# AlexandreRouma/SDRPlusPlus

Measured on AMD Instinct MI355X. Metric: IQ Msamples/s ingested (65536-pt FFT + 32 VFO WFM), higher is better.
Workload: dtype f32

## Files before the change

sdrplusplus_amd/csrc/gfx950/sdrpp_gfx950.h:

```cpp
#pragma once
#include <hip/hip_runtime.h>
#include <stdint.h>

namespace sdrpp_k {

struct UniformF32 {
    const float __attribute__((address_space(4))) * p;
    __device__ __forceinline__ float operator[](int i) const { return p[i]; }
};
__device__ __forceinline__ UniformF32 as_uniform(const void* ptr) {
    UniformF32 u;
    u.p = (const float __attribute__((address_space(4)))*)(uintptr_t)ptr;
    return u;
}

struct UniformI32 {
    const int __attribute__((address_space(4))) * p;
    __device__ __forceinline__ int operator[](int i) const { return p[i]; }
};
__device__ __forceinline__ UniformI32 as_uniform_i32(const void* ptr) {
    UniformI32 u;
    u.p = (const int __attribute__((address_space(4)))*)(uintptr_t)ptr;
    return u;
}

__device__ __forceinline__ int wave_uniform(int v) { return __builtin_amdgcn_readfirstlane(v); }

typedef float f32x2 __attribute__((ext_vector_type(2)));
__device__ __forceinline__ float global_load_f32(const float* p, long long i) { return ((const float __attribute__((address_space(1)))*)(uintptr_t)p)[i]; }
__device__ __forceinline__ int global_load_i32(const int* p, long long i) { return ((const int __attribute__((address_space(1)))*)(uintptr_t)p)[i]; }
__device__ __forceinline__ float2 global_load_f32x2(const float2* p, long long i) {
    const f32x2 v = ((const f32x2 __attribute__((address_space(1)))*)(uintptr_t)p)[i];
    return make_float2(v.x, v.y);
}
__device__ __forceinline__ float4 global_load_f32x4(const float4* p, long long i) {
    typedef float f32x4_ld __attribute__((ext_vector_type(4)));
    const f32x4_ld v = ((const f32x4_ld __attribute__((address_space(1)))*)(uintptr_t)p)[i];
    return make_float4(v.x, v.y, v.z, v.w);
}
typedef float f32x4_a4 __attribute__((ext_vector_type(4), aligned(4)));
__device__ __forceinline__ float4 global_load_f32x4_unaligned(const float* p, long long i) {
    const f32x4_a4 v = *((const f32x4_a4 __attribute__((address_space(1)))*)(uintptr_t)(p + i));
    return make_float4(v.x, v.y, v.z, v.w);
}
__device__ __forceinline__ void global_store_f32x2(float2* p, long long i, float2 v) {
    f32x2 t;
    t.x = v.x;
    t.y = v.y;
    ((f32x2 __attribute__((address_space(1)))*)(uintptr_t)p)[i] = t;
}

__device__ __forceinline__ float2 global_load_f32x2_boff(const void* base, unsigned byte_off) {
    const f32x2 v = *((const f32x2 __attribute__((address_space(1)))*)((const char __attribute__((address_space(1)))*)(uintptr_t)base + byte_off));
    return make_float2(v.x, v.y);
}
__device__ __forceinline__ void global_store_f32x2_boff(void* base, unsigned byte_off, float2 v) {
    f32x2 t;
    t.x = v.x;
    t.y = v.y;
    *((f32x2 __attribute__((address_space(1)))*)((char __attribute__((address_space(1)))*)(uintptr_t)base + byte_off)) = t;
}

__device__ __forceinline__ void global_store_f32_boff(void* base, unsigned byte_off, float v) {
    *((float __attribute__((address_space(1)))*)((char __attribute__((address_space(1)))*)(uintptr_t)base + byte_off)) = v;
}

__device__ __forceinline__ float fast_rcp(float x) { return __builtin_amdgcn_rcpf(x); }

typedef float f32x4_a16 __attribute__((ext_vector_type(4)));
__device__ __forceinline__ void global_store_f32x4(float* p, long long i, float4 v) {
    f32x4_a16 t;
    t.x = v.x;
    t.y = v.y;
    t.z = v.z;
    t.w = v.w;
    *((f32x4_a16 __attribute__((address_space(1)))*)(uintptr_t)(p + i)) = t;
}

typedef unsigned u32x4_t __attribute__((ext_vector_type(4)));
__device__ __forceinline__ uint4 global_load_u32x4(const void* p, long long i) {
    const u32x4_t v = ((const u32x4_t __attribute__((address_space(1)))*)(uintptr_t)p)[i];
    return make_uint4(v.x, v.y, v.z, v.w);
}
__device__ __forceinline__ void global_store_u32x4(void* p, long long i, uint4 v) {
    u32x4_t t;
    t.x = v.x; t.y = v.y; t.z = v.z; t.w = v.w;
    ((u32x4_t __attribute__((address_space(1)))*)(uintptr_t)p)[i] = t;
}
__device__ __forceinline__ unsigned global_load_u32(const void* p, long long i) { return ((const unsigned __attribute__((address_space(1)))*)(uintptr_t)p)[i]; }
__device__ __forceinline__ void global_store_u32(void* p, long long i, unsigned v) { ((unsigned __attribute__((address_space(1)))*)(uintptr_t)p)[i] = v; }

__device__ __forceinline__ void global_store_f32x4_unaligned(float* p, long long i, float4 v) {
    f32x4_a4 t;
    t.x = v.x;
    t.y = v.y;
    t.z = v.z;
    t.w = v.w;
    *((f32x4_a4 __attribute__((address_space(1)))*)(uintptr_t)(p + i)) = t;
}

__device__ __forceinline__ void sched_fence() { __builtin_amdgcn_sched_barrier(0); }
__device__ __forceinline__ int opaque(int v) {
    asm volatile("" : "+v"(v));
    return v;
}

__device__ __forceinline__ void wave_sync() {
    __builtin_amdgcn_fence(__ATOMIC_RELEASE, "wavefront");
    __builtin_amdgcn_wave_barrier();
    __builtin_amdgcn_fence(__ATOMIC_ACQUIRE, "wavefront");
}

#ifdef SDRPP_TICK_TRACE
__device__ unsigned long long g_tick_mark[1 << 16][4];
#define TICK_MARK(k)                                                                                      \
    do {                                                                                                  \
        if (threadIdx.x == 0) { g_tick_mark[blockIdx.x & 0xffff][k] = (unsigned long long)wall_clock64(); } \
    } while (0)
#else
#define TICK_MARK(k) \
    do {             \
    } while (0)
#endif

__device__ __forceinline__ void wave_stores_done() { asm volatile("s_waitcnt vmcnt(0) lgkmcnt(0)" ::: "memory"); }

__device__ __forceinline__ int wave_upper_bound(const int* ends, int n, int b, int* prev_end) {
    const int lane = threadIdx.x & 63;
    const int mine = global_load_i32(ends, lane < n ? lane : (n > 0 ? n - 1 : 0));
    const unsigned long long below = __ballot(lane < n && mine <= b);
    const int idx = (int)__builtin_popcountll(below);
    const int prev = __builtin_amdgcn_readlane(mine, idx > 0 ? idx - 1 : 0);
    *prev_end = idx > 0 ? prev : 0;
    return idx;
}

__device__ __forceinline__ void lds_flag_set(int* f, int v) { __hip_atomic_store(f, v, __ATOMIC_RELEASE, __HIP_MEMORY_SCOPE_WORKGROUP); }
#ifndef SDRPP_FLAG_SLEEP
#define SDRPP_FLAG_SLEEP 8
#endif
__device__ __forceinline__ void lds_flag_wait_ge(int* f, int need, int* timeouts) {
    int looks = 0;
    while (__hip_atomic_load(f, __ATOMIC_ACQUIRE, __HIP_MEMORY_SCOPE_WORKGROUP) < need) {
        __builtin_amdgcn_s_sleep(SDRPP_FLAG_SLEEP);
        if (++looks > (1 << 20)) {
            if ((threadIdx.x & 63) == 0 && timeouts) { __hip_atomic_fetch_add(timeouts, 1, __ATOMIC_RELAXED, __HIP_MEMORY_SCOPE_SYSTEM); }
            break;
        }
    }
}

__device__ __forceinline__ int wave_upper_bound64_rec(const int* ends, int n, int b, int* prev_end, const void* recs, int stride_bytes, int (&rec)[6]) {
    const int lane = threadIdx.x & 63;
    const int mine = global_load_i32(ends, lane);
    const float* rp = reinterpret_cast<const float*>(reinterpret_cast<const char*>(recs) + (size_t)lane * (size_t)stride_bytes);
    const float4 r0 = global_load_f32x4_unaligned(rp, 0);
    const float r4 = global_load_f32(rp, 4), r5 = global_load_f32(rp, 5);
    const unsigned long long below = __ballot(lane < n && mine <= b);
    const int idx = __popcll(below);
    const int prev = __builtin_amdgcn_readlane(mine, idx > 0 ? idx - 1 : 0);
    *prev_end = idx > 0 ? prev : 0;
    const int src = idx < 64 ? idx : 63;
    rec[0] = __builtin_amdgcn_readlane(__float_as_int(r0.x), src);
    rec[1] = __builtin_amdgcn_readlane(__float_as_int(r0.y), src);
    rec[2] = __builtin_amdgcn_readlane(__float_as_int(r0.z), src);
    rec[3] = __builtin_amdgcn_readlane(__float_as_int(r0.w), src);
    rec[4] = __builtin_amdgcn_readlane(__float_as_int(r4), src);
    rec[5] = __builtin_amdgcn_readlane(__float_as_int(r5), src);
    return idx;
}

__device__ __forceinline__ void wave_prio_high() { __builtin_amdgcn_s_setprio(3); }
__device__ __forceinline__ void wave_prio_low() { __builtin_amdgcn_s_setprio(0); }

__device__ __forceinline__ float wave_bcast(float v, int src) { return __int_as_float(__builtin_amdgcn_readlane(__float_as_int(v), src)); }
__device__ __forceinline__ float wave_shr1(float v, float first) {
    const float r = __shfl_up(v, 1, 64);
    return ((threadIdx.x & 63) == 0) ? first : r;
}
__device__ __forceinline__ int wave_first(bool pred) {
    const unsigned long long m = __ballot(pred);
    return m ? (int)__builtin_ctzll(m) : 64;
}
__device__ __forceinline__ float wave_sum(float v) {
#pragma unroll
    for (int d = 32; d >= 1; d >>= 1) { v += __shfl_xor(v, d, 64); }
    return v;
}
__device__ __forceinline__ float wave_max(float v) {
#pragma unroll
    for (int d = 32; d >= 1; d >>= 1) {
        const float o = __shfl_xor(v, d, 64);
        v = (o > v) ? o : v;
    }
    return v;
}

typedef float f32x16 __attribute__((ext_vector_type(16)));
__device__ __forceinline__ f32x16 mfma_zero() {
    f32x16 z;
#pragma unroll
    for (int i = 0; i < 16; i++) { z[i] = 0.0f; }
    return z;
}
__device__ __forceinline__ f32x16 mfma_32x32x2(float a, float b, f32x16 c) { return __builtin_amdgcn_mfma_f32_32x32x2f32(a, b, c, 0, 0, 0); }

__device__ __forceinline__ void pk_sum_diff_f32(float2 a, float2 b, f32x2& s, f32x2& d) {
    f32x2 av, bv;
    av.x = a.x; av.y = a.y; bv.x = b.x; bv.y = b.y;
    asm("v_pk_add_f32 %0, %2, %3\n\tv_pk_add_f32 %1, %2, %3 neg_lo:[1,0] neg_hi:[0,1]\n\ts_nop 1" : "=&v"(s), "=&v"(d) : "v"(av), "v"(bv));
}

typedef float f32x4 __attribute__((ext_vector_type(4)));
__device__ __forceinline__ f32x4 mfma4_zero() {
    f32x4 z;
    z[0] = 0.0f; z[1] = 0.0f; z[2] = 0.0f; z[3] = 0.0f;
    return z;
}
__device__ __forceinline__ f32x4 mfma_16x16x4(float a, float b, f32x4 c) { return __builtin_amdgcn_mfma_f32_16x16x4f32(a, b, c, 0, 0, 0); }

}
```

sdrplusplus_amd/csrc/host_ctx.h:

```cpp
#pragma once

namespace {

constexpr int kArenaSlots = 24;
constexpr size_t kArenaBytes = 4u << 20;
constexpr int kRing = 4;
constexpr int kTickDepth = 18;
constexpr int kResSlots = SDRPP_RESULT_SLOTS;
constexpr int kGroupMax = SDRPP_GROUP_MAX;
constexpr int kResMeta = kResSlots * kGroupMax;
constexpr int kStageSlots = 4;
constexpr int kChanHistCap = 4095;
constexpr size_t kScratchBytes = 64u << 20;
constexpr int kMaxLds = 64 * 1024;

enum Family { F_FFT1 = 0, F_FFT2, F_FFTS, F_ZOOM, F_S1, F_DECIM, F_POLY, F_FIR, F_DEMOD, F_MISC, F_AF, F_PIPE, F_TICK };
const char* kFamilyNames[SDRPP_NUM_KERNEL_FAMILIES] = { "fft_pass1", "fft_pass2", "fft_single", "zoom_palette", "vfo_stage1",
                                                        "vfo_decim", "vfo_poly",  "vfo_fir",    "demod",        "carry_misc", "af_chain",  "vfo_pipe", "tick" };

struct Stream {
    int width = 2;
    int hist_len = 0;
    float* data = nullptr;
    float* base = nullptr;
    size_t cap = 0;
    float* hist[2] = { nullptr, nullptr };
    int cur = 0;
    int n = 0;
    float* extra[kRing - 1] = {};
    int n_extra = 0, rot = 0;
    int clevel = 0;
    int wlevel = 0;
};

struct ToepTab {
    float* d_tl = nullptr;
    int* d_lb = nullptr;
    int tl_len = 0, nsteps = 0, s_in = 0, rows = 0, nvar = 0;
    bool ok = false;
};

struct Vfo {
    bool nco_exact = false;
    int id = 0;
    sdrpp_vfo_desc d{};
    std::vector<float> staps[SDRPP_MAX_DECIM_STAGES];
    std::vector<float> rtaps, ctaps_chan, ataps;
    double theta = 0.0, phi = 0.0;
    std::vector<float2> modtaps;
    bool modtaps_dirty = true;
    int soff[SDRPP_MAX_DECIM_STAGES] = { 0, 0, 0, 0 };
    int tpp = 0, pphase = 0, poff = 0;
    long long seen = 0;
    float* d_staps[SDRPP_MAX_DECIM_STAGES] = { nullptr, nullptr, nullptr, nullptr };
    float* d_staps_nat[SDRPP_MAX_DECIM_STAGES] = { nullptr, nullptr, nullptr, nullptr };
    int s_kp[SDRPP_MAX_DECIM_STAGES] = { 0, 0, 0, 0 };
    float* d_bank = nullptr;
    float* d_cyc = nullptr;
    int cyc_rows = 0, cyc_lmax = 0;
    int chan_kp = 0, audio_kp = 0;
    float* d_chan = nullptr;
    int chan_ntaps = 0;
    std::vector<float> chan_stale;
    float* d_audio = nullptr;
    int audio_ntaps = 0;
    char* d_state = nullptr;
    double theta2 = 0.0, phi2 = 0.0;
    std::vector<Stream> st;
    int i_first = 0, i_poly = -1, i_chan = -1, i_dem = -1, i_out = -1, i_if = 0;
    int lvl_if = 1, lvl_out = 1, lvl_af = 1;
    std::vector<int> tk_if, tk_af;
    ToepTab tp_stage[SDRPP_MAX_DECIM_STAGES], tp_poly, tp_chan, tp_audio;
    bool fused_front = false;
    bool no_fuse = false;
    unsigned long long tap_hash = 0;
    float* d_h12 = nullptr;
    int h12_K = 0, h12_lgD = 0;
    struct Retune { long long pos; double theta_before; };
    std::vector<Retune> recs;
    int i_rot = -1;
    float2* d_rot = nullptr;
    struct Af {
        bool on = false;
        int n_stages = 0, decim_s[SDRPP_MAX_DECIM_STAGES] = { 1, 1, 1, 1 };
        std::vector<float> staps[SDRPP_MAX_DECIM_STAGES], rtaps, htaps;
        float* d_staps[SDRPP_MAX_DECIM_STAGES] = { nullptr, nullptr, nullptr, nullptr };
        int s_kp[SDRPP_MAX_DECIM_STAGES] = { 0, 0, 0, 0 };
        ToepTab tp_stage[SDRPP_MAX_DECIM_STAGES], tp_poly, tp_hpf;
        int interp = 1, decim = 1, tpp = 0;
        float* d_bank = nullptr;
        float* d_hpf = nullptr;
        int hpf_kp = 0;
        float alpha = 0.0f;
        float2* d_last = nullptr;
        int state_cur = 0;
        float4* d_seg = nullptr;
        int seg_cap = 0;
        int soff[SDRPP_MAX_DECIM_STAGES] = { 0, 0, 0, 0 };
        int pphase = 0, poff = 0;
        int i_stage0 = -1, i_poly = -1, i_hpf = -1, i_deemp = -1, i_last = -1;
        int base = -1;
    } af;
};

struct TimingPair { hipEvent_t a, b; int family; };

}

struct sdrpp_ctx {
    int device = 0;
    int64_t max_push = 0;
    hipStream_t own_stream = nullptr;
    hipStream_t stream = nullptr;
    hipStream_t fft_stream = nullptr;
    hipStream_t launch_stream = nullptr;
    hipEvent_t ev_fork = nullptr, ev_join = nullptr;
    std::string err;
    std::string devinfo;

    float* iq_land[2] = { nullptr, nullptr };
    int16_t* iq_land16[2] = { nullptr, nullptr };
    hipEvent_t land_ev[2] = { nullptr, nullptr };
    bool land_used[2] = { false, false };
    int land_cur = 0;
    hipStream_t copy_stream = nullptr;
    hipStream_t side_stream = nullptr;
    std::mutex side_mtx;
    bool async_staged = false;
    bool async_inflight = false;
    hipEvent_t ev_copy = nullptr;
    bool deferred = false;
    int64_t pending = 0;
    std::vector<int> pend_ends;
    float* iq_hist[2] = { nullptr, nullptr };
    int iq_hist_cap = 0;
    int iq_cur = 0;

    struct Pre {
        bool ref_order = false;
        bool on = false;
        int n_stages = 0, decim_s[SDRPP_MAX_DECIM_STAGES] = { 1, 1, 1, 1 };
        std::vector<float> staps[SDRPP_MAX_DECIM_STAGES];
        ToepTab tp[SDRPP_MAX_DECIM_STAGES];
        float* d_staps[SDRPP_MAX_DECIM_STAGES] = { nullptr, nullptr, nullptr, nullptr };
        int s_kp[SDRPP_MAX_DECIM_STAGES] = { 0, 0, 0, 0 };
        int soff[SDRPP_MAX_DECIM_STAGES] = { 0, 0, 0, 0 };
        float dc_rate = 0.0f;
        int conj = 0;
        Stream raw;
        std::vector<Stream> st;
        Stream out;
        float2* d_off = nullptr;
        int state_cur = 0;
        float4* d_seg = nullptr;
        int seg_cap = 0;
        const float* last = nullptr;
        int last_n = 0;
    } pre;

    struct Wf {
        int height = 0;
        float* d_ring = nullptr;
        int cur = 0, lines = 0;
        int width = 0;
        float* d_latest = nullptr;
        float* d_smooth = nullptr;
        float* d_hold = nullptr;
        bool hold_on = false, have_latest = false;
        float alpha = 0.0f, beta = 1.0f, hold_speed = 0.0f;
    } wf;

    char* d_pack = nullptr;
    size_t pack_cap = 0;
    float2* d_gather = nullptr;
    size_t gather_cap = 0;
    GatherJob* d_gather_jobs = nullptr;
    int gather_jobs_cap = 0;

    char* arena_host[kArenaSlots] = {};
    char* arena_host_dev[kArenaSlots] = {};
    hipEvent_t arena_ev[kArenaSlots] = {};
    bool arena_used[kArenaSlots] = {};
    char* arena_dev_slot[kArenaSlots] = {};
    char* arena_dev = nullptr;
    int arena_slot = 0;
    size_t arena_off = 0;

    bool fft_on = false;
    int fft_size = 0, fft_lg = 0, nz = 0, skip = 0;
    float* d_window = nullptr;
    float2* d_tw1 = nullptr;
    float2* d_tw2 = nullptr;
    float2* d_twn = nullptr;
    float2* d_scratch = nullptr;
    float* d_lines = nullptr;
    float* d_lines_grp = nullptr;
    int zoom_grp = 0;
    size_t lines_cap = 0;
    int64_t fft_pos = 0, fft_next = 0;
    int n_lines = 0;
    int view_start = 0, view_size = 0, data_width = 0;
    float wf_min = -120.0f, wf_max = 0.0f;
    int32_t* d_zstart = nullptr;
    std::vector<int32_t> h_zstart, h_zcount;
    int zoom_tp_cache = 0, zoom_tp_grp = -1;
    int32_t* d_zcount = nullptr;
    float* d_zoomed = nullptr;
    int32_t* d_index = nullptr;
    size_t zoom_cap = 0;
    struct FftBufs { float2* scratch = nullptr; float* lines = nullptr; float* grp = nullptr; float* zoomed = nullptr; int32_t* index = nullptr; };
    FftBufs fft_extra[kRing - 1];
    int fft_extra_n = 0, fft_rot = 0;

    int ref_block = 0;
    int nco_exact = 0;
    int pipe_on = 1;
    bool pipe_launched = false;
    int timeouts_seen = 0;
    std::vector<int> vfo_bounds;

    std::map<int, std::unique_ptr<Vfo>> vfos;
    std::vector<Vfo*> vfo_list;
// ... 108 lines not shown
```

sdrplusplus_amd/csrc/host_util.h:

```cpp
#pragma once

namespace {

int fail(sdrpp_ctx* c, int code, const char* fmt, ...) {
    char buf[512];
    va_list ap;
    va_start(ap, fmt);
    vsnprintf(buf, sizeof(buf), fmt, ap);
    va_end(ap);
    if (c) { c->err = buf; }
    return code;
}

#define HIPCHK(c, expr)                                                                                           \
    do {                                                                                                          \
        hipError_t e_ = (expr);                                                                                   \
        if (e_ != hipSuccess) { return fail((c), SDRPP_ERR_HIP, "%s failed: %s", #expr, hipGetErrorString(e_)); } \
    } while (0)

template <class T>
int dev_alloc(sdrpp_ctx* c, T** p, size_t count) {
    void* q = nullptr;
    hipError_t e = hipMalloc(&q, std::max<size_t>(count * sizeof(T), 16));
    if (e != hipSuccess) { return fail(c, SDRPP_ERR_NOMEM, "hipMalloc(%zu bytes) failed: %s", count * sizeof(T), hipGetErrorString(e)); }
// ... 173 lines not shown
    }
    if (s.hist_len > 0) {
        HIPCHK(c, hipMemcpy(nh[0] + (size_t)(new_len - s.hist_len) * s.width, s.hist[s.cur], (size_t)s.hist_len * s.width * sizeof(float), hipMemcpyDeviceToDevice));
    }
    dev_free(s.hist[0]);
    dev_free(s.hist[1]);
    s.hist[0] = nh[0];
    s.hist[1] = nh[1];
    s.cur = 0;
    s.hist_len = new_len;
    return SDRPP_OK;
}

int ensure_iq_hist(sdrpp_ctx* c, int need) {
    if (need <= c->iq_hist_cap) { return SDRPP_OK; }
    int cap = std::max(need, 1024);
    float* nh[2] = { nullptr, nullptr };
    for (int i = 0; i < 2; i++) {
        int rc = dev_alloc(c, &nh[i], (size_t)cap * 2);
        if (rc) { return rc; }
        HIPCHK(c, hipMemset(nh[i], 0, (size_t)cap * 2 * sizeof(float)));
    }
    if (c->iq_hist[c->iq_cur] && c->iq_hist_cap > 0) {
        HIPCHK(c, hipStreamSynchronize(c->stream));
        HIPCHK(c, hipMemcpy(nh[0] + (size_t)(cap - c->iq_hist_cap) * 2, c->iq_hist[c->iq_cur], (size_t)c->iq_hist_cap * 2 * sizeof(float), hipMemcpyDeviceToDevice));
    }
    dev_free(c->iq_hist[0]);
    dev_free(c->iq_hist[1]);
    c->iq_hist[0] = nh[0];
    c->iq_hist[1] = nh[1];
    c->iq_cur = 0;
    c->iq_hist_cap = cap;
    return SDRPP_OK;
}

std::vector<float> blocked_taps(const float* h, int K, int D, int* kp_out) {
    const int R = SDRPP_FIR_R;
    const int per = (K + D - 1) / D;
    const int kp = ((per + R - 1) / R) * R;
    std::vector<float> t((size_t)D * kp, 0.0f);
    for (int k = 0; k < K; k++) { t[(size_t)(k % D) * kp + (size_t)(k / D)] = h[k]; }
    *kp_out = kp;
    return t;
}
int upload_blocked(sdrpp_ctx* c, float** dst, const float* h, int K, int D, int* kp) {
    std::vector<float> t = blocked_taps(h, K, D, kp);
    return upload(c, dst, t.data(), t.size());
}

void toep_free(ToepTab& T) {
    dev_free(T.d_tl);
    dev_free(T.d_lb);
    T = ToepTab{};
}
int toep_upload(sdrpp_ctx* c, ToepTab& T, const std::vector<float>& tl, const std::vector<int>& lb) {
    dev_free(T.d_tl);
    dev_free(T.d_lb);
    T.ok = false;
    int rc = upload(c, &T.d_tl, tl.data(), tl.size());
    if (rc) { return rc; }
    rc = upload(c, &T.d_lb, lb.data(), lb.size());
    if (rc) { return rc; }
    T.tl_len = (int)tl.size();
    T.nvar = (int)lb.size() / 64;
    const int span = (2 * 16 - 1) * T.s_in + 4 * T.nsteps, pl = (span + 8) & ~3;
    T.ok = ((size_t)((T.tl_len + 3) & ~3) + (size_t)4 * 2 * pl) * sizeof(float) <= (size_t)(160 * 1024 / 3);
    return SDRPP_OK;
}
int toep_build_fir(sdrpp_ctx* c, ToepTab& T, const float* h, int K, int D) {
    const int rows = 15, padl = (rows - 1) * D, kp = K + padl, nsteps = (kp + 3) / 4;
    const int mainlen = padl + 4 * nsteps + 4, zb = mainlen;
    std::vector<float> tl((size_t)mainlen + 4 * (size_t)nsteps + 4, 0.0f);
    for (int k = 0; k < K; k++) { tl[(size_t)padl + k] = h[k]; }
    std::vector<int> lb(64);
    for (int lane = 0; lane < 64; lane++) {
        const int m = lane & 15, kk = lane >> 4;
        lb[(size_t)lane] = (m < rows) ? padl - D * m + kk : zb + kk;
    }
    T.nsteps = nsteps;
    T.s_in = rows * D;
    T.rows = rows;
    return toep_upload(c, T, tl, lb);
}
int toep_build_poly(sdrpp_ctx* c, ToepTab& T, const std::vector<float>& bank, int L, int M, int tpp) {
    const int cy_n = 15 / L;
    if (cy_n < 1) { return SDRPP_OK; }
    const int rows = cy_n * L, omax = ((L - 1) + (L - 1) * M) / L, shift_max = (cy_n - 1) * M + omax;
    const int kp = shift_max + tpp, nsteps = (kp + 3) / 4, padp = shift_max, row = padp + 4 * nsteps + 4, zb = L * row;
    std::vector<float> tl((size_t)zb + 4 * (size_t)nsteps + 4, 0.0f);
    for (int ph = 0; ph < L; ph++) {
        for (int q = 0; q < tpp; q++) { tl[(size_t)ph * row + (size_t)padp + q] = bank[(size_t)ph * tpp + q]; }
    }
    std::vector<int> lb((size_t)L * 64);
    for (int ph0 = 0; ph0 < L; ph0++) {
        for (int lane = 0; lane < 64; lane++) {
            const int m = lane & 15, kk = lane >> 4;
            if (m < rows) {
                const int cy = m / L, r = m % L, A = ph0 + r * M;
                lb[(size_t)ph0 * 64 + lane] = (A % L) * row + padp - (cy * M + A / L) + kk;
            }
            else { lb[(size_t)ph0 * 64 + lane] = zb + kk; }
        }
    }
    T.nsteps = nsteps;
    T.s_in = cy_n * M;
    T.rows = rows;
    return toep_upload(c, T, tl, lb);
}

void build_modtaps(Vfo& v) {
    const int K = v.d.stage_ntaps[0];
    const int npairs = (K + 1) / 2;
    v.modtaps.resize((size_t)npairs);
    const double kc = 0.5 * (double)(K - 1);
    for (int k = 0; k < npairs; k++) {
        double t = ((double)k - kc) * v.theta;
        t -= std::rint(t);
        const double a = 2.0 * 3.14159265358979323846 * t;
        const double h = (double)v.staps[0][(size_t)k];
        v.modtaps[(size_t)k] = make_float2((float)(h * std::cos(a)), (float)(h * std::sin(a)));
    }
    if (K & 1) { v.modtaps[(size_t)npairs - 1] = make_float2(v.staps[0][(size_t)npairs - 1], 0.0f); }
    v.modtaps_dirty = false;
}

void vfo_free(Vfo& v) {
    for (int i = 0; i < SDRPP_MAX_DECIM_STAGES; i++) { dev_free(v.d_staps[i]); dev_free(v.d_staps_nat[i]); }
    dev_free(v.d_bank);
    dev_free(v.d_cyc);
    dev_free(v.d_chan);
    dev_free(v.d_audio);
    dev_free(v.d_state);
    dev_free(v.d_h12);
    dev_free(v.d_rot);
    for (int i = 0; i < SDRPP_MAX_DECIM_STAGES; i++) { toep_free(v.tp_stage[i]); }
    toep_free(v.tp_poly);
    toep_free(v.tp_chan);
    toep_free(v.tp_audio);
    for (int i = 0; i < SDRPP_MAX_DECIM_STAGES; i++) {
        dev_free(v.af.d_staps[i]);
        toep_free(v.af.tp_stage[i]);
    }
    toep_free(v.af.tp_poly);
    toep_free(v.af.tp_hpf);
    dev_free(v.af.d_bank);
    dev_free(v.af.d_hpf);
    dev_free(v.af.d_last);
    dev_free(v.af.d_seg);
    for (auto& s : v.st) { stream_free(s); }
    v.st.clear();
}

int vfo_reset_state(sdrpp_ctx* c, Vfo& v) {
    v.phi = 0.0;
    v.phi2 = 0.0;
    v.seen = 0;
    v.recs.clear();
    std::fill(v.chan_stale.begin(), v.chan_stale.end(), 0.0f);
    for (int i = 0; i < SDRPP_MAX_DECIM_STAGES; i++) { v.soff[i] = 0; }
    v.pphase = 0;
    v.poff = 0;
    for (int i = 0; i < SDRPP_MAX_DECIM_STAGES; i++) { v.af.soff[i] = 0; }
    v.af.pphase = 0;
    v.af.poff = 0;
    if (v.af.d_last) { HIPCHK(c, hipMemsetAsync(v.af.d_last, 0, 2 * sizeof(float2), c->stream)); }
    for (auto& s : v.st) {
        for (int i = 0; i < 2; i++) {
            if (s.hist[i]) { HIPCHK(c, hipMemsetAsync(s.hist[i], 0, (size_t)std::max(s.hist_len, 1) * s.width * sizeof(float), c->stream)); }
        }
        s.n = 0;
    }
    AgcState st[2];
    for (int i = 0; i < 2; i++) {
        st[i].set_point = v.d.agc_set_point;
        st[i].attack = v.d.agc_attack;
        st[i].inv_attack = 1.0f - v.d.agc_attack;
        st[i].decay = v.d.agc_decay;
        st[i].inv_decay = 1.0f - v.d.agc_decay;
        st[i].max_gain = v.d.agc_max_gain;
        st[i].max_output_amp = v.d.agc_max_output_amp;
        st[i].amp = v.d.agc_set_point / v.d.agc_init_gain;
    }
    char blob[2 * sizeof(AgcState) + sizeof(float)];
    memcpy(blob, st, sizeof(st));
    float zero = 0.0f;
    memcpy(blob + sizeof(st), &zero, sizeof(float));
    HIPCHK(c, hipStreamSynchronize(c->stream));
    HIPCHK(c, hipMemcpy(v.d_state, blob, sizeof(blob), hipMemcpyHostToDevice));
    const float2 unit[2] = { make_float2(1.0f, 0.0f), make_float2(1.0f, 0.0f) };
    HIPCHK(c, hipMemcpy(v.d_rot, unit, sizeof(unit), hipMemcpyHostToDevice));
    return SDRPP_OK;
}

inline int decim_nout(int n, int off, int D) { return (n > off) ? (n - off + D - 1) / D : 0; }
inline int poly_nout(int n, int poff, int pphase, int L, int M) {
    if (n <= poff) { return 0; }
    const long long need = (long long)L * (n - poff) - pphase;
    return (int)((need + M - 1) / M);
}

void bounds_decim(std::vector<int>& b, int off, int D) {
    for (auto& x : b) { x = decim_nout(x, off, D); }
}
void bounds_poly(std::vector<int>& b, int poff, int pphase, int L, int M) {
    for (auto& x : b) { x = poly_nout(x, poff, pphase, L, M); }
}

struct HostProf {
    struct Acc { double total = 0.0, mx = 0.0; long n = 0; };
    std::map<std::string, Acc> acc;
    bool on = getenv("SDRPP_GPU_HOSTPROF") != nullptr;
    void add(const char* name, double us) {
        Acc& a = acc[name];
        a.total += us;
        a.mx = std::max(a.mx, us);
        a.n++;
    }
    void report() {
        if (!on) { return; }
        for (auto& kv : acc) { fprintf(stderr, "[sdrpp hostprof] %-28s n=%6ld avg %8.1f us max %9.1f us\n", kv.first.c_str(), kv.second.n, kv.second.total / (double)kv.second.n, kv.second.mx); }
    }
};
HostProf g_hostprof;
struct HostScope {
    const char* name;
    std::chrono::steady_clock::time_point t0;
    explicit HostScope(const char* n) : name(n) { if (g_hostprof.on) { t0 = std::chrono::steady_clock::now(); } }
    ~HostScope() {
        if (g_hostprof.on) { g_hostprof.add(name, std::chrono::duration<double, std::micro>(std::chrono::steady_clock::now() - t0).count()); }
    }
};

template <class K, class... A>
void launch(sdrpp_ctx* c, K kernel, dim3 grid, dim3 block, size_t lds, A... args) {
    if (c->tick_planning) {
        if (!c->tick_abort && getenv("SDRPP_TICK_DEBUG")) { fprintf(stderr, "[sdrpp tick] ordinary pass because of %s\n", __PRETTY_FUNCTION__); }
        c->tick_abort = true;
        return;
    }
    HostScope hs("launch");
    hipLaunchKernelGGL(kernel, grid, block, lds, c->launch_stream, args...);
}

void launch_role(sdrpp_ctx* c, const sdrpp_ctx::RoleLaunch& r) {
    const TickEntry& e = r.e;
    const dim3 grid((unsigned)e.gx, (unsigned)e.gy), b256(256);
    hipStream_t st = c->launch_stream;
    HostScope hs("launch");
    switch (e.role) {
    case TR_COPY: hipLaunchKernelGGL(copy_kernel, grid, b256, 0, st, (const CopyJob*)e.jobs); break;
    case TR_CARRY: hipLaunchKernelGGL(carry_kernel, grid, b256, 0, st, (const CarryJob*)e.jobs, e.aux); break;
    case TR_ROT: hipLaunchKernelGGL(vfo_rotate_kernel, grid, b256, 0, st, e.p.src, (const RotJob*)e.jobs); break;
    case TR_FCM_132_4: hipLaunchKernelGGL((vfo_frontcm_kernel<10, 132, 4>), grid, b256, r.lds, st, e.p.src, (const FrontCMJob*)e.jobs); break;
    case TR_FCM_6: hipLaunchKernelGGL((vfo_frontcm_kernel<6, 0, 0>), grid, b256, r.lds, st, e.p.src, (const FrontCMJob*)e.jobs); break;
    case TR_FCM_10: hipLaunchKernelGGL((vfo_frontcm_kernel<10, 0, 0>), grid, b256, r.lds, st, e.p.src, (const FrontCMJob*)e.jobs); break;
    case TR_FCM_16: hipLaunchKernelGGL((vfo_frontcm_kernel<16, 0, 0>), grid, b256, r.lds, st, e.p.src, (const FrontCMJob*)e.jobs); break;
    case TR_FCM16_132_4: hipLaunchKernelGGL((vfo_frontcm16_kernel<132, 4>), grid, b256, r.lds, st, e.p.src, (const FrontCMJob*)e.jobs); break;
    case TR_FCL_0: hipLaunchKernelGGL((vfo_frontcl_kernel<0>), grid, dim3(128), r.lds, st, e.p.src, (const FrontCMJob*)e.jobs); break;
    case TR_FCL_PF: hipLaunchKernelGGL((vfo_frontcl_kernel<SDRPP_FCL_PF>), grid, dim3(128), r.lds, st, e.p.src, (const FrontCMJob*)e.jobs); break;
    case TR_TOEP_C: hipLaunchKernelGGL((vfo_toep_kernel<2, 2, false>), grid, b256, r.lds, st, (const ToepJob*)e.jobs); break;
    case TR_TOEP_R: hipLaunchKernelGGL((vfo_toep_kernel<1, 2, false>), grid, b256, r.lds, st, (const ToepJob*)e.jobs); break;
    case TR_TOEP_Q: hipLaunchKernelGGL((vfo_toep_kernel<1, 2, true>), grid, b256, r.lds, st, (const ToepJob*)e.jobs); break;
    case TR_FIRB_C: hipLaunchKernelGGL((vfo_firb_kernel<2, false>), grid, dim3((unsigned)e.aux), r.lds, st, (const FirBJob*)e.jobs); break;
    case TR_FIRB_R: hipLaunchKernelGGL((vfo_firb_kernel<1, false>), grid, dim3((unsigned)e.aux), r.lds, st, (const FirBJob*)e.jobs); break;
    case TR_FIRB_S: hipLaunchKernelGGL((vfo_firb_kernel<1, true>), grid, dim3((unsigned)e.aux), r.lds, st, (const FirBJob*)e.jobs); break;
    case TR_FIRB_Q: hipLaunchKernelGGL((vfo_firb_kernel<1, true, true>), grid, dim3((unsigned)e.aux), r.lds, st, (const FirBJob*)e.jobs); break;
    case TR_PRE: hipLaunchKernelGGL(vfo_demod_pre_kernel, grid, b256, 0, st, (const PreJob*)e.jobs); break;
    case TR_SEQ: hipLaunchKernelGGL(vfo_sequential_kernel, grid, dim3(64), 0, st, (const SeqJob*)e.jobs, e.aux); break;
    case TR_PIPE: hipLaunchKernelGGL(vfo_pipe_kernel<1>, grid, b256, r.lds, st, (const PipeJob*)e.jobs); break;
    case TR_POLYC: hipLaunchKernelGGL(vfo_polyc_kernel, grid, b256, r.lds, st, (const PolyJob*)e.jobs, e.aux); break;
    case TR_DEEMP_P0: hipLaunchKernelGGL((vfo_deemph_kernel<0, 0>), grid, b256, 0, st, (const DeempJob*)e.jobs); break;
    case TR_DEEMP_P1: hipLaunchKernelGGL((vfo_deemph_kernel<0, 1>), grid, b256, 0, st, (const DeempJob*)e.jobs); break;
    case TR_DC_P0: hipLaunchKernelGGL((vfo_deemph_kernel<1, 0>), grid, b256, 0, st, (const DeempJob*)e.jobs); break;
    case TR_DC_P1: hipLaunchKernelGGL((vfo_deemph_kernel<1, 1>), grid, b256, 0, st, (const DeempJob*)e.jobs); break;
    case TR_WF_RING: hipLaunchKernelGGL(wf_ring_store_kernel, grid, b256, 0, st, e.p.wf.src, e.p.wf.n0, e.p.wf.n1, e.p.wf.a, e.p.wf.n2, e.p.wf.n3); break;
    case TR_WF_TRACE: hipLaunchKernelGGL(wf_trace_kernel, grid, b256, 0, st, e.p.wf.src, e.p.wf.n0, e.p.wf.n1, e.p.wf.a, e.p.wf.b, e.p.wf.f0, e.p.wf.f1, e.p.wf.c, e.p.wf.f2); break;
    default: break;
    }
}
void emit(sdrpp_ctx* c, int level, int fam, int role, int gx, int gy, size_t lds, const void* jobs, const IqSrc* src = nullptr, int aux = 0) {
    if (gx <= 0 || gy <= 0) { return; }
    sdrpp_ctx::RoleLaunch r{};
    r.e.role = role;
    r.e.gx = gx;
    r.e.gy = gy;
    r.e.aux = aux;
    r.e.jobs = jobs;
    if (src) { r.e.p.src = *src; }
    r.lds = lds;
    r.level = level;
    r.fam = fam;
    if (c->tick_planning) { c->emits.push_back(r); }
    else { launch_role(c, r); }
}

void emit_wf(sdrpp_ctx* c, int level, int fam, int role, int gx, int gy, const TickWf& q) {
    if (gx <= 0 || gy <= 0) { return; }
    sdrpp_ctx::RoleLaunch r{};
    r.e.role = role;
    r.e.gx = gx;
    r.e.gy = gy;
    r.e.p.wf = q;
    r.level = level;
    r.fam = fam;
    if (c->tick_planning) { c->emits.push_back(r); }
    else { launch_role(c, r); }
}

int pick_tile(int D, int K, int width_bytes) {
    for (int tile : { 256, 128, 64 }) {
        const int extra = (K - 1 + D - 1) / D;
        const size_t lds = (size_t)D * (tile + extra + 1) * width_bytes;
        if (lds <= (size_t)kMaxLds) { return tile; }
    }
    return 0;
}
size_t fir_lds(int tile, int D, int K, int width_bytes) {
    const int extra = (K - 1 + D - 1) / D;
    return (size_t)D * (tile + extra + 1) * width_bytes;
}

}
```

sdrplusplus_amd/csrc/plan_push.h:

```cpp
#pragma once

namespace {

struct PlanSnapshot {
    struct V { int soff[SDRPP_MAX_DECIM_STAGES]; int pphase, poff; double phi, phi2; long long seen; int i_if, lvl_if, lvl_out, lvl_af; int n[24], cur[24]; size_t nrecs;
               int af_soff[SDRPP_MAX_DECIM_STAGES], af_pphase, af_poff, af_last, af_state; };
    std::vector<V> v;
    int64_t fft_pos, fft_next;
    int n_lines, iq_cur, wf_cur, wf_lines;
    bool wf_have;
    int pre_soff[SDRPP_MAX_DECIM_STAGES], pre_state, pre_raw_cur, pre_cur[SDRPP_MAX_DECIM_STAGES];
};
void plan_snapshot(sdrpp_ctx* c, PlanSnapshot& S, bool rotate = false) {
    S.v.resize(c->vfo_list.size());
    for (size_t i = 0; i < c->vfo_list.size(); i++) {
        Vfo& v = *c->vfo_list[i];
        PlanSnapshot::V& q = S.v[i];
        for (int k = 0; k < SDRPP_MAX_DECIM_STAGES; k++) { q.soff[k] = v.soff[k]; q.af_soff[k] = v.af.soff[k]; }
        q.pphase = v.pphase; q.poff = v.poff; q.phi = v.phi; q.phi2 = v.phi2; q.seen = v.seen; q.i_if = v.i_if; q.lvl_if = v.lvl_if; q.lvl_out = v.lvl_out; q.lvl_af = v.lvl_af;
        q.nrecs = v.recs.size();
        q.af_pphase = v.af.pphase; q.af_poff = v.af.poff; q.af_last = v.af.i_last; q.af_state = v.af.state_cur;
        for (size_t k = 0; k < v.st.size() && k < 24; k++) { q.n[k] = v.st[k].n; q.cur[k] = v.st[k].cur; }
        if (rotate) {
            for (auto& st : v.st) { stream_rotate(st); }
        }
    }
    S.fft_pos = c->fft_pos; S.fft_next = c->fft_next; S.n_lines = c->n_lines; S.iq_cur = c->iq_cur;
    S.wf_cur = c->wf.cur; S.wf_lines = c->wf.lines; S.wf_have = c->wf.have_latest;
    for (int k = 0; k < SDRPP_MAX_DECIM_STAGES; k++) { S.pre_soff[k] = c->pre.soff[k]; }
    S.pre_state = c->pre.state_cur;
    S.pre_raw_cur = c->pre.raw.cur;
    for (size_t k = 0; k < c->pre.st.size() && k < SDRPP_MAX_DECIM_STAGES; k++) { S.pre_cur[k] = c->pre.st[k].cur; }
}
void plan_restore(sdrpp_ctx* c, const PlanSnapshot& S) {
    for (size_t i = 0; i < c->vfo_list.size(); i++) {
        Vfo& v = *c->vfo_list[i];
        const PlanSnapshot::V& q = S.v[i];
        for (int k = 0; k < SDRPP_MAX_DECIM_STAGES; k++) { v.soff[k] = q.soff[k]; v.af.soff[k] = q.af_soff[k]; }
        v.pphase = q.pphase; v.poff = q.poff; v.phi = q.phi; v.phi2 = q.phi2; v.seen = q.seen; v.i_if = q.i_if; v.lvl_if = q.lvl_if; v.lvl_out = q.lvl_out; v.lvl_af = q.lvl_af;
        v.af.pphase = q.af_pphase; v.af.poff = q.af_poff; v.af.i_last = q.af_last; v.af.state_cur = q.af_state;
        for (size_t k = 0; k < v.st.size() && k < 24; k++) { v.st[k].n = q.n[k]; v.st[k].cur = q.cur[k]; }
    }
    c->fft_pos = S.fft_pos; c->fft_next = S.fft_next; c->n_lines = S.n_lines; c->iq_cur = S.iq_cur;
    c->wf.cur = S.wf_cur; c->wf.lines = S.wf_lines; c->wf.have_latest = S.wf_have;
    for (int k = 0; k < SDRPP_MAX_DECIM_STAGES; k++) { c->pre.soff[k] = S.pre_soff[k]; }
    c->pre.state_cur = S.pre_state;
    c->pre.raw.cur = S.pre_raw_cur;
    for (size_t k = 0; k < c->pre.st.size() && k < SDRPP_MAX_DECIM_STAGES; k++) { c->pre.st[k].cur = S.pre_cur[k]; }
}

void block_bounds(sdrpp_ctx* c, int64_t count, const std::vector<int>* push_ends) {
    c->arena_begins++;
    c->arena_allocs = 0;
    std::vector<int>& B = c->vfo_bounds;
    B.clear();
    const std::vector<int> whole{ (int)count };
    int64_t lo = 0;
    for (int e : (push_ends ? *push_ends : whole)) {
        if (c->ref_block > 0) {
            for (int64_t q = lo + c->ref_block; q < e; q += c->ref_block) { B.push_back((int)q); }
        }
        if (e > lo || B.empty()) { B.push_back(e); }
        lo = e;
    }
}
int iq_hist_need(sdrpp_ctx* c) {
    int need_hist = 1;
    if (c->fft_on) { need_hist = std::max(need_hist, c->nz - 1); }
    for (auto& kv : c->vfos) {
        const sdrpp_vfo_desc& d = kv.second->d;
        if (d.n_stages > 0) { need_hist = std::max(need_hist, d.stage_ntaps[0] - 1); }
        if (d.n_stages > 1) { need_hist = std::max(need_hist, d.stage_ntaps[0] - 1 + d.stage_decim[0] * (d.stage_ntaps[1] - 1)); }
    }
    return need_hist;
}
CarryJob iq_carry_job(sdrpp_ctx* c, const float* d_iq, int64_t count) {
    int need = 1;
    if (c->fft_on) {
        const int64_t P = (int64_t)c->nz + c->skip;
        const int64_t partial = c->fft_pos - c->fft_next * P;
        if (partial > 0) { need = std::max(need, (int)std::min<int64_t>(partial, c->nz - 1)); }
    }
    for (auto& kv : c->vfos) {
        const sdrpp_vfo_desc& d = kv.second->d;
        if (d.n_stages > 0) { need = std::max(need, d.stage_ntaps[0] - 1); }
        if (d.n_stages > 1) { need = std::max(need, d.stage_ntaps[0] - 1 + d.stage_decim[0] * (d.stage_ntaps[1] - 1)); }
    }
    need = std::min(need, c->iq_hist_cap);
    return CarryJob{ d_iq, c->iq_hist[c->iq_cur], c->iq_hist[c->iq_cur ^ 1], c->iq_hist_cap, (int)count, 2, need };
}

int push_common(sdrpp_ctx* c, const float* d_iq, int64_t count, const std::vector<int>* push_ends = nullptr) {
    if (count == 0) {
        c->n_lines = 0;
        for (auto& kv : c->vfos) {
            for (auto& s : kv.second->st) { s.n = 0; }
        }
        return SDRPP_OK;
    }
    int rc0;
    {
        HostScope hs("arena_begin (backpressure)");
        rc0 = arena_begin(c);
    }
    if (rc0) { return rc0; }
    static thread_local PlanSnapshot snap;
    plan_snapshot(c, snap);
    c->plan_lvl0 = 0;
    block_bounds(c, count, push_ends);
    if (c->pre.on) {
        rc0 = run_preproc(c, &d_iq, &count);
        if (rc0) {
            plan_restore(c, snap);
            return rc0;
        }
        if (count == 0) {
            c->n_lines = 0;
            for (auto& kv : c->vfos) {
                for (auto& s : kv.second->st) { s.n = 0; }
            }
            return arena_end(c);
        }
    }
    int rc = ensure_iq_hist(c, iq_hist_need(c));
    if (rc) {
        plan_restore(c, snap);
        return rc;
    }
    IqSrc src{ (const float2*)d_iq, (const float2*)c->iq_hist[c->iq_cur], c->iq_hist_cap, (long long)count };
    bool fft_work = false;
    if (c->fft_on) {
        const int64_t P = (int64_t)c->nz + c->skip;
        fft_work = (c->fft_pos + count) - c->nz - c->fft_next * P >= 0;
    }
    const bool fork = fft_work && !c->vfos.empty();
    if (fork) {
        HostScope hs("fork events");
        HIPCHK(c, hipEventRecord(c->ev_fork, c->stream));
        HIPCHK(c, hipStreamWaitEvent(c->fft_stream, c->ev_fork, 0));
        c->launch_stream = c->fft_stream;
    }
    {
        HostScope hs("do_fft");
        rc = do_fft(c, src, count);
    }
    c->launch_stream = c->stream;
    if (fork) { (void)hipEventRecord(c->ev_join, c->fft_stream); }
    if (!rc) {
        const CarryJob iqc = iq_carry_job(c, d_iq, count);
        if (c->vfos.empty()) {
            std::vector<CarryJob> carry{ iqc };
            CarryJob* d_carry = arena_push(c, carry);
            rc = arena_commit(c);
            if (!rc) {
                FamilyTimer t(c, F_MISC);
                const int iq_elems = carry[0].need * 2;
                launch(c, carry_kernel, dim3((unsigned)std::max(1, std::min((iq_elems + 8191) / 8192, 512)), 1), dim3(256), 0, (const CarryJob*)d_carry, 0);
            }
        }
        else {
            HostScope hs("do_vfos");
            rc = do_vfos_plan(c, src, count, iqc);
        }
    }
    HostScope hs2("join + arena_end");
    if (fork) { (void)hipStreamWaitEvent(c->stream, c->ev_join, 0); }
    if (rc) {
        plan_restore(c, snap);
        (void)arena_end(c);
        return rc;
    }
    c->iq_cur ^= 1;
    rc = arena_end(c);
    if (rc) { return rc; }
    hipError_t e = hipGetLastError();
    if (e != hipSuccess) { return fail(c, SDRPP_ERR_HIP, "kernel launch failed: %s", hipGetErrorString(e)); }
    return SDRPP_OK;
}

}
```

sdrplusplus_amd/csrc/plan_vfo.h:

```cpp
#pragma once

namespace {

struct S1Member { Vfo* v; int K, lgD, off0, nout; double phi0; int min_idx; int fused, K2, lgD2, off2, nout2; unsigned long long taph;
                  int shift = 0, oshift = 0; };

std::string member_key(char kind, const S1Member* m, int n) {
    unsigned long long h1 = 1469598103934665603ull ^ (unsigned char)kind, h2 = 0x9e3779b97f4a7c15ull + (unsigned char)kind;
    for (int i = 0; i < n; i++) {
        unsigned long long tb;
        memcpy(&tb, &m[i].v->theta, 8);
        const unsigned long long id = (unsigned long long)(unsigned)m[i].v->id;
        h1 = (h1 ^ id) * 1099511628211ull;
        h1 = (h1 ^ tb) * 1099511628211ull;
        h2 ^= id + 0x9e3779b97f4a7c15ull + (h2 << 6) + (h2 >> 2);
        h2 ^= tb + 0x9e3779b97f4a7c15ull + (h2 << 6) + (h2 >> 2);
    }
    char raw[16];
    memcpy(raw, &h1, 8);
    memcpy(raw + 8, &h2, 8);
    return std::string(raw, 16);
}

int front2_t2(int K1, int D1, int K2, int D2, int vt) {
// ... 10 lines not shown
bool frontcm_ok(int K1, int lgD1, int K2, int lgD2, int* pf) {
    const int K = K1 + (K2 - 1) * (1 << lgD1), lgD = lgD1 + lgD2;
    if (K < 9 || lgD < 1 || lgD > 5) { return false; }
    const int nsamp = (SDRPP_FCM_TILE - 1) * (1 << lgD) + K;
    if (nsamp > 16 * 64) { return false; }
    *pf = nsamp <= 6 * 64 ? 6 : (nsamp <= 10 * 64 ? 10 : 16);
    return (size_t)frontcm_layout(K, lgD).total * 4 <= (size_t)(160 * 1024 / 3);
}

ToepJob toep_job(const ToepTab& T, int var, StreamIn in, float* out, int base0, int nout, float inv_dev) {
    ToepJob j{};
    j.in = in;
    j.out = out;
    j.tl = T.d_tl;
    j.lbase = T.d_lb + (size_t)var * 64;
    j.tl_len = T.tl_len;
    j.nsteps = T.nsteps;
    j.s_in = T.s_in;
    j.rows = T.rows;
    j.base0 = base0;
    j.nout = nout;
    j.mt_per_wave = 1;
    j.inv_deviation = inv_dev;
    return j;
}

struct ToepPlan { int grid_x = 0; size_t lds = 0; };
ToepPlan toep_plan(std::vector<ToepJob>& jobs, int npl, int max_blocks = 2048) {
    ToepPlan P;
    if (jobs.empty()) { return P; }
    const int G = 2;
    int mtw = 1;
    for (; mtw < 16; mtw++) {
        size_t blocks = 0;
        for (auto& jb : jobs) { blocks += (size_t)((jb.nout + G * 16 * jb.rows - 1) / (G * 16 * jb.rows) + 4 * mtw - 1) / (size_t)(4 * mtw); }
        if (blocks <= (size_t)max_blocks) { break; }
    }
    for (auto& jb : jobs) {
        jb.mt_per_wave = mtw;
        const int nmt = (jb.nout + G * 16 * jb.rows - 1) / (G * 16 * jb.rows);
        P.grid_x = std::max(P.grid_x, (nmt + 4 * mtw - 1) / (4 * mtw));
        const int span = (G * 16 - 1) * jb.s_in + 4 * jb.nsteps, pl = (span + 8) & ~3;
        P.lds = std::max(P.lds, ((size_t)((jb.tl_len + 3) & ~3) + (size_t)4 * npl * pl) * sizeof(float));
    }
    return P;
}

void launch_toep(sdrpp_ctx* c, std::vector<ToepJob>& jobs, ToepJob* d_jobs, const ToepPlan& P, int width, bool quad) {
    if (jobs.empty() || P.grid_x == 0) { return; }
    const dim3 grid((unsigned)P.grid_x, (unsigned)jobs.size());
    if (quad) { launch(c, vfo_toep_kernel<1, 2, true>, grid, dim3(256), P.lds, (const ToepJob*)d_jobs); }
    else if (width == 2) { launch(c, vfo_toep_kernel<2, 2, false>, grid, dim3(256), P.lds, (const ToepJob*)d_jobs); }
    else { launch(c, vfo_toep_kernel<1, 2, false>, grid, dim3(256), P.lds, (const ToepJob*)d_jobs); }
}

constexpr int kPipeG = 1;
constexpr int kPipeBpc = 5;
constexpr int kPipeBpcMin = 3;
bool pipe_layout_try(PipeJob& J, int fifo_tiles, size_t* lds_bytes) {
    const int G = kPipeG;
    int off = 0;
    auto take = [&](int nfloats) { const int o = off; off += (nfloats + 3) & ~3; return o; };
    for (int s = 0; s < 4; s++) { J.tl_off[s] = take(J.st[s].tl_len); }
    int W[4], span[4], omt[4];
    for (int s = 0; s < 4; s++) {
        W[s] = G * 16 * J.st[s].s_in;
        span[s] = W[s] - J.st[s].s_in + 4 * J.st[s].nsteps;
        omt[s] = G * 16 * J.st[s].rows;
    }
    if (((span[0] + 1) >> 1) > (G == 1 ? 5 : 9) * 64) { return false; }
    J.win_off = take(2 * ((span[0] + 8) & ~3));
    J.zero_lo = off;
    for (int i = 0; i < 3; i++) {
        const int s = i + 1, h = span[s] - W[s];
        if (h < 0) { return false; }
        const int R = std::max(2, (W[s] + h + omt[i] + W[s] - 1) / W[s]) * W[s];
        if (i < 2) {
            J.ring_len[i] = R;
            J.ring_mir[i] = h;
            J.ring_off[i] = take(2 * (R + h));
        }
        else {
            J.dring_len = R;
            J.dring_mir = h;
            J.dring_off = take(R + h);
        }
    }
    J.ring_len[2] = fifo_tiles * omt[2];
    J.ring_mir[2] = 0;
    J.ring_off[2] = take(J.ring_len[2]);
    J.zero_hi = off;
    J.flag_off = take(8);
    *lds_bytes = (size_t)off * sizeof(float);
    return *lds_bytes <= (size_t)(160 * 1024) / kPipeBpcMin;
}
bool pipe_layout(PipeJob& J, size_t* lds_bytes) { return pipe_layout_try(J, 2, lds_bytes) || pipe_layout_try(J, 1, lds_bytes); }
int pipe_segments(const std::vector<PipeJob>& pipes, int forced, size_t lds) {
    if (pipes.empty()) { return 0; }
    const int bpc = std::max(kPipeBpcMin, std::min(kPipeBpc, (int)((size_t)(160 * 1024) / std::max<size_t>(lds, 1))));
    int max_nmt = 1;
    for (auto& pj : pipes) { max_nmt = std::max(max_nmt, (pj.st[3].nout + kPipeG * 16 * pj.st[3].rows - 1) / (kPipeG * 16 * pj.st[3].rows)); }
    if (forced >= 2) { return std::min(forced, max_nmt); }
    const int s_full = (256 * bpc + (int)pipes.size() - 1) / (int)pipes.size();
    if (max_nmt >= 12 * s_full) { return s_full; }
    if (max_nmt <= 16) { return std::max(1, (max_nmt + 1) / 2); }
    return 0;
}

constexpr int kLevels = 28;
template <class T>
struct Lev {
    std::vector<T> at[kLevels];
    T* dev[kLevels] = {};
    int top = 0;
    void add(int l, const T& j) {
        if (l >= kLevels) { l = kLevels - 1; }
        at[l].push_back(j);
        if (l + 1 > top) { top = l + 1; }
    }
};
template <class T>
bool arena_push_lev(sdrpp_ctx* c, Lev<T>& L) {
    for (int l = 0; l < L.top; l++) {
        if (L.at[l].empty()) { continue; }
        L.dev[l] = arena_push(c, L.at[l]);
        if (!L.dev[l]) { return false; }
    }
    return true;
}

struct BankPlan {
    sdrpp_ctx* c;
    IqSrc src{};
    int n_in = 0;
    bool ticking = false;
    int L0 = 0;
    static constexpr int carry_last = kLevels - 1;
    static constexpr int carry_wave_max = 8192;
    const std::vector<int>& fb;
    bool blocks = false;
    std::vector<S1Member> s1;
    std::vector<RotJob> rot;
    Lev<FirBJob> f_dec;
    std::vector<RotXJob> rotx;
    std::vector<RetuneJob> retune;
    Lev<PolyJob> poly;
    Lev<PolyBJob> polyb[4];
    Lev<FirBJob> chan;
    Lev<SeqJob> seq;
    Lev<PreJob> pre;
    Lev<FirBJob> audio;
    Lev<FirBJob> audio_fm;
    Lev<ToepJob> t_dec, t_poly, t_chan, t_audio, t_audio_fm;
    std::vector<PipeJob> pipes;
    size_t pipe_lds = 0;
    PipeJob* d_pipes = nullptr;
    int pipe_seg = 0;
    int pipe_lvl = 0;
    Lev<ToepJob> t_af_dec, t_af_poly, t_af_hpf;
    Lev<FirBJob> af_dec, af_hpf;
    Lev<PolyJob> af_poly;
    Lev<DeempJob> af_deemp;
    Lev<SsbRotXJob> ssbx_l;
    Lev<CarryJob> carry;
    int max_rot = 0;
    struct S1Launch { int vt; std::vector<Stage1Job> jobs; int max_nout = 0; int tile = 256; size_t lds = 0; };
    struct F2Launch { int vt; std::vector<Front2Job> jobs; int max_blocks = 0; size_t lds = 0; };
    struct FCMLaunch { std::vector<FrontCMJob> jobs; int max_blocks = 0; size_t lds = 0; };
    S1Launch s1l[4];
    F2Launch f2l[4];
    FCMLaunch fcm[3];
    FCMLaunch fcl;
    int fcl_nw = 2;
    const int vts[4] = { 8, 4, 2, 1 };
    Stage1Job* d_s1[4] = {};
    Front2Job* d_f2[4] = {};
    FrontCMJob* d_fcl = nullptr;
    FrontCMJob* d_fcm[3] = {};
    RotXJob* d_rotx = nullptr;
    RotXHead* d_rotx_head = nullptr;
    RetuneJob* d_retune = nullptr;
    RotJob* d_rot = nullptr;
    const int* d_fb = nullptr;
    struct ToepList { Lev<ToepJob>* L; int npl, width; bool quad; int fam; int role; };
    static constexpr int kToepLists = 8;
    ToepList tlists[kToepLists] = { { &t_dec, 2, 2, false, F_DECIM, TR_TOEP_C },      { &t_poly, 2, 2, false, F_POLY, TR_TOEP_C },       { &t_chan, 2, 2, false, F_FIR, TR_TOEP_C },
                                    { &t_audio, 1, 1, false, F_FIR, TR_TOEP_R },      { &t_audio_fm, 2, 1, true, F_FIR, TR_TOEP_Q },     { &t_af_dec, 2, 2, false, F_AF, TR_TOEP_C },
                                    { &t_af_poly, 2, 2, false, F_AF, TR_TOEP_C },     { &t_af_hpf, 2, 2, false, F_AF, TR_TOEP_C } };
    ToepPlan tplan[kToepLists][kLevels];

    explicit BankPlan(sdrpp_ctx* c_) : c(c_), fb(c_->vfo_bounds) {
        for (int i = 0; i < 4; i++) { s1l[i].vt = vts[i]; f2l[i].vt = vts[i]; }
    }
    template <class T>
    static void lev_reset(Lev<T>& L) {
        for (int l = 0; l < L.top; l++) {
            L.at[l].clear();
            L.dev[l] = nullptr;
        }
        L.top = 0;
    }
    void begin(const IqSrc& src_, int64_t count, const CarryJob& iq_carry) {
        src = src_;
        n_in = (int)count;
        ticking = c->tick_planning;
        L0 = ticking ? c->plan_lvl0 : 0;
        blocks = fb.size() > 1;
        s1.clear(); rot.clear(); rotx.clear(); retune.clear(); pipes.clear();
        lev_reset(f_dec); lev_reset(poly);
        for (auto& q : polyb) { lev_reset(q); }
        lev_reset(chan); lev_reset(seq); lev_reset(pre); lev_reset(audio); lev_reset(audio_fm);
        lev_reset(t_dec); lev_reset(t_poly); lev_reset(t_chan); lev_reset(t_audio); lev_reset(t_audio_fm);
        lev_reset(t_af_dec); lev_reset(t_af_poly); lev_reset(t_af_hpf); lev_reset(af_dec); lev_reset(af_hpf); lev_reset(af_poly); lev_reset(af_deemp);
        lev_reset(ssbx_l); lev_reset(carry);
        pipe_lds = 0;
        d_pipes = nullptr;
        pipe_seg = 0;
        pipe_lvl = 0;
        max_rot = 0;
        fcl_nw = 2;
        for (int i = 0; i < 4; i++) {
            s1l[i].jobs.clear(); s1l[i].max_nout = 0; s1l[i].tile = 256; s1l[i].lds = 0;
            f2l[i].jobs.clear(); f2l[i].max_blocks = 0; f2l[i].lds = 0;
            d_s1[i] = nullptr;
            d_f2[i] = nullptr;
        }
        for (int i = 0; i < 3; i++) {
            fcm[i].jobs.clear(); fcm[i].max_blocks = 0; fcm[i].lds = 0;
            d_fcm[i] = nullptr;
        }
        fcl.jobs.clear(); fcl.max_blocks = 0; fcl.lds = 0;
        d_fcl = nullptr; d_rotx = nullptr; d_retune = nullptr; d_rot = nullptr; d_fb = nullptr;
        for (auto& row : tplan) {
            for (auto& q : row) { q = ToepPlan{}; }
        }
        carry.add(ticking ? L0 + 1 : carry_last, iq_carry);
    }
    BankPlan(const BankPlan&) = delete;
    BankPlan& operator=(const BankPlan&) = delete;

    int chain(Vfo& v) {
        Stream* cur = &v.st[(size_t)v.i_first];
        int lvl = L0 + 1;
        for (auto& s : v.st) { s.clevel = 0; s.wlevel = 0; }
        cur->wlevel = lvl;
        const bool agc_mode = v.d.demod == SDRPP_DEMOD_AM || (v.d.demod >= SDRPP_DEMOD_USB && v.d.demod <= SDRPP_DEMOD_DSB);
        const bool need_bnd = agc_mode && (blocks || v.nco_exact);
        std::vector<int> bnd;
        if (need_bnd) { bnd = fb; }
        const bool split = c->grp_ends.size() > 1;
        std::vector<int>& tk = v.tk_if;
        tk.clear();
        v.tk_af.clear();
        if (split) { tk = c->grp_ends; }
        int first_sep = 0;
        double phi_end = 0.0;
        bool have_phi_end = false;
        if (v.nco_exact) {
            Stream* tgt = (v.d.n_stages == 0) ? cur : &v.st[(size_t)v.i_rot];
            rotx.push_back(RotXJob{ (float2*)tgt->data, v.d_rot, v.d.phase_delta_re, v.d.phase_delta_im });
            tgt->n = n_in;
            tgt->wlevel = lvl;
            cur = tgt;
        }
        else if (v.d.n_stages == 0) {
            rot.push_back(RotJob{ v.theta, v.phi, (float2*)cur->data, n_in });
            cur->n = n_in;
            max_rot = std::max(max_rot, n_in);
        }
        else {
            const int D = v.d.stage_decim[0];
            const int nout = decim_nout(n_in, v.soff[0], D);
            if (v.modtaps_dirty) { build_modtaps(v); }
            const int K0 = v.d.stage_ntaps[0];
            S1Member mem{ &v, K0, ilog2(D), v.soff[0], nout, v.phi, 0, 0, 0, 0, 0, 0, v.tap_hash };
            int need = K0 - 1;
            first_sep = 1;
            if (need_bnd) { bounds_decim(bnd, v.soff[0], D); }
            if (split) { bounds_decim(tk, v.soff[0], D); }
            if (v.fused_front) {
                const int D2 = v.d.stage_decim[1];
                mem.fused = 1;
                mem.K2 = v.d.stage_ntaps[1];
                mem.lgD2 = ilog2(D2);
                mem.off2 = v.soff[1];
                mem.nout2 = decim_nout(nout, v.soff[1], D2);
                need = K0 - 1 + D * (mem.K2 - 1);
                first_sep = 2;
                if (need_bnd) { bounds_decim(bnd, v.soff[1], D2); }
                if (split) { bounds_decim(tk, v.soff[1], D2); }
            }
            mem.min_idx = (v.seen >= need) ? -need : -(int)v.seen;
            if (!split) { s1.push_back(mem); }
            else {
                int so0 = v.soff[0], so1 = v.soff[1], prev_e = 0, oshift = 0;
                long long seen = v.seen;
                double ph = v.phi;
                for (size_t j = 0; j < c->grp_ends.size(); j++) {
                    const int nj = c->grp_ends[j] - prev_e;
                    S1Member m = mem;
                    m.off0 = so0;
                    m.nout = decim_nout(nj, so0, D);
                    m.phi0 = ph;
                    int outs = m.nout;
                    if (mem.fused) {
                        m.off2 = so1;
                        m.nout2 = decim_nout(m.nout, so1, v.d.stage_decim[1]);
                        outs = m.nout2;
                    }
                    m.min_idx = ((seen >= need) ? -need : -(int)seen) + prev_e;
                    m.shift = prev_e;
                    m.oshift = oshift;
                    if (outs > 0) { s1.push_back(m); }
                    so0 = so0 + m.nout * D - nj;
                    if (mem.fused) { so1 = so1 + m.nout2 * v.d.stage_decim[1] - m.nout; }
                    const double pj = ph + (double)nj * v.theta;
                    ph = pj - std::floor(pj);
                    seen += nj;
                    oshift += outs;
                    prev_e = c->grp_ends[j];
                }
                phi_end = ph;
                have_phi_end = true;
            }
            {
                const int D1 = D, Kc = v.h12_K;
                const int off = mem.fused ? mem.off0 + (mem.off2 - (mem.K2 - 1)) * D1 - (K0 - 1) : mem.off0 - (K0 - 1);
                const int nout_f = mem.fused ? mem.nout2 : nout;
                while (!v.recs.empty() && v.recs.front().pos - v.seen <= (long long)off) { v.recs.erase(v.recs.begin()); }
                while (v.recs.size() > SDRPP_RETUNE_MAX_SEG - 1) { v.recs.erase(v.recs.begin()); }
                if (!v.recs.empty() && nout_f > 0) {
                    const long long r_last = v.recs.back().pos - v.seen;
                    const long long Dc = 1ll << v.h12_lgD;
                    const int nfix = (int)std::min<long long>((long long)nout_f, (r_last - off + Dc - 1) / Dc);
                    if (nfix > 0) {
                        RetuneJob rj{};
                        rj.out = (float2*)v.st[(size_t)v.i_first + (mem.fused ? 1 : 0)].data;
                        rj.taps = v.d_h12;
                        rj.K = Kc;
                        rj.log2_decim = v.h12_lgD;
                        rj.off = off;
                        rj.nfix = nfix;
                        rj.min_idx = mem.min_idx;
                        const int nr = (int)v.recs.size();
                        rj.nseg = nr + 1;
                        double P = v.phi + v.theta * (double)r_last;
                        for (int q = nr; q >= 1; q--) {
                            const long long Sq = v.recs[(size_t)q - 1].pos - v.seen;
                            rj.start[q] = (int)std::max<long long>(Sq, -2000000000ll);
                            rj.theta[q] = (q == nr) ? v.theta : v.recs[(size_t)q].theta_before;
                            rj.phi[q] = P - std::floor(P);
                            if (q >= 2) {
                                const long long Sp = v.recs[(size_t)q - 2].pos - v.seen;
                                P = P + v.recs[(size_t)q - 1].theta_before * (double)(Sp - Sq);
                            }
                        }
                        rj.start[0] = rj.start[1];
                        rj.theta[0] = v.recs[0].theta_before;
                        rj.phi[0] = rj.phi[1];
                        retune.push_back(rj);
                    }
                }
            }
            v.soff[0] = v.soff[0] + nout * D - n_in;
            cur->n = nout;
            if (mem.fused) {
                Stream* nxt = &v.st[(size_t)v.i_first + 1];
                v.soff[1] = v.soff[1] + mem.nout2 * v.d.stage_decim[1] - nout;
                cur->n = 0;
                nxt->n = mem.nout2;
                nxt->wlevel = lvl;
                cur = nxt;
            }
        }
        const int last_dec = v.d.n_stages - 1;
        bool piped_be = c->pipe_on && !ticking && (v.d.demod == SDRPP_DEMOD_WFM || v.d.demod == SDRPP_DEMOD_NFM) && last_dec >= first_sep && v.tp_stage[last_dec].ok &&
                        v.i_poly >= 0 && v.tp_poly.ok && v.i_chan >= 0 && v.chan_ntaps > 0 && v.tp_chan.ok && v.tp_audio.ok;
        PipeJob pj{};
        size_t pj_lds = 0;
        if (piped_be) {
            pj.st[0] = toep_job(v.tp_stage[last_dec], 0, StreamIn{}, nullptr, 0, 0, 0.0f);
            pj.st[1] = toep_job(v.tp_poly, 0, StreamIn{}, nullptr, 0, 0, 0.0f);
            pj.st[2] = toep_job(v.tp_chan, 0, StreamIn{}, nullptr, 0, 0, 0.0f);
            pj.st[3] = toep_job(v.tp_audio, 0, StreamIn{}, nullptr, 0, 0, 0.0f);
            pj.timeouts = c->hd_tick_flag ? (int*)(c->hd_tick_flag + 8) : nullptr;
            piped_be = pipe_layout(pj, &pj_lds);
        }
        for (int s = first_sep; s < v.d.n_stages; s++) {
            Stream* nxt = &v.st[(size_t)v.i_first + s];
            const int Ds = v.d.stage_decim[s];
            const int no = decim_nout(cur->n, v.soff[s], Ds);
            if (need_bnd) { bounds_decim(bnd, v.soff[s], Ds); }
            if (split) { bounds_decim(tk, v.soff[s], Ds); }
            lvl++;
            cur->clevel = lvl;
            if (piped_be && s == last_dec) {
                pj.st[0] = toep_job(v.tp_stage[s], 0, stream_in(*cur), nxt->data, v.soff[s] - (v.d.stage_ntaps[s] - 1), no, 0.0f);
                pj.keep[0] = std::max(0, no - nxt->hist_len);
                pj.dec_stage = s;
                pj.lvl = lvl;
            }
            else if (v.tp_stage[s].ok) { t_dec.add(lvl, toep_job(v.tp_stage[s], 0, stream_in(*cur), nxt->data, v.soff[s] - (v.d.stage_ntaps[s] - 1), no, 0.0f)); }
            else { f_dec.add(lvl, FirBJob{ stream_in(*cur), nxt->data, v.d_staps[s], v.d.stage_ntaps[s], ilog2(Ds), v.soff[s], no, v.s_kp[s] }); }
            v.soff[s] = v.soff[s] + no * Ds - cur->n;
            nxt->n = no;
            nxt->wlevel = lvl;
            cur = nxt;
        }
        if (v.i_poly >= 0) {
            Stream* nxt = &v.st[(size_t)v.i_poly];
            const int no = poly_nout(cur->n, v.poff, v.pphase, v.d.interp, v.d.decim);
            if (need_bnd) { bounds_poly(bnd, v.poff, v.pphase, v.d.interp, v.d.decim); }
            if (split) { bounds_poly(tk, v.poff, v.pphase, v.d.interp, v.d.decim); }
            lvl++;
            cur->clevel = lvl;
            if (piped_be) {
                pj.st[1] = toep_job(v.tp_poly, v.pphase, stream_in(*cur), nxt->data, v.poff - (v.tpp - 1), no, 0.0f);
                pj.keep[1] = std::max(0, no - nxt->hist_len);
            }
            else if (v.tp_poly.ok) { t_poly.add(lvl, toep_job(v.tp_poly, v.pphase, stream_in(*cur), nxt->data, v.poff - (v.tpp - 1), no, 0.0f)); }
            else if (v.d_cyc) {
                polyb[(v.cyc_lmax == 4 ? 0 : 1) + ((v.d.decim & 1) ? 2 : 0)].add(lvl, PolyBJob{ stream_in(*cur), (float2*)nxt->data, v.d_cyc + (size_t)v.pphase * v.cyc_rows * v.cyc_lmax, v.d.interp, v.d.decim,
                                                                  v.tpp, v.poff, no, v.cyc_rows });
            }
            else {
                poly.add(lvl, PolyJob{ stream_in(*cur), (float2*)nxt->data, v.d_bank, v.d.interp, v.d.decim, v.tpp, v.pphase, v.poff, no });
            }
            const long long A = (long long)v.pphase + (long long)no * v.d.decim;
            v.pphase = (int)(A % v.d.interp);
            v.poff = v.poff + (int)(A / v.d.interp) - cur->n;
            nxt->n = no;
            nxt->wlevel = lvl;
            cur = nxt;
        }
        if (v.i_chan >= 0 && v.chan_ntaps > 0) {
            Stream* nxt = &v.st[(size_t)v.i_chan];
            lvl++;
            cur->clevel = lvl;
            if (piped_be) {
                pj.st[2] = toep_job(v.tp_chan, 0, stream_in(*cur), nxt->data, -(v.chan_ntaps - 1), cur->n, 0.0f);
                pj.keep[2] = 0;
            }
            else if (v.tp_chan.ok) { t_chan.add(lvl, toep_job(v.tp_chan, 0, stream_in(*cur), nxt->data, -(v.chan_ntaps - 1), cur->n, 0.0f)); }
            else { chan.add(lvl, FirBJob{ stream_in(*cur), nxt->data, v.d_chan, v.chan_ntaps, 0, 0, cur->n, v.chan_kp }); }
            nxt->n = cur->n;
            nxt->wlevel = lvl;
            cur = nxt;
        }
        v.i_if = (int)(cur - &v.st[0]);
        v.lvl_if = lvl;
        v.lvl_out = lvl;
        const int nif = cur->n;
        AgcState* agc = (AgcState*)v.d_state;
        float* dc = (float*)(v.d_state + 2 * sizeof(AgcState));
        const int* d_bnd = nullptr;
        if (need_bnd) {
            d_bnd = arena_push(c, bnd);
            if (!d_bnd) { return fail(c, SDRPP_ERR_UNSUPPORTED, "job arena exhausted"); }
        }
        const int nbnd = need_bnd ? (int)bnd.size() : 0;
        if (v.d.demod == SDRPP_DEMOD_WFM || v.d.demod == SDRPP_DEMOD_NFM) {
            Stream& out = v.st[(size_t)v.i_out];
            lvl++;
            cur->clevel = lvl;
            if (piped_be) {
                pj.st[3] = toep_job(v.tp_audio, 0, stream_in(*cur), out.data, -(v.audio_ntaps - 1), nif, v.d.inv_deviation);
                pipes.push_back(pj);
                pipe_lds = std::max(pipe_lds, pj_lds);
            }
            else if (v.tp_audio.ok) { t_audio_fm.add(lvl, toep_job(v.tp_audio, 0, stream_in(*cur), out.data, -(v.audio_ntaps - 1), nif, v.d.inv_deviation)); }
            else { audio_fm.add(lvl, FirBJob{ stream_in(*cur), out.data, v.d_audio, v.audio_ntaps, 0, 0, nif, v.audio_kp, v.d.inv_deviation }); }
            out.n = nif;
            out.wlevel = lvl;
            v.lvl_out = lvl;
        }
        else if (v.d.demod == SDRPP_DEMOD_AM) {
            Stream& dem = v.st[(size_t)v.i_dem];
            Stream& out = v.st[(size_t)v.i_out];
            if (!v.d.am_carrier_agc) { pre.add(lvl + 1, PreJob{ 2, nif, (const float2*)cur->data, dem.data, 0.0, 0.0 }); }
            seq.add(lvl + 2, SeqJob{ 2, nif, (const float2*)cur->data, dem.data, nullptr, agc, agc + 1, dc, v.d.dc_block_rate, v.d.am_carrier_agc, d_bnd, nbnd });
            dem.n = nif;
            dem.wlevel = lvl + 2;
            lvl += 3;
            dem.clevel = lvl;
            if (v.tp_audio.ok) { t_audio.add(lvl, toep_job(v.tp_audio, 0, stream_in(dem), out.data, -(v.audio_ntaps - 1), nif, 0.0f)); }
            else { audio.add(lvl, FirBJob{ stream_in(dem), out.data, v.d_audio, v.audio_ntaps, 0, 0, nif, v.audio_kp }); }
            out.n = nif;
            out.wlevel = lvl;
            v.lvl_out = lvl;
        }
        else if (v.d.demod >= SDRPP_DEMOD_USB && v.d.demod <= SDRPP_DEMOD_DSB) {
            Stream& dem = v.st[(size_t)v.i_dem];
            Stream& out = v.st[(size_t)v.i_out];
            if (v.nco_exact) { ssbx_l.add(lvl + 1, SsbRotXJob{ (const float2*)cur->data, dem.data, v.d_rot + 1, v.d.ssb_phase_delta_re, v.d.ssb_phase_delta_im, d_bnd, nbnd }); }
            else if (split) {
                int lo = 0;
                for (size_t j = 0; j < tk.size(); j++) {
                    const int nj = tk[j] - lo;
                    if (nj > 0) { pre.add(lvl + 1, PreJob{ v.d.demod, nj, (const float2*)cur->data + lo, dem.data + (size_t)lo * (size_t)dem.width, v.theta2, v.phi2 }); }
                    const double q2 = v.phi2 + (double)nj * v.theta2;
                    v.phi2 = q2 - std::floor(q2);
                    lo = tk[j];
                }
            }
            else { pre.add(lvl + 1, PreJob{ v.d.demod, nif, (const float2*)cur->data, dem.data, v.theta2, v.phi2 }); }
            seq.add(lvl + 2, SeqJob{ v.d.demod, nif, (const float2*)cur->data, dem.data, out.data, agc, agc + 1, dc, 0.0f, 0, d_bnd, nbnd });
            lvl += 2;
            dem.n = 0;
            out.n = nif;
            out.wlevel = lvl;
            v.lvl_out = lvl;
            if (!split || v.nco_exact) {
                const double p2 = v.phi2 + (double)nif * v.theta2;
                v.phi2 = p2 - std::floor(p2);
            }
        }
        if (v.af.on && v.i_out >= 0) {
            Vfo::Af& a = v.af;
            Stream* acur = &v.st[(size_t)v.i_out];
            if (split) { v.tk_af = tk; }
            for (int s = 0; s < a.n_stages; s++) {
                Stream* nxt = &v.st[(size_t)a.i_stage0 + s];
                const int Ds = a.decim_s[s], K = (int)a.staps[s].size();
                const int no = decim_nout(acur->n, a.soff[s], Ds);
                if (split) { bounds_decim(v.tk_af, a.soff[s], Ds); }
                lvl++;
                acur->clevel = lvl;
                if (a.tp_stage[s].ok) { t_af_dec.add(lvl, toep_job(a.tp_stage[s], 0, stream_in(*acur), nxt->data, a.soff[s] - (K - 1), no, 0.0f)); }
                else { af_dec.add(lvl, FirBJob{ stream_in(*acur), nxt->data, a.d_staps[s], K, ilog2(Ds), a.soff[s], no, a.s_kp[s] }); }
                a.soff[s] = a.soff[s] + no * Ds - acur->n;
                nxt->n = no;
                nxt->wlevel = lvl;
                acur = nxt;
            }
            if (a.i_poly >= 0) {
                Stream* nxt = &v.st[(size_t)a.i_poly];
                const int no = poly_nout(acur->n, a.poff, a.pphase, a.interp, a.decim);
                if (split) { bounds_poly(v.tk_af, a.poff, a.pphase, a.interp, a.decim); }
                lvl++;
                acur->clevel = lvl;
                if (a.tp_poly.ok) { t_af_poly.add(lvl, toep_job(a.tp_poly, a.pphase, stream_in(*acur), nxt->data, a.poff - (a.tpp - 1), no, 0.0f)); }
                else { af_poly.add(lvl, PolyJob{ stream_in(*acur), (float2*)nxt->data, a.d_bank, a.interp, a.decim, a.tpp, a.pphase, a.poff, no }); }
                const long long A = (long long)a.pphase + (long long)no * a.decim;
                a.pphase = (int)(A % a.interp);
                a.poff = a.poff + (int)(A / a.interp) - acur->n;
                nxt->n = no;
                nxt->wlevel = lvl;
                acur = nxt;
            }
            if (a.i_hpf >= 0) {
                Stream* nxt = &v.st[(size_t)a.i_hpf];
                const int K = (int)a.htaps.size();
                lvl++;
                acur->clevel = lvl;
                if (a.tp_hpf.ok) { t_af_hpf.add(lvl, toep_job(a.tp_hpf, 0, stream_in(*acur), nxt->data, -(K - 1), acur->n, 0.0f)); }
                else { af_hpf.add(lvl, FirBJob{ stream_in(*acur), nxt->data, a.d_hpf, K, 0, 0, acur->n, a.hpf_kp }); }
                nxt->n = acur->n;
                nxt->wlevel = lvl;
                acur = nxt;
            }
            if (a.i_deemp >= 0) {
                Stream* nxt = &v.st[(size_t)a.i_deemp];
                lvl++;
                const int nseg = std::min(a.seg_cap, (acur->n + SDRPP_DEEMP_SEG - 1) / SDRPP_DEEMP_SEG);
                af_deemp.add(lvl, DeempJob{ (const float2*)acur->data, (float2*)nxt->data, acur->n, a.alpha, a.d_last + a.state_cur, a.d_last + (a.state_cur ^ 1),
                                             a.d_seg + (size_t)a.state_cur * ((size_t)a.seg_cap + 1), nseg, 0 });
                if (nseg > 0) { a.state_cur ^= 1; }
                nxt->n = acur->n;
                lvl += 1;
                nxt->wlevel = lvl;
                acur = nxt;
            }
            a.i_last = (int)(acur - &v.st[0]);
            v.lvl_af = lvl;
        }
        if (have_phi_end) { v.phi = phi_end; }
        else {
            const double p = v.phi + (double)n_in * v.theta;
            v.phi = p - std::floor(p);
        }
        v.seen += n_in;
        const Stream* phantom = (v.fused_front && v.d.n_stages >= 2 && !v.nco_exact) ? &v.st[(size_t)v.i_first] : nullptr;
        for (auto& s : v.st) {
            if (s.hist_len > 0 && s.data && &s != phantom) {
                const int cl = !ticking ? carry_last : (s.clevel > 0 ? s.clevel : (s.wlevel > 0 ? s.wlevel + 1 : lvl + 1));
                carry.add(cl, CarryJob{ s.data, s.hist[s.cur], s.hist[s.cur ^ 1], s.hist_len, s.n, s.width, s.hist_len });
            }
        }
        c->plan_top = std::max(c->plan_top, lvl + 2);
        return SDRPP_OK;
    }

    int group_front() {
        auto same = [](const S1Member& a, const S1Member& b) {
            return a.fused == b.fused && a.K == b.K && a.lgD == b.lgD && a.off0 == b.off0 && a.nout == b.nout && a.min_idx == b.min_idx && a.K2 == b.K2 &&
                   a.lgD2 == b.lgD2 && a.off2 == b.off2 && a.nout2 == b.nout2 && a.taph == b.taph && a.shift == b.shift && a.oshift == b.oshift;
        };
        std::sort(s1.begin(), s1.end(), [](const S1Member& a, const S1Member& b) {
            if (a.fused != b.fused) { return a.fused < b.fused; }
            if (a.K != b.K) { return a.K < b.K; }
            if (a.lgD != b.lgD) { return a.lgD < b.lgD; }
            if (a.off0 != b.off0) { return a.off0 < b.off0; }
            if (a.nout != b.nout) { return a.nout < b.nout; }
            if (a.min_idx != b.min_idx) { return a.min_idx < b.min_idx; }
            if (a.K2 != b.K2) { return a.K2 < b.K2; }
            if (a.lgD2 != b.lgD2) { return a.lgD2 < b.lgD2; }
            if (a.off2 != b.off2) { return a.off2 < b.off2; }
            if (a.nout2 != b.nout2) { return a.nout2 < b.nout2; }
            if (a.taph != b.taph) { return a.taph < b.taph; }
            if (a.shift != b.shift) { return a.shift < b.shift; }
            if (a.oshift != b.oshift) { return a.oshift < b.oshift; }
            return a.v->id < b.v->id;
        });
        if (ticking) {
            fcl_nw = 4;
            for (auto& m : s1) {
                if (!m.fused && m.lgD >= 5 && m.K >= 9 && (size_t)frontcl_lds_floats(m.K, m.lgD, 4) * 4 > (size_t)(160 * 1024 / 2)) { fcl_nw = 2; }
            }
        }
        size_t i = 0;
        while (i < s1.size()) {
            size_t j = i;
            while (j < s1.size() && same(s1[j], s1[i])) { j++; }
            size_t g = i;
            int m_pf = 0;
            const bool m_fused = s1[i].fused && frontcm_ok(s1[i].K, s1[i].lgD, s1[i].K2, s1[i].lgD2, &m_pf);
            const bool m_long = !m_fused && !s1[i].fused && s1[i].lgD >= 5 && s1[i].K >= 9 && (size_t)frontcl_lds_floats(s1[i].K, s1[i].lgD) * 4 <= (size_t)kMaxLds;
            const bool m_ok = m_fused || m_long;
            const size_t m_min = m_long ? 2 : 17;
            while (m_ok && j - g >= m_min) {
                const int vt = (int)std::min<size_t>(j - g, SDRPP_FCM_VT);
                S1Member h = s1[g];
                if (m_long) {
                    h.K2 = 1;
                    h.lgD2 = 0;
                    h.off2 = 0;
                    h.nout2 = h.nout;
                }
                const int D1 = 1 << h.lgD;
                const int K = h.K + (h.K2 - 1) * D1, lgD = h.lgD + h.lgD2;
                const int NP = (K + 1) / 2, NP4 = (NP + 31) / 32 * 32;
                const std::string key = member_key(m_long ? 'L' : 'M', &s1[g], vt);
                float2* d_taps = nullptr;
                auto it = c->s1_tap_cache.find(key);
                if (it != c->s1_tap_cache.end()) { d_taps = it->second; }
                else {
                    std::vector<float2> host((size_t)NP4 * 32 + (size_t)SDRPP_FCM_VT * SDRPP_FCM_TILE, make_float2(0.0f, 0.0f));
                    float* at = reinterpret_cast<float*>(host.data());
                    std::vector<double> h12((size_t)K);
                    const double kc = 0.5 * (double)(K - 1);
                    for (int m = 0; m < vt; m++) {
                        const Vfo& vv = *s1[g + m].v;
                        std::fill(h12.begin(), h12.end(), 0.0);
                        for (int k2 = 0; k2 < h.K2; k2++) {
                            const double w2 = m_long ? 1.0 : (double)vv.staps[1][(size_t)k2];
                            for (int k1 = 0; k1 < h.K; k1++) { h12[(size_t)k2 * D1 + k1] += w2 * (double)vv.staps[0][(size_t)k1]; }
                        }
                        for (int pz = 0; pz < NP; pz++) {
                            double t = ((double)pz - kc) * vv.theta;
                            t -= std::rint(t);
                            const double a = 2.0 * 3.14159265358979323846 * t;
                            double gr = h12[(size_t)pz] * std::cos(a), gi = h12[(size_t)pz] * std::sin(a);
                            if ((K & 1) && pz == NP - 1) { gr = h12[(size_t)pz]; gi = 0.0; }
                            at[(size_t)pz * 64 + m] = (float)gr;
                            at[(size_t)pz * 64 + 32 + m] = (float)-gi;
                        }
                    }
                    for (int m = 0; m < SDRPP_FCM_VT; m++) {
                        const double step = m < vt ? s1[g + m].v->theta * (double)(1 << lgD) : 0.0;
                        for (int jj = 0; jj < SDRPP_FCM_TILE; jj++) {
                            double tt = step * (double)jj;
                            tt -= std::rint(tt);
                            const double a = 2.0 * 3.14159265358979323846 * tt;
                            host[(size_t)NP4 * 32 + (size_t)m * SDRPP_FCM_TILE + jj] = make_float2((float)std::cos(a), (float)std::sin(a));
                        }
                    }
                    if (c->s1_tap_cache.size() > 4096) {
                        HIPCHK(c, hipStreamSynchronize(c->stream));
                        for (auto& e : c->s1_tap_cache) { (void)hipFree(e.second); }
                        c->s1_tap_cache.clear();
                    }
                    int rc = dev_alloc(c, &d_taps, host.size());
                    if (rc) { return rc; }
                    HIPCHK(c, hipMemcpyAsync(d_taps, host.data(), host.size() * sizeof(float2), hipMemcpyHostToDevice, c->stream));
                    HIPCHK(c, hipStreamSynchronize(c->stream));
                    c->s1_tap_cache[key] = d_taps;
                }
                FrontCMJob job{};
                job.nv = vt;
                job.ntaps = K;
                job.log2_decim = lgD;
                job.off = h.off0 + (h.off2 - (h.K2 - 1)) * D1 - (h.K - 1) + h.shift;
                job.nout = h.nout2;
                job.min_idx = h.min_idx;
                job.anchor = h.shift;
                const int tile_n = (m_long && vt <= 16) ? 16 : SDRPP_FCM_TILE;
                const int ntiles = (h.nout2 + tile_n - 1) / tile_n;
                const int long_blocks = m_long ? std::max(1, (int)((size_t)(160 * 1024) / ((size_t)frontcl_lds_floats(K, lgD, fcl_nw) * 4))) : 0;
                const int nsub = std::max<int>(1, (int)c->grp_ends.size());
                const int resident = std::max(64, (m_long ? 256 * long_blocks * fcl_nw : (c->tick_planning ? std::min(3072, c->tick_fcm_waves) : 3072)) / nsub);
                job.tiles_per_wave = std::max(1, (ntiles + resident - 1) / resident);
                job.atab = reinterpret_cast<const float*>(d_taps);
                job.ptab = d_taps + (size_t)NP4 * 32;
                for (int m = 0; m < SDRPP_FCM_VT; m++) {
                    Vfo* v = s1[g + std::min(m, vt - 1)].v;
                    job.theta[m] = v->theta;
                    job.phi0[m] = s1[g + std::min(m, vt - 1)].phi0;
                    job.out[m] = (float2*)v->st[(size_t)v->i_first + (m_long ? 0 : 1)].data + h.oshift;
                }
                if (m_long) {
                    fcl.jobs.push_back(job);
                    fcl.max_blocks = std::max(fcl.max_blocks, (ntiles + fcl_nw * job.tiles_per_wave - 1) / (fcl_nw * job.tiles_per_wave));
                    fcl.lds = std::max(fcl.lds, (size_t)frontcl_lds_floats(K, lgD, fcl_nw) * 4);
                }
                else {
                    FCMLaunch& L = fcm[m_pf == 6 ? 0 : (m_pf == 10 ? 1 : 2)];
                    L.jobs.push_back(job);
                    L.max_blocks = std::max(L.max_blocks, (ntiles + 4 * job.tiles_per_wave - 1) / (4 * job.tiles_per_wave));
                    L.lds = std::max(L.lds, (size_t)frontcm_layout(K, lgD).total * 4);
                }
                g += (size_t)vt;
            }
            while (g < j) {
                const size_t left = j - g;
                int li = left >= 8 ? 0 : (left >= 4 ? 1 : (left >= 2 ? 2 : 3));
                if (ticking) { li = 3; }
                const int vt = vts[li];
                const std::string key = member_key('V', &s1[g], vt);
                float2* d_taps = nullptr;
                auto it = c->s1_tap_cache.find(key);
                if (it != c->s1_tap_cache.end()) { d_taps = it->second; }
                else {
                    const int K = (s1[g].K + 1) / 2;
                    std::vector<float2> host((size_t)K * vt + (size_t)256 * vt);
                    for (int k = 0; k < K; k++) {
                        for (int m = 0; m < vt; m++) { host[(size_t)k * vt + m] = s1[g + m].v->modtaps[(size_t)k]; }
                    }
// ... 306 lines not shown
            const int tile = threads * R;
            emit(c, level, fam, width == 2 ? TR_FIRB_C : (quad ? TR_FIRB_Q : (stereo ? TR_FIRB_S : TR_FIRB_R)), (max_nout + tile - 1) / tile, (int)jobs.size(), lds, d_jobs, nullptr, threads);
            return SDRPP_OK;
    }
    int launch_polyc(int level, int fam, std::vector<PolyJob>& jobs, PolyJob* d_jobs) {
            if (jobs.empty()) { return SDRPP_OK; }
            int cap2 = kMaxLds / (int)sizeof(float2);
            if (ticking) {
                int need = c->tick_lds_cap / (int)sizeof(float2);
                for (auto& jb : jobs) { need = std::max(need, jb.tpp + 2 * jb.decim + 1); }
                cap2 = std::min(cap2, need);
            }
            bool fits = true;
            int max_nout = 0, max_tiles = 0;
            for (auto& jb : jobs) {
                max_nout = std::max(max_nout, jb.nout);
                const int ct = std::min(64, (cap2 - jb.tpp - jb.decim) / jb.decim);
                if (ct < 1) { fits = false; continue; }
                const int ncyc = (jb.nout + jb.interp - 1) / jb.interp;
                max_tiles = std::max(max_tiles, (ncyc + ct - 1) / ct);
            }
            if (max_nout == 0) { return SDRPP_OK; }
            if (fits) {
                const int ppw = (long long)max_tiles * (long long)jobs.size() >= 64 ? 6 : 2;
                int G = 1;
                for (auto& jb : jobs) { G = std::max(G, ((jb.interp + 3) / 4 + ppw - 1) / ppw); }
                if (!ticking && (long long)max_tiles * (long long)jobs.size() >= 1024) { G = 1; }
                G = std::max(1, std::min(G, 128));
                emit(c, level, fam, TR_POLYC, max_tiles * G, (int)jobs.size(), (size_t)cap2 * sizeof(float2), d_jobs, nullptr, cap2 | ((G - 1) << 24));
                return SDRPP_OK;
            }
            size_t lds = 0;
            const int tile = 256;
            for (auto& jb : jobs) {
                const size_t ns = (size_t)((long long)tile * jb.decim / jb.interp) + jb.tpp + 4;
                lds = std::max(lds, ns * sizeof(float2));
            }
            if (lds > (size_t)kMaxLds) { return fail(c, SDRPP_ERR_UNSUPPORTED, "polyphase tile does not fit in LDS"); }
            if (c->tick_planning) { emit(c, level, fam, TR_POLY, (max_nout + tile - 1) / tile, (int)jobs.size(), lds, d_jobs); }
            else { launch(c, vfo_poly_kernel, dim3((max_nout + tile - 1) / tile, (unsigned)jobs.size()), dim3(tile), lds, (const PolyJob*)d_jobs); }
            return SDRPP_OK;
    }
    int launch_polyb(int li, std::vector<PolyBJob>& jobs, PolyBJob* d_jobs) {
            if (jobs.empty()) { return SDRPP_OK; }
            int max_cycles = 0, threads = 256;
            size_t lds = 0;
            auto lds_for = [&](const PolyBJob& jb, int nt) { return (size_t)jb.decim * (size_t)(nt + jb.rows / jb.decim + 2) * sizeof(float2); };
            for (auto& jb : jobs) {
                max_cycles = std::max(max_cycles, (jb.nout + jb.interp - 1) / jb.interp);
                int nt = 256;
                while (nt >= 32 && lds_for(jb, nt) > (size_t)kMaxLds) { nt >>= 1; }
                if (nt < 32) { return fail(c, SDRPP_ERR_UNSUPPORTED, "polyphase tile does not fit in LDS"); }
                threads = std::min(threads, nt);
            }
            if (max_cycles == 0) { return SDRPP_OK; }
            while (threads > 64 && (size_t)((max_cycles + threads - 1) / threads) * jobs.size() < 2048) { threads >>= 1; }
            for (auto& jb : jobs) { lds = std::max(lds, lds_for(jb, threads)); }
            const dim3 grid((max_cycles + threads - 1) / threads, (unsigned)jobs.size());
            if (li == 0) { launch(c, vfo_polyb_kernel<4, false>, grid, dim3(threads), lds, (const PolyBJob*)d_jobs); }
            else if (li == 1) { launch(c, vfo_polyb_kernel<8, false>, grid, dim3(threads), lds, (const PolyBJob*)d_jobs); }
            else if (li == 2) { launch(c, vfo_polyb_kernel<4, true>, grid, dim3(threads), lds, (const PolyBJob*)d_jobs); }
            else { launch(c, vfo_polyb_kernel<8, true>, grid, dim3(threads), lds, (const PolyBJob*)d_jobs); }
            return SDRPP_OK;
    }
    void emit_toep(int i, int l) {
            Lev<ToepJob>& L = *tlists[i].L;
            if (l >= L.top || L.at[l].empty() || tplan[i][l].grid_x == 0) { return; }
            emit(c, l, tlists[i].fam, tlists[i].role, tplan[i][l].grid_x, (int)L.at[l].size(), tplan[i][l].lds, L.dev[l]);
    }
    void launch_carry(int l) {
            std::vector<CarryJob>& cj = carry.at[l];
            if (cj.empty()) { return; }
            const bool has_iq = (l == (ticking ? L0 + 1 : carry_last));
            const int iq_elems = has_iq ? cj[0].need * cj[0].width : 0;
            int mx = 0;
            for (size_t k = has_iq ? 1 : 0; k < cj.size(); k++) { mx = std::max(mx, cj[k].need * cj[k].width); }
            auto per_vfo = [&](const CarryJob* dev, int njobs) {
                if (njobs <= 0) { return; }
                if (mx <= carry_wave_max) { emit(c, l, F_MISC, TR_CARRY, 1, (njobs + 3) / 4, 0, dev, nullptr, njobs); }
                else { emit(c, l, F_MISC, TR_CARRY, std::max(1, std::min((mx + 8191) / 8192, 64)), njobs, 0, dev); }
            };
            if (!ticking && iq_elems > carry_wave_max && iq_elems <= 128 * 1024 * 2 && cj.size() > 1) {
                emit(c, l, F_MISC, TR_CARRY, 32, (int)cj.size(), 0, carry.dev[l]);
            }
            else if (has_iq && (iq_elems > carry_wave_max || cj.size() == 1)) {
                emit(c, l, F_MISC, TR_CARRY, std::max(1, std::min((iq_elems + 8191) / 8192, 512)), 1, 0, carry.dev[l]);
                per_vfo(carry.dev[l] + 1, (int)cj.size() - 1);
            }
            else {
                mx = std::max(mx, iq_elems);
                per_vfo(carry.dev[l], (int)cj.size());
            }
    }

    int emit_levels() {
        int rc = SDRPP_OK;
        int top = std::max({ t_dec.top, t_poly.top, t_chan.top, t_audio.top, t_audio_fm.top, t_af_dec.top, t_af_poly.top, t_af_hpf.top, f_dec.top, poly.top,
                             polyb[0].top, polyb[1].top, polyb[2].top, polyb[3].top, chan.top, seq.top, pre.top, audio.top, audio_fm.top, af_dec.top, af_hpf.top,
                             af_poly.top, af_deemp.top, ssbx_l.top, carry.top, d_pipes ? pipe_lvl + 1 : 0 });
        for (int l = 1; l < top; l++) {
            {
                FamilyTimer t(c, F_DECIM);
                emit_toep(0, l);
                if (l < f_dec.top) {
                    rc = launch_fir(l, F_DECIM, f_dec.at[l], f_dec.dev[l], 2, false);
                    if (rc) { return rc; }
                }
            }
            if (d_pipes && l == pipe_lvl) {
                FamilyTimer t(c, F_PIPE);
                c->pipe_launched = true;
                emit(c, l, F_PIPE, TR_PIPE, pipe_seg, (int)pipes.size(), pipe_lds, d_pipes);
            }
            {
                FamilyTimer t(c, F_POLY);
                emit_toep(1, l);
                if (l < poly.top) {
                    rc = launch_polyc(l, F_POLY, poly.at[l], poly.dev[l]);
                    if (rc) { return rc; }
                }
                for (int li = 0; li < 4; li++) {
                    if (l < polyb[li].top) {
                        rc = launch_polyb(li, polyb[li].at[l], polyb[li].dev[l]);
                        if (rc) { return rc; }
                    }
                }
            }
            {
                FamilyTimer t(c, F_FIR);
                emit_toep(2, l);
                if (l < chan.top) {
                    rc = launch_fir(l, F_FIR, chan.at[l], chan.dev[l], 2, false);
                    if (rc) { return rc; }
                }
            }
            if ((l < pre.top && !pre.at[l].empty()) || (l < seq.top && !seq.at[l].empty()) || (l < ssbx_l.top && !ssbx_l.at[l].empty())) {
                FamilyTimer t(c, F_DEMOD);
                if (l < ssbx_l.top && !ssbx_l.at[l].empty()) {
                    const int nj = (int)ssbx_l.at[l].size();
                    if (c->tick_planning) { emit(c, l, F_DEMOD, TR_SSBX, (nj + 3) / 4, 1, 0, ssbx_l.dev[l], nullptr, nj); }
                    else { launch(c, vfo_ssb_rotate_exact_kernel, dim3((unsigned)nj), dim3(64), 0, (const SsbRotXJob*)ssbx_l.dev[l]); }
                }
                if (l < pre.top && !pre.at[l].empty()) {
                    int mx = 0;
                    for (auto& q : pre.at[l]) { mx = std::max(mx, q.n); }
                    if (mx > 0) { emit(c, l, F_DEMOD, TR_PRE, std::min((mx + 255) / 256, 1024), (int)pre.at[l].size(), 0, pre.dev[l]); }
                }
                if (l < seq.top && !seq.at[l].empty()) { emit(c, l, F_DEMOD, TR_SEQ, (int)seq.at[l].size(), 1, 0, seq.dev[l], nullptr, (int)seq.at[l].size()); }
            }
            {
                FamilyTimer t(c, F_FIR);
                emit_toep(3, l);
                emit_toep(4, l);
                if (l < audio.top) {
                    rc = launch_fir(l, F_FIR, audio.at[l], audio.dev[l], 1, true);
                    if (rc) { return rc; }
                }
                if (l < audio_fm.top) {
                    rc = launch_fir(l, F_FIR, audio_fm.at[l], audio_fm.dev[l], 1, true, true);
                    if (rc) { return rc; }
                }
            }
            if (l < std::max({ t_af_dec.top, t_af_poly.top, t_af_hpf.top, af_dec.top, af_hpf.top, af_poly.top, af_deemp.top })) {
                FamilyTimer t(c, F_AF);
                emit_toep(5, l);
                if (l < af_dec.top) {
                    rc = launch_fir(l, F_AF, af_dec.at[l], af_dec.dev[l], 2, false);
                    if (rc) { return rc; }
                }
                emit_toep(6, l);
                if (l < af_poly.top) {
                    rc = launch_polyc(l, F_AF, af_poly.at[l], af_poly.dev[l]);
                    if (rc) { return rc; }
                }
                emit_toep(7, l);
                if (l < af_hpf.top) {
                    rc = launch_fir(l, F_AF, af_hpf.at[l], af_hpf.dev[l], 2, false);
                    if (rc) { return rc; }
                }
                if (l < af_deemp.top && !af_deemp.at[l].empty()) {
                    int max_seg = 0;
                    for (auto& jb : af_deemp.at[l]) { max_seg = std::max(max_seg, jb.nseg); }
                    if (max_seg > 0) {
                        emit(c, l, F_AF, TR_DEEMP_P0, max_seg, (int)af_deemp.at[l].size(), 3 * 256 * sizeof(float), af_deemp.dev[l]);
                        emit(c, l + 1, F_AF, TR_DEEMP_P1, max_seg, (int)af_deemp.at[l].size(), 3 * 256 * sizeof(float), af_deemp.dev[l]);
                    }
                }
            }
            if (l < carry.top && !carry.at[l].empty()) {
                FamilyTimer t(c, F_MISC);
                launch_carry(l);
            }
        }
        return SDRPP_OK;
    }
};

int do_vfos_plan(sdrpp_ctx* c, const IqSrc& src, int64_t count, const CarryJob& iq_carry) {
    if (c->vfos.empty()) { return SDRPP_OK; }
#ifdef SDRPP_TOEP_KNOCK
    {
        static bool once = false;
        if (!once) {
            once = true;
            const int m = getenv("SDRPP_TOEP_KNOCK") ? atoi(getenv("SDRPP_TOEP_KNOCK")) : 0;
            (void)hipMemcpyToSymbol(HIP_SYMBOL(sdrpp_k::g_toep_knock), &m, sizeof(int));
        }
    }
#endif
    HostScope hs_all("plan: vfo bank");
    if (!c->bank_plan) {
        c->bank_plan = new BankPlan(c);
        c->bank_plan_free = [](void* q) { delete static_cast<BankPlan*>(q); };
    }
    BankPlan* P = static_cast<BankPlan*>(c->bank_plan);
    P->begin(src, count, iq_carry);
    int rc = SDRPP_OK;
    {
        HostScope hs("plan: chains");
        for (size_t i = 0; i < c->vfo_list.size(); i++) {
            rc = P->chain(*c->vfo_list[i]);
            if (rc) { return rc; }
        }
    }
    {
        HostScope hs("plan: group_front");
        rc = P->group_front();
    }
    if (!rc) {
        HostScope hs("plan: upload");
        rc = P->upload();
    }
    if (!rc) {
        HostScope hs("plan: emit");
        rc = P->emit_front();
        if (!rc) { rc = P->emit_levels(); }
    }
    if (rc) { return rc; }
    for (size_t i = 0; i < c->vfo_list.size(); i++) {
        for (auto& s : c->vfo_list[i]->st) {
            if (s.hist_len > 0 && s.data) { s.cur ^= 1; }
        }
    }
    return SDRPP_OK;
}

}
```

sdrplusplus_amd/csrc/sdrpp_gpu.hip:

```cpp
#include <hip/hip_runtime.h>
#include <hip/hip_ext.h>

#include <algorithm>
#include <chrono>
#include <atomic>
#include <cmath>
#include <cstdarg>
#include <cstdio>
#include <cstring>
#include <deque>
#include <map>
#include <memory>
#include <mutex>
#include <string>
#include <thread>
#include <vector>

#include "../../include/sdrpp_gpu.h"
#include "fft_kernels.h"
#include "host_design.h"
#include "vfo_kernels.h"
#include "pipe_kernels.h"
#include "tick_kernels.h"

// ... 732 lines not shown
        }
    }
    const bool has_poly = (d->interp != d->decim);
    if (has_poly && (d->interp <= 0 || d->decim <= 0 || d->resamp_ntaps <= 0 || !d->resamp_taps)) { return fail(c, SDRPP_ERR_INVALID, "bad polyphase description"); }
    if (d->chan_ntaps < 0 || d->chan_ntaps > kChanHistCap + 1) { return fail(c, SDRPP_ERR_UNSUPPORTED, "channel filter of %d taps (max %d)", d->chan_ntaps, kChanHistCap + 1); }
    if (d->demod < SDRPP_DEMOD_RAW || d->demod > SDRPP_DEMOD_DSB) { return fail(c, SDRPP_ERR_INVALID, "demod %d", d->demod); }
    HIPCHK(c, hipStreamSynchronize(c->stream));
    struct VfoFreer {
        void operator()(Vfo* p) const {
            if (p) {
                vfo_free(*p);
                delete p;
            }
        }
    };
    std::unique_ptr<Vfo, VfoFreer> v(new Vfo);
    v->id = c->next_id++;
    v->d = *d;
    if (d->nco_mode < 0 || d->nco_mode > 2) { return fail(c, SDRPP_ERR_INVALID, "nco_mode %d: 0 (context), 1 (closed form) or 2 (reference rotator)", d->nco_mode); }
    v->nco_exact = d->nco_mode == 0 ? (c->nco_exact != 0) : (d->nco_mode == 2);
    int rc;
    size_t cap = (size_t)c->max_push;
    auto add_stream = [&](int width, int hist, size_t capn) -> int {
        v->st.emplace_back();
        int r = stream_alloc(c, v->st.back(), width, hist, capn);
        return r ? -1 : (int)v->st.size() - 1;
    };
    const int tpp = has_poly ? (d->resamp_ntaps + d->interp - 1) / d->interp : 0;
    const bool fm = (d->demod == SDRPP_DEMOD_WFM || d->demod == SDRPP_DEMOD_NFM);
    const bool fm_mode = (d->demod == SDRPP_DEMOD_WFM || d->demod == SDRPP_DEMOD_NFM);
    const int if_hist = fm_mode ? std::max(d->audio_ntaps, 1) + 1 : 1;
    const int chan_hist = ((std::max(std::max(d->chan_ntaps - 1, 1), if_hist) + 63) / 64) * 64;
    auto hist_after_decim = [&]() -> int {
        if (has_poly) { return tpp - 1; }
        return chan_hist;
    };
    for (int s = 0; s < d->n_stages; s++) {
        v->staps[s].assign(d->stage_taps[s], d->stage_taps[s] + d->stage_ntaps[s]);
        v->d.stage_taps[s] = nullptr;
        rc = upload_blocked(c, &v->d_staps[s], v->staps[s].data(), (int)v->staps[s].size(), d->stage_decim[s], &v->s_kp[s]);
        if (rc) { return rc; }
        rc = upload(c, &v->d_staps_nat[s], v->staps[s].data(), v->staps[s].size());
        if (rc) { return rc; }
        if (s >= 1 || v->nco_exact) {
            rc = toep_build_fir(c, v->tp_stage[s], v->staps[s].data(), (int)v->staps[s].size(), d->stage_decim[s]);
            if (rc) { return rc; }
        }
        cap = cap / (size_t)d->stage_decim[s] + 2;
        const int hist = (s + 1 < d->n_stages) ? d->stage_ntaps[s + 1] - 1 : hist_after_decim();
        if (add_stream(2, hist, cap) < 0) { return SDRPP_ERR_NOMEM; }
    }
    if (d->n_stages == 0) {
        if (add_stream(2, hist_after_decim(), cap) < 0) { return SDRPP_ERR_NOMEM; }
    }
    v->i_first = 0;
    {
        unsigned long long hsh = 1469598103934665603ull;
        for (int s = 0; s < std::min(d->n_stages, 2); s++) {
            for (float t : v->staps[s]) {
                unsigned u;
                memcpy(&u, &t, 4);
                hsh = (hsh ^ u) * 1099511628211ull;
            }
        }
        v->tap_hash = hsh;
        if (d->n_stages >= 2) {
            const std::vector<float>& h2 = v->staps[1];
            for (size_t k = 0; k < h2.size() / 2; k++) { v->no_fuse = v->no_fuse || (h2[k] != h2[h2.size() - 1 - k]); }
        }
        v->fused_front = !v->nco_exact && !v->no_fuse && d->n_stages >= 2 && front2_t2(d->stage_ntaps[0], d->stage_decim[0], d->stage_ntaps[1], d->stage_decim[1], 8) > 0;
        if (d->n_stages >= 1 && !v->nco_exact) {
            const int K0 = d->stage_ntaps[0], D1 = d->stage_decim[0], K2 = v->fused_front ? d->stage_ntaps[1] : 1;
            const int K = K0 + (K2 - 1) * D1;
            std::vector<double> h12((size_t)K, 0.0);
            for (int k2 = 0; k2 < K2; k2++) {
                const double w2 = v->fused_front ? (double)v->staps[1][(size_t)k2] : 1.0;
                for (int k1 = 0; k1 < K0; k1++) { h12[(size_t)k2 * D1 + k1] += w2 * (double)v->staps[0][(size_t)k1]; }
            }
            std::vector<float> hf(h12.begin(), h12.end());
            rc = upload(c, &v->d_h12, hf.data(), hf.size());
            if (rc) { return rc; }
            v->h12_K = K;
            v->h12_lgD = ilog2(D1) + (v->fused_front ? ilog2(d->stage_decim[1]) : 0);
        }
        if (v->nco_exact && d->n_stages >= 1) {
            v->i_rot = add_stream(2, d->stage_ntaps[0] - 1, (size_t)c->max_push);
            if (v->i_rot < 0) { return SDRPP_ERR_NOMEM; }
        }
    }
    if (has_poly) {
        v->rtaps.assign(d->resamp_taps, d->resamp_taps + d->resamp_ntaps);
        v->d.resamp_taps = nullptr;
        v->tpp = tpp;
        std::vector<float> bank((size_t)d->interp * tpp, 0.0f);
        const int tot = d->interp * tpp;
        for (int i = 0; i < tot; i++) { bank[(size_t)((d->interp - 1) - (i % d->interp)) * tpp + (size_t)(i / d->interp)] = (i < d->resamp_ntaps) ? v->rtaps[(size_t)i] : 0.0f; }
        rc = upload(c, &v->d_bank, bank.data(), bank.size());
        if (rc) { return rc; }
        rc = toep_build_poly(c, v->tp_poly, bank, d->interp, d->decim, tpp);
        if (rc) { return rc; }
        if (d->interp <= 8) {
            const int L = d->interp, M = d->decim, lmax = (L <= 4) ? 4 : 8, rows = tpp + M;
            std::vector<float> cyc((size_t)L * rows * lmax, 0.0f);
            for (int ph0 = 0; ph0 < L; ph0++) {
                for (int r = 0; r < L; r++) {
                    const int A = ph0 + r * M, ph = A % L, o = A / L;
                    for (int k = 0; k < tpp; k++) { cyc[((size_t)ph0 * rows + (size_t)(k + o)) * lmax + r] = bank[(size_t)ph * tpp + k]; }
                }
            }
            rc = upload(c, &v->d_cyc, cyc.data(), cyc.size());
            if (rc) { return rc; }
            v->cyc_rows = rows;
            v->cyc_lmax = lmax;
        }
        cap = cap * (size_t)d->interp / (size_t)d->decim + 4;
        v->i_poly = add_stream(2, chan_hist, cap);
        if (v->i_poly < 0) { return SDRPP_ERR_NOMEM; }
    }
    v->i_chan = add_stream(2, if_hist, cap);
    if (v->i_chan < 0) { return SDRPP_ERR_NOMEM; }
    if (d->chan_ntaps > 0) {
        if (!d->chan_taps) { return fail(c, SDRPP_ERR_INVALID, "chan_taps null"); }
        v->ctaps_chan.assign(d->chan_taps, d->chan_taps + d->chan_ntaps);
        rc = upload_blocked(c, &v->d_chan, v->ctaps_chan.data(), (int)v->ctaps_chan.size(), 1, &v->chan_kp);
        if (rc) { return rc; }
        rc = toep_build_fir(c, v->tp_chan, v->ctaps_chan.data(), (int)v->ctaps_chan.size(), 1);
        if (rc) { return rc; }
        v->chan_ntaps = d->chan_ntaps;
    }
    v->d.chan_taps = nullptr;
    if (d->demod != SDRPP_DEMOD_RAW) {
        if (fm || d->demod == SDRPP_DEMOD_AM) {
            static const float unit = 1.0f;
            const float* at = d->audio_ntaps > 0 ? d->audio_taps : &unit;
            const int an = d->audio_ntaps > 0 ? d->audio_ntaps : 1;
            if (d->audio_ntaps > 0 && !d->audio_taps) { return fail(c, SDRPP_ERR_INVALID, "audio_taps null"); }
            v->ataps.assign(at, at + an);
            v->audio_ntaps = an;
            rc = upload_blocked(c, &v->d_audio, v->ataps.data(), (int)v->ataps.size(), 1, &v->audio_kp);
            if (rc) { return rc; }
            rc = toep_build_fir(c, v->tp_audio, v->ataps.data(), (int)v->ataps.size(), 1);
            if (rc) { return rc; }
            if (!fm) {
                v->i_dem = add_stream(1, std::max(an - 1, 1), cap);
                if (v->i_dem < 0) { return SDRPP_ERR_NOMEM; }
            }
        }
        if (d->demod >= SDRPP_DEMOD_USB) {
            v->i_dem = add_stream(1, 0, cap);
            if (v->i_dem < 0) { return SDRPP_ERR_NOMEM; }
        }
        v->i_out = add_stream(2, 0, cap);
        if (v->i_out < 0) { return SDRPP_ERR_NOMEM; }
    }
    v->d.audio_taps = nullptr;
    rc = dev_alloc(c, &v->d_state, 2 * sizeof(AgcState) + sizeof(float));
    if (rc) { return rc; }
    rc = dev_alloc(c, &v->d_rot, 2);
    if (rc) { return rc; }
    v->theta = sdrpp_host::turnsPerSample(d->phase_delta_re, d->phase_delta_im);
    v->theta2 = sdrpp_host::turnsPerSample(d->ssb_phase_delta_re, d->ssb_phase_delta_im);
    if (d->demod < SDRPP_DEMOD_USB) { v->theta2 = 0.0; }
    v->modtaps_dirty = true;
    rc = vfo_reset_state(c, *v);
    if (rc) { return rc; }
    const int vid = v->id;
    *id = vid;
    c->vfos[vid] = std::unique_ptr<Vfo>(v.release());
    vfo_list_rebuild(c);
    return SDRPP_OK;
}

int sdrpp_vfo_remove(sdrpp_ctx* c, int id) {
    DeviceScope dev_scope_(c);
    if (!c) { return SDRPP_ERR_INVALID; }
    FLUSH_PENDING(c);
    auto it = c->vfos.find(id);
    if (it == c->vfos.end()) { return fail(c, SDRPP_ERR_NOT_FOUND, "no VFO %d", id); }
    HIPCHK(c, hipStreamSynchronize(c->stream));
    vfo_free(*it->second);
    c->vfos.erase(it);
    vfo_list_rebuild(c);
    return SDRPP_OK;
}

int sdrpp_vfo_count(sdrpp_ctx* c) { return c ? (int)c->vfos.size() : SDRPP_ERR_INVALID; }

static int hist_tail_copy(sdrpp_ctx* c, Stream& to, const Stream& from, int max_samples) {
    if (!to.hist[to.cur] || !from.hist[from.cur] || to.width != from.width) { return SDRPP_OK; }
    const int H = std::min(std::min(from.hist_len, to.hist_len), max_samples);
    if (H <= 0) { return SDRPP_OK; }
    const size_t w = (size_t)to.width;
    HIPCHK(c, hipMemcpy(to.hist[to.cur] + (size_t)(to.hist_len - H) * w, from.hist[from.cur] + (size_t)(from.hist_len - H) * w, (size_t)H * w * sizeof(float), hipMemcpyDeviceToDevice));
    return SDRPP_OK;
}
int sdrpp_vfo_replace(sdrpp_ctx* c, int old_id, const sdrpp_vfo_desc* d, int keep, int* new_id) {
    DeviceScope dev_scope_(c);
    if (!c || !d || !new_id || keep < 0 || keep > 3) { return SDRPP_ERR_INVALID; }
    FLUSH_PENDING(c);
    if (c->vfos.find(old_id) == c->vfos.end()) { return fail(c, SDRPP_ERR_NOT_FOUND, "no VFO %d", old_id); }
    int nid = 0;
    int rc = sdrpp_vfo_add(c, d, &nid);
    if (rc) { return rc; }
    HIPCHK(c, hipStreamSynchronize(c->stream));
    Vfo& o = *c->vfos[old_id];
    Vfo& n = *c->vfos[nid];
    auto feed_idx = [](const Vfo& v) { return (v.i_poly >= 0) ? v.i_poly : v.i_first + std::max(v.d.n_stages, 1) - 1; };
    Stream& of = o.st[(size_t)feed_idx(o)];
    Stream& nf = n.st[(size_t)feed_idx(n)];
    if (keep & 1) {
        if (o.nco_exact == n.nco_exact) {
            n.phi = o.phi;
            if (o.d_rot && n.d_rot) { HIPCHK(c, hipMemcpy(n.d_rot, o.d_rot, sizeof(float2), hipMemcpyDeviceToDevice)); }
        }
        const int w = of.width;
        std::vector<float> line;
        if (o.chan_ntaps > 1 && of.hist[of.cur] && of.hist_len >= o.chan_ntaps - 1) {
            line.resize((size_t)(o.chan_ntaps - 1) * (size_t)w);
            HIPCHK(c, hipMemcpy(line.data(), of.hist[of.cur] + (size_t)(of.hist_len - (o.chan_ntaps - 1)) * w, line.size() * sizeof(float), hipMemcpyDeviceToHost));
        }
        else if (o.chan_ntaps == 0) { line = o.chan_stale; }
        if (n.chan_ntaps > 0 && nf.width == w) {
            if (nf.hist[nf.cur]) {
                HIPCHK(c, hipMemset(nf.hist[nf.cur], 0, (size_t)nf.hist_len * (size_t)w * sizeof(float)));
                const int have = (int)(line.size() / (size_t)w), m = std::min(have, std::min(n.chan_ntaps - 1, nf.hist_len));
                if (m > 0) { HIPCHK(c, hipMemcpy(nf.hist[nf.cur] + (size_t)(nf.hist_len - m) * w, line.data() + (size_t)(have - m) * w, (size_t)m * w * sizeof(float), hipMemcpyHostToDevice)); }
            }
        }
        else if (n.chan_ntaps == 0) { n.chan_stale = line; }
    }
    if ((keep & 2) && o.d.demod == n.d.demod) {
        Stream& oif = (o.chan_ntaps > 0 && o.i_chan >= 0) ? o.st[(size_t)o.i_chan] : of;
        Stream& nif = (n.chan_ntaps > 0 && n.i_chan >= 0) ? n.st[(size_t)n.i_chan] : nf;
        const int if_need = (n.d.demod == SDRPP_DEMOD_WFM || n.d.demod == SDRPP_DEMOD_NFM) ? std::max(n.audio_ntaps, 1) + 1 : 1;
        rc = hist_tail_copy(c, nif, oif, if_need);
        if (rc) { return rc; }
        if (o.i_dem >= 0 && n.i_dem >= 0) {
            rc = hist_tail_copy(c, n.st[(size_t)n.i_dem], o.st[(size_t)o.i_dem], 1 << 30);
            if (rc) { return rc; }
        }
        if (o.d_state && n.d_state) { HIPCHK(c, hipMemcpy(n.d_state, o.d_state, 2 * sizeof(AgcState) + sizeof(float), hipMemcpyDeviceToDevice)); }
        n.phi2 = o.phi2;
        if (o.d_rot && n.d_rot) { HIPCHK(c, hipMemcpy(n.d_rot + 1, o.d_rot + 1, sizeof(float2), hipMemcpyDeviceToDevice)); }
    }
    rc = sdrpp_vfo_remove(c, old_id);
    if (rc) { return rc; }
    *new_id = nid;
    return SDRPP_OK;
}

int sdrpp_vfo_set_phase_delta(sdrpp_ctx* c, int id, float re, float im) {
    DeviceScope dev_scope_(c);
    if (!c) { return SDRPP_ERR_INVALID; }
    FLUSH_PENDING(c);
    auto it = c->vfos.find(id);
    if (it == c->vfos.end()) { return fail(c, SDRPP_ERR_NOT_FOUND, "no VFO %d", id); }
    Vfo& v = *it->second;
    const double th = sdrpp_host::turnsPerSample(re, im);
    if (!v.nco_exact && v.d.n_stages > 0 && th != v.theta) {
        if (!v.recs.empty() && v.recs.back().pos == v.seen) {  }
        else { v.recs.push_back(Vfo::Retune{ v.seen, v.theta }); }
    }
    v.d.phase_delta_re = re;
    v.d.phase_delta_im = im;
    v.theta = th;
    v.modtaps_dirty = true;
    return SDRPP_OK;
}

int sdrpp_vfo_set_channel_taps(sdrpp_ctx* c, int id, const float* taps, int n) {
    DeviceScope dev_scope_(c);
    if (!c || n < 0 || n > kChanHistCap + 1 || (n > 0 && !taps)) { return SDRPP_ERR_INVALID; }
    FLUSH_PENDING(c);
    auto it = c->vfos.find(id);
    if (it == c->vfos.end()) { return fail(c, SDRPP_ERR_NOT_FOUND, "no VFO %d", id); }
    Vfo& v = *it->second;
    HIPCHK(c, hipStreamSynchronize(c->stream));
    {
        const int idx = (v.i_poly >= 0) ? v.i_poly : v.i_first + std::max(v.d.n_stages, 1) - 1;
        Stream& fs = v.st[(size_t)idx];
        const int old_n = v.chan_ntaps, w = fs.width;
        const bool was_on = old_n > 0, now_on = n > 0;
        if (was_on != now_on && v.i_chan >= 0) {
            Stream& cs = v.st[(size_t)v.i_chan];
            if (was_on) {
                v.chan_stale.assign((size_t)std::max(old_n - 1, 0) * (size_t)w, 0.0f);
                if (old_n > 1 && fs.hist[fs.cur] && fs.hist_len >= old_n - 1) {
                    HIPCHK(c, hipMemcpy(v.chan_stale.data(), fs.hist[fs.cur] + (size_t)(fs.hist_len - (old_n - 1)) * w, v.chan_stale.size() * sizeof(float), hipMemcpyDeviceToHost));
                }
            }
            if (now_on) {
                int rc = stream_grow_hist(c, fs, n - 1);
                if (rc) { return rc; }
            }
            Stream& from = was_on ? cs : fs;
            Stream& to = was_on ? fs : cs;
            const int H = std::min(from.hist_len, to.hist_len);
            if (H > 0 && from.hist[from.cur] && to.hist[to.cur] && from.width == to.width) {
                HIPCHK(c, hipMemcpy(to.hist[to.cur] + (size_t)(to.hist_len - H) * w, from.hist[from.cur] + (size_t)(from.hist_len - H) * w, (size_t)H * w * sizeof(float), hipMemcpyDeviceToDevice));
            }
            if (now_on && fs.hist[fs.cur]) {
                HIPCHK(c, hipMemset(fs.hist[fs.cur], 0, (size_t)fs.hist_len * (size_t)w * sizeof(float)));
                const int have = (int)(v.chan_stale.size() / (size_t)w), m = std::min(have, std::min(n - 1, fs.hist_len));
                if (m > 0) {
                    HIPCHK(c, hipMemcpy(fs.hist[fs.cur] + (size_t)(fs.hist_len - m) * w, v.chan_stale.data() + (size_t)(have - m) * w, (size_t)m * w * sizeof(float), hipMemcpyHostToDevice));
                }
            }
        }
        else {
            int rc = stream_grow_hist(c, fs, n - 1);
            if (rc) { return rc; }
            const int keep = std::max(old_n - 1, 0);
            if (n > old_n && fs.hist_len > keep && fs.hist[fs.cur]) {
                HIPCHK(c, hipMemset(fs.hist[fs.cur], 0, (size_t)(fs.hist_len - keep) * (size_t)w * sizeof(float)));
            }
        }
    }
    v.ctaps_chan.assign(taps, taps + n);
    v.chan_ntaps = n;
    v.d.chan_ntaps = n;
    if (n > 0) {
        int rc = upload_blocked(c, &v.d_chan, v.ctaps_chan.data(), n, 1, &v.chan_kp);
        if (rc) { return rc; }
        rc = toep_build_fir(c, v.tp_chan, v.ctaps_chan.data(), n, 1);
        if (rc) { return rc; }
    }
    return SDRPP_OK;
}

static void af_detach(Vfo& v) {
    Vfo::Af& a = v.af;
    for (int i = 0; i < SDRPP_MAX_DECIM_STAGES; i++) {
        dev_free(a.d_staps[i]);
        toep_free(a.tp_stage[i]);
    }
    toep_free(a.tp_poly);
    toep_free(a.tp_hpf);
    dev_free(a.d_bank);
    dev_free(a.d_hpf);
    dev_free(a.d_last);
    dev_free(a.d_seg);
    if (a.base >= 0) {
        for (size_t i = (size_t)a.base; i < v.st.size(); i++) { stream_free(v.st[i]); }
        v.st.resize((size_t)a.base);
    }
    a = Vfo::Af{};
}

int sdrpp_vfo_set_af(sdrpp_ctx* c, int id, const sdrpp_af_desc* af) {
    DeviceScope dev_scope_(c);
    if (!c) { return SDRPP_ERR_INVALID; }
    FLUSH_PENDING(c);
    auto it = c->vfos.find(id);
    if (it == c->vfos.end()) { return fail(c, SDRPP_ERR_NOT_FOUND, "no VFO %d", id); }
    Vfo& v = *it->second;
    HIPCHK(c, hipStreamSynchronize(c->stream));
    af_detach(v);
    if (!af) { return SDRPP_OK; }
    if (v.d.demod == SDRPP_DEMOD_RAW || v.i_out < 0) { return fail(c, SDRPP_ERR_UNSUPPORTED, "the AF chain needs a demodulating VFO"); }
    if (af->n_stages < 0 || af->n_stages > SDRPP_MAX_DECIM_STAGES) { return fail(c, SDRPP_ERR_INVALID, "af n_stages %d", af->n_stages); }
    for (int s = 0; s < af->n_stages; s++) {
        if (!is_pow2(af->stage_decim[s]) || af->stage_ntaps[s] <= 0 || !af->stage_taps[s]) { return fail(c, SDRPP_ERR_UNSUPPORTED, "af stage %d: decimation must be a power of two with taps", s); }
    }
    const bool has_poly = af->interp != af->decim;
    if (has_poly && (af->interp <= 0 || af->decim <= 0 || af->resamp_ntaps <= 0 || !af->resamp_taps)) { return fail(c, SDRPP_ERR_INVALID, "bad af polyphase description"); }
    if (af->hpf_ntaps < 0 || af->hpf_ntaps > kChanHistCap + 1 || (af->hpf_ntaps > 0 && !af->hpf_taps)) { return fail(c, SDRPP_ERR_INVALID, "bad af high-pass description"); }
    Vfo::Af& a = v.af;
    a.base = (int)v.st.size();
    a.n_stages = af->n_stages;
    a.interp = has_poly ? af->interp : 1;
    a.decim = has_poly ? af->decim : 1;
    a.tpp = has_poly ? (af->resamp_ntaps + af->interp - 1) / af->interp : 0;
    a.alpha = af->deemph_alpha;
    int rc;
    auto need_of = [&](int stage) -> int {
        if (stage < a.n_stages) { return af->stage_ntaps[stage] - 1; }
        if (stage <= a.n_stages && has_poly) { return a.tpp - 1; }
        if (stage <= a.n_stages + 1 && af->hpf_ntaps > 0) { return af->hpf_ntaps - 1; }
        return 0;
    };
    rc = stream_grow_hist(c, v.st[(size_t)v.i_out], need_of(0));
    if (rc) { return rc; }
    size_t cap = v.st[(size_t)v.i_out].cap;
    auto add_stream = [&](int hist, size_t capn) -> int {
        v.st.emplace_back();
        int r = stream_alloc(c, v.st.back(), 2, hist, capn);
        return r ? -1 : (int)v.st.size() - 1;
    };
    for (int s = 0; s < a.n_stages; s++) {
        a.decim_s[s] = af->stage_decim[s];
        a.staps[s].assign(af->stage_taps[s], af->stage_taps[s] + af->stage_ntaps[s]);
        rc = upload_blocked(c, &a.d_staps[s], a.staps[s].data(), (int)a.staps[s].size(), a.decim_s[s], &a.s_kp[s]);
        if (rc) { return rc; }
        rc = toep_build_fir(c, a.tp_stage[s], a.staps[s].data(), (int)a.staps[s].size(), a.decim_s[s]);
        if (rc) { return rc; }
        cap = cap / (size_t)a.decim_s[s] + 2;
        const int idx = add_stream(need_of(s + 1), cap);
        if (idx < 0) { return SDRPP_ERR_NOMEM; }
        if (s == 0) { a.i_stage0 = idx; }
    }
    if (has_poly) {
        a.rtaps.assign(af->resamp_taps, af->resamp_taps + af->resamp_ntaps);
        std::vector<float> bank((size_t)a.interp * a.tpp, 0.0f);
        const int tot = a.interp * a.tpp;
        for (int i = 0; i < tot; i++) { bank[(size_t)((a.interp - 1) - (i % a.interp)) * a.tpp + (size_t)(i / a.interp)] = (i < af->resamp_ntaps) ? a.rtaps[(size_t)i] : 0.0f; }
        rc = upload(c, &a.d_bank, bank.data(), bank.size());
        if (rc) { return rc; }
        rc = toep_build_poly(c, a.tp_poly, bank, a.interp, a.decim, a.tpp);
        if (rc) { return rc; }
        cap = cap * (size_t)a.interp / (size_t)a.decim + 4;
        a.i_poly = add_stream(need_of(a.n_stages + 1), cap);
        if (a.i_poly < 0) { return SDRPP_ERR_NOMEM; }
    }
    if (af->hpf_ntaps > 0) {
        a.htaps.assign(af->hpf_taps, af->hpf_taps + af->hpf_ntaps);
        rc = upload_blocked(c, &a.d_hpf, a.htaps.data(), (int)a.htaps.size(), 1, &a.hpf_kp);
        if (rc) { return rc; }
        rc = toep_build_fir(c, a.tp_hpf, a.htaps.data(), (int)a.htaps.size(), 1);
        if (rc) { return rc; }
        a.i_hpf = add_stream(0, cap);
        if (a.i_hpf < 0) { return SDRPP_ERR_NOMEM; }
    }
    if (a.alpha != 0.0f) {
        rc = dev_alloc(c, &a.d_last, 2);
        if (rc) { return rc; }
        HIPCHK(c, hipMemset(a.d_last, 0, 2 * sizeof(float2)));
        a.state_cur = 0;
        a.seg_cap = (int)(cap / SDRPP_DEEMP_SEG) + 2;
        rc = dev_alloc(c, &a.d_seg, 2 * ((size_t)a.seg_cap + 1));
        if (rc) { return rc; }
// ... 601 lines not shown
    c->stage_open = -1;
    c->pipelined = on != 0;
    c->res_flags = on ? result_flags : 0;
    return SDRPP_OK;
}
int sdrpp_set_pipeline_group(sdrpp_ctx* c, int max_blocks, int adaptive) {
    DeviceScope dev_scope_(c);
    if (!c || max_blocks < 1 || max_blocks > kGroupMax) { return c ? fail(c, SDRPP_ERR_INVALID, "sdrpp_set_pipeline_group: 1 .. %d blocks per launch", kGroupMax) : SDRPP_ERR_INVALID; }
    if (c->pipelined) {
        int rc = tick_group_launch(c);
        if (rc) { return rc; }
    }
    c->group_max = max_blocks;
    c->group_adaptive = (adaptive & 1) != 0;
    c->stage_pend_stable = (adaptive & 2) != 0;
    return SDRPP_OK;
}
int sdrpp_pipeline_launch_held(sdrpp_ctx* c) {
    DeviceScope dev_scope_(c);
    if (!c) { return SDRPP_ERR_INVALID; }
    return c->pipelined ? tick_group_launch(c) : SDRPP_OK;
}
int sdrpp_pipeline_group_stats(sdrpp_ctx* c, int64_t* out, int max) {
    if (!c || !out || max < 0) { return SDRPP_ERR_INVALID; }
    const int64_t v[5] = { (int64_t)c->groups, c->stat_groups, c->stat_group_blocks, c->stat_group_max, (int64_t)c->held.ends.size() };
    int n = 0;
    for (; n < 5 && n < max; n++) { out[n] = v[n]; }
    return n;
}
uint64_t sdrpp_ticket(sdrpp_ctx* c) { return c ? c->pushes : 0; }
int sdrpp_pipeline_flush(sdrpp_ctx* c) {
    DeviceScope dev_scope_(c);
    if (!c) { return SDRPP_ERR_INVALID; }
    if (!c->pipelined) { return SDRPP_OK; }
    int rc = tick_group_launch(c);
    return rc ? rc : tick_drain(c);
}
static bool ticket_is_held_back(const sdrpp_ctx* c, uint64_t ticket) {
    return c->held.kind >= 0 && !c->held.ends.empty() && ticket <= c->pushes && ticket + c->held.ends.size() > c->pushes;
}
static sdrpp_ctx::Result* result_of(sdrpp_ctx* c, uint64_t ticket) {
    if (!c || ticket == 0 || ticket > c->pushes) { return nullptr; }
    sdrpp_ctx::Result& R = c->res[ticket % kResMeta];
    if (R.ticket != ticket) { return nullptr; }
    if (R.held) { return &R; }
    return (R.epoch == c->res_epoch && tick_results_region(c, R.group)) ? &R : nullptr;
}
int sdrpp_result_ready(sdrpp_ctx* c, uint64_t ticket) {
    if (c && ticket_is_held_back(c, ticket)) { return 0; }
    sdrpp_ctx::Result* R = result_of(c, ticket);
    if (!R) { return c ? fail(c, SDRPP_ERR_NOT_FOUND, "no results for block %llu (not gathered, overwritten, or processed as an ordinary pass)", (unsigned long long)ticket) : SDRPP_ERR_INVALID; }
    if (R->done_tick > c->ticks) { return 0; }
    DeviceScope dev_scope_(c);
    return tick_results_visible(c, R->done_tick, false);
}
int sdrpp_result_wait(sdrpp_ctx* c, uint64_t ticket, sdrpp_result* out) {
    DeviceScope dev_scope_(c);
    if (!c || !out) { return SDRPP_ERR_INVALID; }
    if (ticket_is_held_back(c, ticket)) {
        int rc = tick_group_launch(c);
        if (rc) { return rc; }
    }
    sdrpp_ctx::Result* R = result_of(c, ticket);
    if (!R) { return fail(c, SDRPP_ERR_NOT_FOUND, "no results for block %llu (not gathered, overwritten, or processed as an ordinary pass)", (unsigned long long)ticket); }
    while (R->done_tick > c->ticks) {
        int rc = tick_group_launch(c);
        if (!rc && R->done_tick <= c->ticks) { break; }
        if (!rc) { rc = arena_begin(c); }
        if (!rc) { rc = tick_launch(c, nullptr); }
        if (rc) { return rc; }
        if (c->tickq.empty() && R->done_tick > c->ticks) { return fail(c, SDRPP_ERR_HIP, "internal: block %llu cannot complete", (unsigned long long)ticket); }
    }
    {
        const int vis = tick_results_visible(c, R->done_tick, true);
        if (vis < 0) { return vis; }
    }
    if (!tick_is_done(c, R->done_tick)) { return fail(c, SDRPP_ERR_HIP, "tick %llu did not complete", (unsigned long long)R->done_tick); }
    if (!R->held) {
        sdrpp_ctx::ResRegion* g = tick_results_region(c, R->group);
        if (!g) { return fail(c, SDRPP_ERR_NOT_FOUND, "no results for block %llu (overwritten)", (unsigned long long)ticket); }
        R->held = true;
        g->held++;
    }
    const char* base = R->base;
    out->ticket = ticket;
    out->n_vfo = (int)R->ids.size();
    out->ids = R->ids.data();
    out->offsets = R->offsets.data();
    out->counts = R->counts.data();
    out->samples = reinterpret_cast<const float*>(base);
    out->n_lines = R->n_lines;
    out->fft_size = R->fft_size;
    out->data_width = R->data_width;
    const bool zo = R->n_lines > 0 && (R->flags & 2) && R->data_width > 0;
    out->zoomed = zo ? reinterpret_cast<const float*>(base + R->off_zoomed) : nullptr;
    out->index = zo ? reinterpret_cast<const int32_t*>(base + R->off_index) : nullptr;
    out->raw = (R->n_lines > 0 && (R->flags & 4)) ? reinterpret_cast<const float*>(base + R->off_raw) : nullptr;
    out->n_iq = R->n_iq;
    out->iq = R->n_iq > 0 ? reinterpret_cast<const float*>(base + R->off_iq) : nullptr;
    return SDRPP_OK;
}
int sdrpp_result_release(sdrpp_ctx* c, uint64_t ticket) {
    if (!c || ticket == 0 || ticket > c->pushes) { return c ? SDRPP_ERR_NOT_FOUND : SDRPP_ERR_INVALID; }
    sdrpp_ctx::Result& R = c->res[ticket % kResMeta];
    if (R.ticket != ticket) { return SDRPP_ERR_NOT_FOUND; }
    if (R.held) {
        if (sdrpp_ctx::ResRegion* g = tick_results_region(c, R.group)) {
            if (g->held > 0) { g->held--; }
        }
        if (R.epoch != c->res_epoch) {
            for (size_t i = 0; i < c->res_retired.size(); i++) {
                if (c->res_retired[i].epoch == R.epoch && --c->res_retired[i].held <= 0) {
                    DeviceScope dev_scope_(c);
                    (void)hipHostFree(c->res_retired[i].ring);
                    c->res_retired.erase(c->res_retired.begin() + (long)i);
                    break;
                }
            }
        }
    }
    R.held = false;
    R.ticket = 0;
    return SDRPP_OK;
}

int sdrpp_result_take_lines(sdrpp_ctx* c, uint64_t ticket, float* zoomed_dst, int32_t* index_dst, int max_lines, int* n_lines) {
    sdrpp_result r{};
    int rc = sdrpp_result_wait(c, ticket, &r);
    if (rc) { return rc; }
    if (n_lines) { *n_lines = r.n_lines; }
    if (r.n_lines > max_lines) {
        (void)sdrpp_result_release(c, ticket);
        return fail(c, SDRPP_ERR_INVALID, "block %llu completed %d lines, room for %d", (unsigned long long)ticket, r.n_lines, max_lines);
    }
    if (r.n_lines > 0 && r.zoomed) {
        const size_t bytes = (size_t)r.n_lines * (size_t)r.data_width * 4;
        if (zoomed_dst) { memcpy(zoomed_dst, r.zoomed, bytes); }
        if (index_dst) { memcpy(index_dst, r.index, bytes); }
    }
    return sdrpp_result_release(c, ticket);
}
int sdrpp_pipeline_stats(sdrpp_ctx* c, int64_t* out, int max) {
    if (!c || !out || max < 0) { return SDRPP_ERR_INVALID; }
    const int64_t head[SDRPP_PIPELINE_STATS_HEAD] = { (int64_t)c->ticks, c->stat_tick_blocks, c->stat_pass_blocks, c->stat_crowded, c->stat_last_depth, (int64_t)TR_COUNT, 0, c->stat_last_table_bytes };
    int n = 0;
    for (; n < SDRPP_PIPELINE_STATS_HEAD && n < max; n++) { out[n] = head[n]; }
    for (int r = 0; r < TR_COUNT && n < max; r++, n++) { out[n] = c->stat_role_wgs[r]; }
    return n;
}
const char* sdrpp_pipeline_role_name(int role) {
    static const char* const names[] = { "none", "copy", "carry", "rot", "fcm_132_4", "fcm_6", "fcm_10", "fcm_16", "fcm16_132_4", "fcl_0", "fcl_pf", "toep_c", "toep_r", "toep_q",
                                         "firb_c", "firb_r", "firb_s", "firb_q", "pre", "seq", "fft_s10", "fft_s11", "fft_s12", "fft_p1_5", "fft_p1_6", "fft_p1_7", "fft_p1_8", "fft_p1_9",
                                         "fft_p1_10", "fft_p2_7", "fft_p2_8", "fft_p2_9", "fft_p2_10", "fft_p2row", "fft_tr", "zoom_16", "zoom_4", "zoom_1", "polyc", "deemp_p0", "deemp_p1",
                                         "dc_p0", "dc_p1", "wf_ring", "wf_trace", "pipe", "rotx16", "fird", "ssbx", "s1_1", "s1d_1", "f2_1", "poly" };
    static_assert(sizeof(names) / sizeof(names[0]) == TR_COUNT, "role names out of step with TickRole");
    return (role >= 0 && role < TR_COUNT) ? names[role] : nullptr;
}

int sdrpp_timing_enable(sdrpp_ctx* c, int on) {
    DeviceScope dev_scope_(c);
    if (!c) { return SDRPP_ERR_INVALID; }
    timing_flush(c);
    c->timing = on != 0;
    c->timing_mask = (on > 1) ? (unsigned)(on >> 1) : 0xffffffffu;
    for (int i = 0; i < SDRPP_NUM_KERNEL_FAMILIES; i++) {
        c->fam_ms[i] = 0.0;
        c->fam_launch[i] = 0;
    }
    return SDRPP_OK;
}

int sdrpp_timing_read(sdrpp_ctx* c, double* ms, int64_t* launches) {
    DeviceScope dev_scope_(c);
    if (!c) { return SDRPP_ERR_INVALID; }
    timing_flush(c);
    for (int i = 0; i < SDRPP_NUM_KERNEL_FAMILIES; i++) {
        if (ms) { ms[i] = c->fam_ms[i]; }
        if (launches) { launches[i] = c->fam_launch[i]; }
    }
    return SDRPP_OK;
}

}
```

sdrplusplus_amd/csrc/tick_host.h:

```cpp
#pragma once

namespace {

void tick_wait_done(sdrpp_ctx* c, uint64_t nticks) {
    if (!c->h_tick_flag) { return; }
    const volatile unsigned* f = c->h_tick_flag;
    long spins = 0;
    while ((int)((unsigned)nticks - *f) > 0) {
        if (++spins > 2000) { std::this_thread::yield(); }
        if (spins > 40000000) {
            (void)hipStreamSynchronize(c->stream);
            if ((int)((unsigned)nticks - *f) > 0) { return; }
        }
    }
}
hipEvent_t tick_event_take(sdrpp_ctx* c, uint64_t behind_tick) {
    const int k = c->tick_ev_next;
    c->tick_ev_next = (k + 1) % sdrpp_ctx::kTickEvents;
    tick_ev_resolve(c, k);
    if (!c->tick_ev[k] && hipEventCreate(&c->tick_ev[k]) != hipSuccess) { return nullptr; }
    c->tick_ev_tick[k] = behind_tick;
    c->tick_ev_last = behind_tick;
    return c->tick_ev[k];
}
int tick_results_visible(sdrpp_ctx* c, uint64_t nticks, bool wait) {
    if (nticks == 0) { return 1; }
    if (wait) { tick_wait_done(c, nticks); }
    else if (c->h_tick_flag && (int)((unsigned)nticks - *(const volatile unsigned*)c->h_tick_flag) > 0) { return 0; }
    int best = -1;
    for (int k = 0; k < sdrpp_ctx::kTickEvents; k++) {
        if (c->tick_ev[k] && c->tick_ev_tick[k] >= nticks && (best < 0 || c->tick_ev_tick[k] < c->tick_ev_tick[best])) { best = k; }
    }
    hipEvent_t ev = best >= 0 ? c->tick_ev[best] : nullptr;
    if (!ev) {
        ev = tick_event_take(c, c->ticks);
        if (!ev || hipEventRecord(ev, c->stream) != hipSuccess) { return fail(c, SDRPP_ERR_HIP, "hipEventRecord failed"); }
    }
    long spins = 0;
    for (;;) {
        const hipError_t e = hipEventQuery(ev);
        if (e == hipSuccess) { return 1; }
        if (e != hipErrorNotReady) { return fail(c, SDRPP_ERR_HIP, "hipEventQuery: %s", hipGetErrorString(e)); }
        if (!wait) { return 0; }
        if (++spins > 200) { std::this_thread::yield(); }
    }
}
bool tick_is_done(const sdrpp_ctx* c, uint64_t nticks) { return !c->h_tick_flag || (int)((unsigned)nticks - *(const volatile unsigned*)c->h_tick_flag) <= 0; }

inline int tick_role_weight(int role, bool crowded) {
    if (role == TR_ROTX16) { return 120; }
    if (role == TR_COPY) { return 110; }
    if (role >= TR_FFT_P1_5 && role <= TR_FFT_P1_10) { return crowded ? 45 : 70; }
    switch (role) {
    case TR_FCL_0: case TR_FCL_PF: return 72;
    case TR_FCM_132_4: case TR_FCM_6: case TR_FCM_10: case TR_FCM_16: case TR_FCM16_132_4: case TR_S1_1: case TR_S1D_1: case TR_F2_1: return 90;
    case TR_SEQ: case TR_SSBX: return 85;
    case TR_FIRB_C: case TR_FIRB_R: case TR_FIRB_S: case TR_FIRB_Q: return 70;
    case TR_POLYC: return 55;
    case TR_DEEMP_P1: case TR_DC_P1: return 52;
    case TR_DEEMP_P0: case TR_DC_P0: return 48;
    case TR_TOEP_Q: return 65;
    case TR_TOEP_C: case TR_TOEP_R: case TR_FFT_S10: case TR_FFT_S11: case TR_FFT_S12: return 60;
    case TR_FFT_P2_7: case TR_FFT_P2_8: case TR_FFT_P2_9: case TR_FFT_P2_10: case TR_FFT_P2ROW: return 50;
    case TR_FFT_TR: return 25;
    case TR_ROT: case TR_PRE: return 30;
    case TR_ZOOM_16: case TR_ZOOM_4: case TR_ZOOM_1: return 20;
    default: return 10;
    }
}
int tick_launch(sdrpp_ctx* c, const CopyJob* land) {
    std::vector<sdrpp_ctx::RoleLaunch> now;
    if (!c->tickq.empty()) {
        now.swap(c->tickq.front());
        c->tickq.pop_front();
    }
    if ((int)now.size() != c->next_tab_n) { return fail(c, SDRPP_ERR_HIP, "internal: tick table out of step (%zu roles queued, %d uploaded)", now.size(), c->next_tab_n); }
    TickTable* tab_dev_next = nullptr;
    int tab_n_next = 0;
    if (!c->tickq.empty() && !c->tickq.front().empty()) {
        std::vector<sdrpp_ctx::RoleLaunch>& nx = c->tickq.front();
        long long wgs = 0;
        for (auto& r : nx) { wgs += (long long)r.e.gx * r.e.gy; }
        const bool crowded = wgs > 3ll * c->num_cus;
        std::stable_sort(nx.begin(), nx.end(), [crowded](const sdrpp_ctx::RoleLaunch& a, const sdrpp_ctx::RoleLaunch& b) { return tick_role_weight(a.e.role, crowded) > tick_role_weight(b.e.role, crowded); });
        if (nx.size() > SDRPP_TICK_MAX_ENTRIES) { return fail(c, SDRPP_ERR_UNSUPPORTED, "internal: %zu roles in one tick", nx.size()); }
        const size_t off = (c->arena_off + 63) & ~(size_t)63;
        if (off + sizeof(TickTable) > kArenaBytes) { return fail(c, SDRPP_ERR_UNSUPPORTED, "job arena exhausted"); }
        TickTable* T = reinterpret_cast<TickTable*>(c->arena_host[c->arena_slot] + off);
        T->n = (int)nx.size();
        int total = 0;
        for (size_t i = 0; i < nx.size(); i++) {
            total += nx[i].e.gx * nx[i].e.gy;
            T->block_end[i] = total;
            T->e[i] = nx[i].e;
        }
        c->arena_off = off + offsetof(TickTable, e) + nx.size() * sizeof(TickEntry);
        tab_dev_next = reinterpret_cast<TickTable*>(c->arena_dev + off);
        tab_n_next = (int)nx.size();
    }
    TickL0 l0{};
    if (land && land->bytes > 0) {
        l0.job[0] = *land;
        l0.blocks[0] = (int)std::max<long long>(1, std::min<long long>((land->bytes + 8191) / 8192, c->tick_land_blocks));
    }
    if (c->arena_off > 0) {
        l0.job[1] = CopyJob{ c->arena_host_dev[c->arena_slot], c->arena_dev, (long long)((c->arena_off + 15) & ~(size_t)15), 0, 0 };
        l0.blocks[1] = (int)std::max<size_t>(1, std::min<size_t>((c->arena_off + 4095) / 4096, 16));
    }
    int blocks = l0.blocks[0] + l0.blocks[1];
    size_t lds = 0;
    bool set1 = false;
    long long role_wgs = 0;
    bool to_host = false;
    for (auto& r : now) {
        to_host = to_host || r.to_host;
        blocks += r.e.gx * r.e.gy;
        role_wgs += (long long)r.e.gx * r.e.gy;
        lds = std::max(lds, r.lds);
        set1 = set1 || r.e.role == TR_FCL_PF || r.e.role == TR_FCM_6 || r.e.role == TR_FCM_10 || r.e.role == TR_FCM_16;
        if (r.e.role >= 0 && r.e.role < 64) { c->stat_role_wgs[r.e.role] += (int64_t)r.e.gx * r.e.gy; }
    }
    if (role_wgs > 3ll * c->num_cus) { c->stat_crowded++; }
    {
        const int l0_at = c->tick_l0_at;
        const int role_blocks = blocks - l0.blocks[0] - l0.blocks[1];
        l0.first = l0_at < 0 ? role_blocks : std::min(l0_at, role_blocks);
    }
    if (blocks == 0) {
        c->next_tab = tab_dev_next;
        c->next_tab_n = tab_n_next;
        for (auto& R : c->res) {
            if (R.ticket != 0 && R.done_tick > c->ticks) { R.done_tick--; }
        }
        return SDRPP_OK;
    }
    c->tick_target += (unsigned)blocks;
    c->ticks++;
    TickDone done{ c->d_tick_counter, c->hd_tick_flag, c->tick_target, (unsigned)c->ticks };
    hipEvent_t stop_ev = nullptr;
    const TickTable* tab = c->next_tab_n > 0 ? c->next_tab : c->empty_tab;
    {
        const bool timed = c->timing && ((c->timing_mask >> F_TICK) & 1u);
        c->fam_launch[F_TICK]++;
        hipEvent_t ea = nullptr;
        if (timed || to_host) {
            const int k = c->tick_ev_next;
            stop_ev = tick_event_take(c, c->ticks);
            if (!stop_ev) { return fail(c, SDRPP_ERR_HIP, "hipEventCreate failed"); }
            if (timed) {
                ea = get_event(c);
                c->tick_ev_start[k] = ea;
            }
        }
        HostScope hs("launch");
        if (stop_ev) {
            if (set1) { hipExtLaunchKernelGGL((tick_kernel<1>), dim3((unsigned)blocks), dim3(256), (unsigned)lds, c->stream, ea, stop_ev, 0, l0, tab, done); }
            else { hipExtLaunchKernelGGL((tick_kernel<0>), dim3((unsigned)blocks), dim3(256), (unsigned)lds, c->stream, ea, stop_ev, 0, l0, tab, done); }
        }
        else if (set1) { hipLaunchKernelGGL((tick_kernel<1>), dim3((unsigned)blocks), dim3(256), lds, c->stream, l0, tab, done); }
        else { hipLaunchKernelGGL((tick_kernel<0>), dim3((unsigned)blocks), dim3(256), lds, c->stream, l0, tab, done); }
    }
    c->arena_tick[c->arena_slot] = c->ticks;
    c->next_tab = tab_dev_next;
    c->next_tab_n = tab_n_next;
    hipError_t e = hipGetLastError();
    if (e != hipSuccess) { return fail(c, SDRPP_ERR_HIP, "tick launch failed: %s", hipGetErrorString(e)); }
    return SDRPP_OK;
}
int tick_drain(sdrpp_ctx* c) {
    while (!c->tickq.empty()) {
        int rc = arena_begin(c);
        if (rc) { return rc; }
        rc = tick_launch(c, nullptr);
        if (rc) { return rc; }
    }
    return SDRPP_OK;
}

bool tick_eligible(sdrpp_ctx* c) {
    if ((c->pre.on && c->pre.ref_order) || c->deferred) { return false; }
    for (auto& kv : c->vfos) {
        const Vfo& v = *kv.second;
        if ((v.nco_exact && c->rot_exact_single) || !v.recs.empty() || v.st.size() > 24) { return false; }
    }
    return true;
}

const Stream& result_stream(const Vfo& v, int* level = nullptr) {
    if (v.af.on && v.af.i_last >= 0 && v.d.demod != SDRPP_DEMOD_RAW) {
        if (level) { *level = v.lvl_af; }
        return v.st[(size_t)v.af.i_last];
    }
    const bool raw = v.d.demod == SDRPP_DEMOD_RAW;
    if (level) { *level = raw ? v.lvl_if : v.lvl_out; }
    return raw ? v.st[(size_t)v.i_if] : v.st[(size_t)v.i_out];
}
size_t tick_results_need(sdrpp_ctx* c) {
    size_t need = 0;
    if (c->res_flags & 1) {
        for (auto& kv : c->vfos) {
            const Vfo& v = *kv.second;
            size_t cap = std::max(result_stream(v).cap, v.st[(size_t)v.i_if].cap);
            if (v.i_out >= 0) { cap = std::max(cap, v.st[(size_t)v.i_out].cap); }
            need += ((cap + 16) * 8 + 15) & ~(size_t)15;
        }
    }
    if ((c->res_flags & 8) && c->pre.on) {
        size_t cap = c->pre.out.base ? c->pre.out.cap : 0;
        for (auto& st : c->pre.st) { cap = std::max(cap, st.cap); }
        need += ((cap + 16) * 8 + 15) & ~(size_t)15;
    }
    if (c->fft_on) {
        if ((c->res_flags & 2) && c->data_width > 0) { need += 2 * ((c->lines_cap * (size_t)c->data_width * 4 + 15) & ~(size_t)15); }
        if (c->res_flags & 4) { need += (c->lines_cap * (size_t)c->fft_size * 4 + 15) & ~(size_t)15; }
// ... 463 lines not shown
```

sdrplusplus_amd/csrc/tick_kernels.h:

```cpp
#pragma once
#include <cstddef>

namespace sdrpp_k {

struct CopyJob {
    const void* src;
    void* dst;
    long long bytes;
    int kind;
    int pad;
};
__device__ __forceinline__ void copy_one(const CopyJob& job, int bx, int gx) {
    const long long tid = (long long)bx * 256 + threadIdx.x, nth = (long long)gx * 256;
    if ((job.kind & 0xff) == 1) {
        const short* in = reinterpret_cast<const short*>(job.src);
        float* out = reinterpret_cast<float*>(job.dst);
        const float inv = 1.0f / 32768.0f;
        const long long n = job.bytes / 2;
        for (long long i = tid; i < n; i += nth) { out[i] = ((float)in[i]) * inv; }
    }
    else if ((job.kind & 0xff) == 2) {
        const float2* in = reinterpret_cast<const float2*>(job.src);
        float2* out = reinterpret_cast<float2*>(job.dst);
        const long long n = job.bytes / 8;
        for (long long i = tid; i < n; i += nth) {
            const float2 x = in[i];
            out[i] = make_float2(x.x, -x.y);
        }
    }
    else {
        const bool al16 = ((((unsigned long long)job.src) | ((unsigned long long)job.dst)) & 15ull) == 0ull;
        long long done = 0;
        if (al16) {
            const long long n16 = job.bytes / 16;
            constexpr int U = 8;
            long long i = tid;
            for (; i + (U - 1) * nth < n16; i += U * nth) {
                uint4 v[U];
#pragma unroll
                for (int u = 0; u < U; u++) { v[u] = global_load_u32x4(job.src, i + u * nth); }
#pragma unroll
                for (int u = 0; u < U; u++) { global_store_u32x4(job.dst, i + u * nth, v[u]); }
            }
            for (; i < n16; i += nth) { global_store_u32x4(job.dst, i, global_load_u32x4(job.src, i)); }
            done = n16 * 4;
        }
        const long long n4 = job.bytes / 4;
        for (long long i = done + tid; i < n4; i += nth) { global_store_u32(job.dst, i, global_load_u32(job.src, i)); }
    }
}
__device__ __forceinline__ void copy_body(const KIdx bid, const KIdx gdim, const CopyJob* __restrict__ jobs) { copy_one(jobs[bid.y], bid.x, gdim.x); }
__global__ __launch_bounds__(256) void copy_kernel(const CopyJob* __restrict__ jobs) { copy_body(kidx(blockIdx), kidx(gridDim), jobs); }

enum TickRole : int {
    TR_NONE = 0,
    TR_COPY,
    TR_CARRY,
    TR_ROT,
    TR_FCM_132_4,
    TR_FCM_6,
    TR_FCM_10,
    TR_FCM_16,
    TR_FCM16_132_4,
    TR_FCL_0,
    TR_FCL_PF,
    TR_TOEP_C,
    TR_TOEP_R,
    TR_TOEP_Q,
    TR_FIRB_C,
    TR_FIRB_R,
    TR_FIRB_S,
    TR_FIRB_Q,
    TR_PRE,
    TR_SEQ,
    TR_FFT_S10, TR_FFT_S11, TR_FFT_S12,
    TR_FFT_P1_5, TR_FFT_P1_6, TR_FFT_P1_7, TR_FFT_P1_8, TR_FFT_P1_9, TR_FFT_P1_10,
    TR_FFT_P2_7, TR_FFT_P2_8, TR_FFT_P2_9, TR_FFT_P2_10,
    TR_FFT_P2ROW, TR_FFT_TR,
    TR_ZOOM_16, TR_ZOOM_4, TR_ZOOM_1,
    TR_POLYC,
    TR_DEEMP_P0, TR_DEEMP_P1,
    TR_DC_P0, TR_DC_P1,
    TR_WF_RING, TR_WF_TRACE,
    TR_PIPE,
    TR_ROTX16,
    TR_FIRD,
    TR_SSBX,
    TR_S1_1,
    TR_S1D_1,
    TR_F2_1,
    TR_POLY,
    TR_COUNT
};
struct TickP1 { IqSrc src; FrameGeom g; const float* window; const float2* tw1; const float2* twn; float2* scratch; int lg2, ntiles; };
struct TickP2 { const float2* scratch; const float2* tw2; float* out; float* grp; int lg1, ntiles; };
struct TickFS { IqSrc src; FrameGeom g; const float* window; const float2* tw; float* out; };
struct TickZoom { const float* lines; const int32_t* zs; const int32_t* zc; float* zoomed; int32_t* index; const float* grp; int fft_size, data_width, gsz; float wf_min, wf_max; int pad; };
struct TickWf { const float* src; float* a; float* b; float* c; int n0, n1, n2, n3; float f0, f1, f2, pad; };
struct TickEntry {
    int role, gx, gy, aux;
    const void* jobs;
    union {
        IqSrc src;
        TickP1 p1;
        TickP2 p2;
        TickFS fs;
        TickZoom z;
        TickWf wf;
    } p;
};
#define SDRPP_TICK_MAX_ENTRIES 64
struct TickTable {
    int n, pad[3];
    int block_end[SDRPP_TICK_MAX_ENTRIES];
    TickEntry e[SDRPP_TICK_MAX_ENTRIES];
};
struct TickL0 {
    CopyJob job[2];
    int blocks[2];
    int first;
    int pad;
};
struct TickDone {
    unsigned* counter;
    unsigned* host_flag;
    unsigned target;
    unsigned value;
};
__device__ __forceinline__ void tick_finish(const TickDone& d) {
    wave_stores_done();
    __syncthreads();
    if (threadIdx.x == 0) {
        const unsigned old = atomicAdd(d.counter, 1u);
        if (old + 1u == d.target) {
            __threadfence_system();
            *reinterpret_cast<volatile unsigned*>(d.host_flag) = d.value;
        }
    }
}

__host__ __device__ inline size_t tick_lds_fft_single(int lg, int fpw) { return ((size_t)(1 << lg) / 2 + (size_t)fpw * ((1 << lg) + (1 << lg) / 16)) * 8; }
__host__ __device__ inline size_t tick_lds_fft_p1(int lg1, int c) { return ((size_t)(1 << lg1) / 2 + (size_t)(1 << lg1) * c) * 8; }
__host__ __device__ inline size_t tick_lds_fft_p2(int lg2, int r) { return ((size_t)(1 << lg2) / 2 + (size_t)r * ((1 << lg2) + (1 << lg2) / 16)) * 8; }
__host__ __device__ inline size_t tick_lds_zoom(int tp) { return (size_t)(256 / tp) * (tp + 1) * 4; }

template <int LG, int FPW>
__device__ __forceinline__ void tick_fft_single(const KIdx bid, float* smem, const TickFS& q) {
    const IqSrc src = q.src;
    const FrameGeom g = q.g;
    float2* tw = reinterpret_cast<float2*>(smem);
    fft_single_body<LG, FPW>(bid, tw, tw + FftSingleLds<LG, FPW>::TW, src, g, q.window, q.tw, q.out);
}
template <int LG1, int C>
__device__ __forceinline__ void tick_fft_p1(const KIdx bid, const KIdx gdim, float* smem, const TickP1& q) {
    static_assert(((1 << LG1) / 16) * C == 256, "tick roles run in 256-thread workgroups");
    const IqSrc src = q.src;
    const FrameGeom g = q.g;
    float2* tw = reinterpret_cast<float2*>(smem);
    fft_pass1_body<LG1, C>(bid, tw, tw + (1 << LG1) / 2, src, g, q.window, q.tw1, q.twn, q.scratch, q.lg2, q.ntiles, gdim.x);
}
template <int LG2, int R>
__device__ __forceinline__ void tick_fft_p2(const KIdx bid, const KIdx gdim, float* smem, const TickP2& q) {
    static_assert(((1 << LG2) / 16) * R == 256, "tick roles run in 256-thread workgroups");
    float2* tw = reinterpret_cast<float2*>(smem);
    fft_pass2_body<LG2, R>(bid, tw, tw + (1 << LG2) / 2, q.scratch, q.tw2, q.out, q.lg1, q.ntiles, q.grp, gdim.x);
}
template <int TP>
__device__ __forceinline__ void tick_zoom(const KIdx bid, float* smem, const TickZoom& q, int groups) {
    for (int i = 0; i < groups; i++) {
        if (i > 0) { __syncthreads(); }
        zoom_palette_body<TP>(KIdx{ bid.x * groups + i, bid.y }, smem, q.lines, q.fft_size, q.data_width, q.zs, q.zc, q.wf_min, q.wf_max, q.zoomed, q.index, q.grp, q.gsz);
    }
}

#ifdef SDRPP_TICK_TRACE
struct TickTraceRec { unsigned tick; short role, entry; int block; unsigned long long t0, t1; unsigned hwid, xcc; unsigned long long m[4]; };
#define SDRPP_TICK_TRACE_CAP (1 << 20)
__device__ TickTraceRec g_tick_trace[SDRPP_TICK_TRACE_CAP];
__device__ unsigned g_tick_trace_n;
#endif

template <int SET>
__global__ __launch_bounds__(256, SET == 1 ? 2 : 3) void tick_kernel(TickL0 l0, const TickTable* __restrict__ tab, TickDone done) {
    HIP_DYNAMIC_SHARED(float, smem)
    int b = (int)blockIdx.x;
    const int nb0 = l0.blocks[0] + l0.blocks[1];
    const bool is_l0 = b >= l0.first && b < l0.first + nb0;
    if (is_l0) { b -= l0.first; }
    else if (b >= l0.first + nb0) { b -= nb0; }
#ifdef SDRPP_TICK_TRACE
    const unsigned long long tr_t0 = (unsigned long long)wall_clock64();
    int tr_role = -1, tr_entry = -1;
#endif
    if (is_l0) {
        if (b < l0.blocks[0]) { copy_one(l0.job[0], b, l0.blocks[0]); }
        else { copy_one(l0.job[1], b - l0.blocks[0], l0.blocks[1]); }
    }
    else {
        const int n = tab->n;
        int first = 0;
        static_assert(offsetof(TickEntry, jobs) == 16 && sizeof(void*) == 8, "wave_upper_bound64_rec hands out the first six dwords of an entry");
        int hdr[6];
        const int ei = wave_upper_bound64_rec(tab->block_end, n, b, &first, tab->e, (int)sizeof(TickEntry), hdr);
        if (ei < n) {
            const TickEntry& e = tab->e[ei];
            const int e_role = hdr[0], e_gy = hdr[2], e_aux = hdr[3];
            const void* e_jobs = reinterpret_cast<const void*>(((unsigned long long)(unsigned)hdr[5] << 32) | (unsigned long long)(unsigned)hdr[4]);
#ifdef SDRPP_TICK_TRACE
            tr_role = e_role;
            tr_entry = ei;
#endif
            const int lb = b - first, gx = hdr[1];
            const KIdx bid{ lb % gx, lb / gx }, gdim{ gx, e_gy };
            switch (e_role) {
            case TR_COPY: copy_body(bid, gdim, reinterpret_cast<const CopyJob*>(e_jobs)); break;
            case TR_CARRY: carry_body(bid, gdim, reinterpret_cast<const CarryJob*>(e_jobs), e_aux); break;
            case TR_ROTX16: {
                const IqSrc src = e.p.src;
                const RotXHead h = *reinterpret_cast<const RotXHead*>(e_jobs);
                vfo_rotate_exact4_body<16>(bid.x, reinterpret_cast<float2*>(smem), src, h.jobs, h.njobs, h.bounds, h.nb, h.vpw);
            } break;
            case TR_FIRD: vfo_fir_direct_body<false>(bid, gdim, reinterpret_cast<const FirBJob*>(e_jobs)); break;
            case TR_POLY: vfo_poly_body(bid, reinterpret_cast<float2*>(smem), reinterpret_cast<const PolyJob*>(e_jobs)); break;
            case TR_S1_1: { const IqSrc src = e.p.src; vfo_stage1_body<1>(bid, reinterpret_cast<float2*>(smem), e_aux, 256, src, reinterpret_cast<const Stage1Job*>(e_jobs)); } break;
            case TR_S1D_1: { const IqSrc src = e.p.src; vfo_stage1_direct_body<1>(bid, src, reinterpret_cast<const Stage1Job*>(e_jobs)); } break;
            case TR_F2_1: { const IqSrc src = e.p.src; vfo_front2_body<1, 0, 0>(bid, reinterpret_cast<float2*>(smem), src, reinterpret_cast<const Front2Job*>(e_jobs)); } break;
            case TR_SSBX: {
                const int j = bid.x * 4 + ((int)threadIdx.x >> 6);
                if (j < e_aux) { vfo_ssb_rotate_exact_body(j, reinterpret_cast<const SsbRotXJob*>(e_jobs)); }
            } break;
            case TR_ROT: { const IqSrc src = e.p.src; vfo_rotate_body(bid, gdim, src, reinterpret_cast<const RotJob*>(e_jobs)); } break;
            case TR_FCM_132_4: { const IqSrc src = e.p.src; vfo_frontcm_body<10, 132, 4>(bid, smem, src, reinterpret_cast<const FrontCMJob*>(e_jobs)); } break;
            case TR_FCM_6:
                if constexpr (SET == 1) { const IqSrc src = e.p.src; vfo_frontcm_body<6, 0, 0>(bid, smem, src, reinterpret_cast<const FrontCMJob*>(e_jobs)); }
                break;
            case TR_FCM_10:
                if constexpr (SET == 1) { const IqSrc src = e.p.src; vfo_frontcm_body<10, 0, 0>(bid, smem, src, reinterpret_cast<const FrontCMJob*>(e_jobs)); }
                break;
            case TR_FCM_16:
                if constexpr (SET == 1) { const IqSrc src = e.p.src; vfo_frontcm_body<16, 0, 0>(bid, smem, src, reinterpret_cast<const FrontCMJob*>(e_jobs)); }
                break;
            case TR_FCM16_132_4: { const IqSrc src = e.p.src; vfo_frontcm16_body<132, 4>(bid, smem, src, reinterpret_cast<const FrontCMJob*>(e_jobs)); } break;
            case TR_FCL_0: { const IqSrc src = e.p.src; vfo_frontcl_body<0>(bid, smem, src, reinterpret_cast<const FrontCMJob*>(e_jobs), e_aux == 4 ? 4 : 2); } break;
            case TR_FCL_PF:
                if constexpr (SET == 1) { const IqSrc src = e.p.src; vfo_frontcl_body<SDRPP_FCL_PF>(bid, smem, src, reinterpret_cast<const FrontCMJob*>(e_jobs), e_aux == 4 ? 4 : 2); }
                break;
            case TR_TOEP_C: vfo_toep_body<2, 2, false>(bid, gdim, smem, reinterpret_cast<const ToepJob*>(e_jobs)); break;
            case TR_TOEP_R: vfo_toep_body<1, 2, false>(bid, gdim, smem, reinterpret_cast<const ToepJob*>(e_jobs)); break;
            case TR_TOEP_Q: vfo_toep_body<1, 2, true>(bid, gdim, smem, reinterpret_cast<const ToepJob*>(e_jobs)); break;
            case TR_FIRB_C:
                vfo_firb_body<2, false>(bid, smem, e_aux, reinterpret_cast<const FirBJob*>(e_jobs));
                break;
            case TR_FIRB_R:
                vfo_firb_body<1, false>(bid, smem, e_aux, reinterpret_cast<const FirBJob*>(e_jobs));
                break;
            case TR_FIRB_S:
                vfo_firb_body<1, true>(bid, smem, e_aux, reinterpret_cast<const FirBJob*>(e_jobs));
                break;
            case TR_FIRB_Q:
                vfo_firb_body<1, true, true>(bid, smem, e_aux, reinterpret_cast<const FirBJob*>(e_jobs));
                break;
            case TR_PRE: vfo_demod_pre_body(bid, gdim, reinterpret_cast<const PreJob*>(e_jobs)); break;
            case TR_SEQ:
                if (threadIdx.x < 64) { vfo_sequential_body(bid, reinterpret_cast<const SeqJob*>(e_jobs), e_aux); }
                break;
            case TR_FFT_S10: tick_fft_single<10, 4>(bid, smem, e.p.fs); break;
            case TR_FFT_S11: tick_fft_single<11, 2>(bid, smem, e.p.fs); break;
            case TR_FFT_S12: tick_fft_single<12, 1>(bid, smem, e.p.fs); break;
            case TR_FFT_P1_5: tick_fft_p1<5, 128>(bid, gdim, smem, e.p.p1); break;
            case TR_FFT_P1_6: tick_fft_p1<6, 64>(bid, gdim, smem, e.p.p1); break;
            case TR_FFT_P1_7: tick_fft_p1<7, 32>(bid, gdim, smem, e.p.p1); break;
            case TR_FFT_P1_8: tick_fft_p1<8, 16>(bid, gdim, smem, e.p.p1); break;
            case TR_FFT_P1_9: tick_fft_p1<9, 8>(bid, gdim, smem, e.p.p1); break;
            case TR_FFT_P1_10: tick_fft_p1<10, 4>(bid, gdim, smem, e.p.p1); break;
            case TR_FFT_P2_7: tick_fft_p2<7, 32>(bid, gdim, smem, e.p.p2); break;
            case TR_FFT_P2_8: tick_fft_p2<8, 16>(bid, gdim, smem, e.p.p2); break;
            case TR_FFT_P2_9: tick_fft_p2<9, 8>(bid, gdim, smem, e.p.p2); break;
            case TR_FFT_P2_10: tick_fft_p2<10, 4>(bid, gdim, smem, e.p.p2); break;
            case TR_FFT_P2ROW: {
                float2* tw = reinterpret_cast<float2*>(smem);
                fft_pass2row_body<12>(bid, tw, tw + (1 << 12) / 2, const_cast<float2*>(e.p.p2.scratch), e.p.p2.tw2, e.p.p2.lg1);
            } break;
            case TR_FFT_TR: fft_transpose_body(bid, smem, reinterpret_cast<const float*>(e.p.p2.scratch), e.p.p2.out, e.p.p2.grp, e.p.p2.lg1, 12, e_aux); break;
            case TR_ZOOM_16: tick_zoom<16>(bid, smem, e.p.z, e_aux > 0 ? e_aux : 1); break;
            case TR_ZOOM_4: tick_zoom<4>(bid, smem, e.p.z, e_aux > 0 ? e_aux : 1); break;
            case TR_ZOOM_1: tick_zoom<1>(bid, smem, e.p.z, e_aux > 0 ? e_aux : 1); break;
            case TR_POLYC: vfo_polyc_body(bid, reinterpret_cast<float2*>(smem), reinterpret_cast<const PolyJob*>(e_jobs), e_aux); break;
            case TR_DEEMP_P0: vfo_deemph_body<0, 0>(bid, smem, reinterpret_cast<const DeempJob*>(e_jobs)); break;
            case TR_DEEMP_P1: vfo_deemph_body<0, 1>(bid, smem, reinterpret_cast<const DeempJob*>(e_jobs)); break;
            case TR_DC_P0: vfo_deemph_body<1, 0>(bid, smem, reinterpret_cast<const DeempJob*>(e_jobs)); break;
            case TR_DC_P1: vfo_deemph_body<1, 1>(bid, smem, reinterpret_cast<const DeempJob*>(e_jobs)); break;
            case TR_WF_RING: { const TickWf q = e.p.wf; wf_ring_store_body(bid, gdim, q.src, q.n0, q.n1, q.a, q.n2, q.n3); } break;
            case TR_WF_TRACE: { const TickWf q = e.p.wf; wf_trace_body(bid, q.src, q.n0, q.n1, q.a, q.b, q.f0, q.f1, q.c, q.f2); } break;
            case TR_PIPE: vfo_pipe_body<1>(bid, gdim, smem, reinterpret_cast<const PipeJob*>(e_jobs)); break;
            default: break;
            }
        }
    }
#ifdef SDRPP_TICK_TRACE
    __syncthreads();
    if (threadIdx.x == 0) {
        const unsigned k = atomicAdd(&g_tick_trace_n, 1u);
        if (k < SDRPP_TICK_TRACE_CAP) {
            unsigned hw = 0, xcc = 0;
            asm volatile("s_getreg_b32 %0, hwreg(HW_REG_HW_ID)" : "=s"(hw));
            asm volatile("s_getreg_b32 %0, hwreg(HW_REG_XCC_ID)" : "=s"(xcc));
            TickTraceRec rec{ done.value, (short)tr_role, (short)tr_entry, (int)blockIdx.x, tr_t0, (unsigned long long)wall_clock64(), hw, xcc, { 0, 0, 0, 0 } };
            for (int q = 0; q < 4; q++) {
                rec.m[q] = g_tick_mark[blockIdx.x & 0xffff][q];
                g_tick_mark[blockIdx.x & 0xffff][q] = 0;
            }
            g_tick_trace[k] = rec;
        }
    }
#endif
    tick_finish(done);
}

}
```

sdrplusplus_amd/csrc/vfo_toep_kernels.h:

```cpp
#pragma once

struct ToepJob {
    StreamIn in;
    float* out;
    const float* tl;
    const int* lbase;
    int tl_len, nsteps;
    int s_in, rows;
    int base0;
    int nout;
    int mt_per_wave;
    float inv_deviation;
};

#ifdef SDRPP_TOEP_KNOCK
__device__ int g_toep_knock;
#endif
#ifdef SDRPP_TOEP_PROF
__device__ unsigned long long g_toep_prof[4][8];
#define TOEP_TICK() ((long long)__builtin_readcyclecounter())
#endif

template <int WIDTH, int G, bool QUAD>
__device__ __forceinline__ void vfo_toep_body(const KIdx bid, const KIdx gdim, float* smemt, const ToepJob* __restrict__ jobs) {
    const ToepJob job = jobs[bid.y];
    const int tid = threadIdx.x, lane = tid & 63, wv = tid >> 6;
#ifdef SDRPP_TOEP_KNOCK
    const int knock = g_toep_knock;
#endif
    const int nsteps = job.nsteps, s_in = job.s_in, rows = job.rows;
    const int span = (G * 16 - 1) * s_in + 4 * nsteps;
    const int pl = (span + 8) & ~3;
    constexpr int NPL = (WIDTH == 2 || QUAD) ? 2 : 1;
    const int tl_pad = (job.tl_len + 3) & ~3;
    float* TLs = smemt;
    float* XR = smemt + tl_pad + wv * NPL * pl;
    float* XI = XR + pl;
    {
        constexpr int NB = 4;
        for (int i0 = tid; i0 < job.tl_len; i0 += 256 * NB) {
            float tv[NB];
#pragma unroll
            for (int q = 0; q < NB; q++) { tv[q] = global_load_f32(job.tl, min(i0 + q * 256, job.tl_len - 1)); }
#pragma unroll
            for (int q = 0; q < NB; q++) {
                if (i0 + q * 256 < job.tl_len) { TLs[i0 + q * 256] = tv[q]; }
            }
        }
    }
    __syncthreads();
    TICK_MARK(0);
    const int omt = G * 16 * rows;
    const int mt0 = bid.x * 4 + wv, mts = gdim.x * 4;
    const int c = lane & 15, kk = lane >> 4;
    const float* Bp = TLs + global_load_i32(job.lbase, lane);
    const float* Ar = XR + c * s_in + kk;
    const float* Ai = XI + c * s_in + kk;
    constexpr bool ILV = (WIDTH == 2) && !QUAD;
    float2* X2 = reinterpret_cast<float2*>(XR);
    const float2* A2 = X2 + c * s_in + kk;
    constexpr int PF = 18;
    constexpr int PF4 = 9;
    constexpr bool CPLX_IN = (WIDTH == 2) || QUAD;
    const int cnt = QUAD ? span + 1 : span;
    const int npair = (cnt + 1) >> 1;
    const bool piped = ILV ? (npair <= PF4 * 64) : (cnt <= PF * 64);
    float2 pf2[(CPLX_IN && !ILV) ? PF : 1];
    float pf1[CPLX_IN ? 1 : PF];
    float4 pf4[ILV ? PF4 : 1];
    auto fetch = [&](int mt) {
#ifdef SDRPP_TOEP_KNOCK
        if (knock & 2) { return; }
#endif
        const int lo = job.base0 + mt * G * 16 * s_in - (QUAD ? 1 : 0);
        const bool inside = lo >= 0 && lo + cnt <= job.in.n;
        if constexpr (ILV) {
            if (inside) {
#pragma unroll
                for (int q = 0; q < PF4; q++) {
                    const int e = q * 64 + lane;
                    pf4[q] = (e < npair) ? global_load_f32x4_unaligned(job.in.data, 2ll * (lo + 2 * e)) : make_float4(0.0f, 0.0f, 0.0f, 0.0f);
                }
            }
            else {
#pragma unroll
                for (int q = 0; q < PF4; q++) {
                    const int e = q * 64 + lane;
                    const float2 a = stream_load2_nb(job.in, lo + 2 * e, e < npair), b = stream_load2_nb(job.in, lo + 2 * e + 1, e < npair);
                    pf4[q] = make_float4(a.x, a.y, b.x, b.y);
                }
            }
        }
        else if constexpr (CPLX_IN) {
            if (inside) {
                const float2* src2 = reinterpret_cast<const float2*>(job.in.data) + lo;
#pragma unroll
                for (int q = 0; q < PF; q++) {
                    const int s = q * 64 + lane;
                    pf2[q] = (s < cnt) ? global_load_f32x2(src2, s) : make_float2(0.0f, 0.0f);
                }
            }
            else {
#pragma unroll
                for (int q = 0; q < PF; q++) {
                    const int s = q * 64 + lane;
                    pf2[q] = stream_load2_nb(job.in, lo + s, s < cnt);
                }
            }
        }
        else {
            if (inside) {
#pragma unroll
                for (int q = 0; q < PF; q++) {
                    const int s = q * 64 + lane;
                    pf1[q] = (s < cnt) ? global_load_f32(job.in.data + lo, s) : 0.0f;
                }
            }
            else {
#pragma unroll
                for (int q = 0; q < PF; q++) {
                    const int s = q * 64 + lane;
                    pf1[q] = stream_load1_nb(job.in, lo + s, s < cnt);
                }
            }
        }
    };
    auto window_store = [&]() {
        if constexpr (ILV) {
            float4* X4 = reinterpret_cast<float4*>(XR);
#pragma unroll
            for (int q = 0; q < PF4; q++) {
                const int e = q * 64 + lane;
                if (e < npair) { X4[e] = pf4[q]; }
            }
            return;
        }
#pragma unroll
        for (int q = 0; q < PF; q++) {
            const int s = q * 64 + lane;
            if (s < cnt) {
                if constexpr (QUAD) { XI[s] = fm_phase(pf2[q].y, pf2[q].x); }
                else if constexpr (WIDTH == 2) {
                    XR[s] = pf2[q].x;
                    XI[s] = pf2[q].y;
                }
                else { XR[s] = pf1[q]; }
            }
        }
    };
    auto discriminate = [&]() {
        if constexpr (QUAD) {
            wave_sync();
            for (int s = lane; s < span; s += 64) { XR[s] = normalize_phase(XI[s + 1] - XI[s]) * job.inv_deviation; }
        }
    };
#ifdef SDRPP_TOEP_PROF
    long long tp_acc[5] = { 0, 0, 0, 0, 0 }, tp_rounds = 0;
    const long long tp_birth = TOEP_TICK();
#endif
    if (piped && mt0 * omt < job.nout) {
        fetch(mt0);
        window_store();
        if (1 < job.mt_per_wave && (mt0 + mts) * omt < job.nout) { fetch(mt0 + mts); }
        discriminate();
        TICK_MARK(1);
    }
    for (int it = 0; it < job.mt_per_wave; it++) {
        const int mt = mt0 + it * mts;
        const int obase = mt * omt;
        if (obase >= job.nout) { break; }
        if (!piped) {
            const int lo = job.base0 + mt * G * 16 * s_in - (QUAD ? 1 : 0);
            for (int s = lane; s < cnt; s += 64) {
                if constexpr (QUAD) {
                    const float2 x = stream_load2(job.in, lo + s);
                    XI[s] = fm_phase(x.y, x.x);
                }
                else if constexpr (WIDTH == 2) { X2[s] = stream_load2(job.in, lo + s); }
                else { XR[s] = stream_load1(job.in, lo + s); }
            }
            discriminate();
        }
        wave_sync();
#ifdef SDRPP_TOEP_PROF
        const long long tp0 = TOEP_TICK();
#endif
        f32x4 accR[G], accI[G];
#pragma unroll
        for (int g = 0; g < G; g++) { accR[g] = mfma4_zero(); accI[g] = mfma4_zero(); }
        {
            constexpr int U = (WIDTH == 2) ? 4 : 8;
            int t0 = 0;
#ifdef SDRPP_TOEP_KNOCK
            if (knock & 4) { t0 = nsteps; }
#endif
            for (; t0 + U <= nsteps; t0 += U) {
                float b[U], xr[U][G], xi[U][G];
#pragma unroll
                for (int u = 0; u < U; u++) {
                    b[u] = Bp[4 * (t0 + u)];
#pragma unroll
                    for (int g = 0; g < G; g++) {
                        if constexpr (ILV) {
                            const float2 a = A2[g * 16 * s_in + 4 * (t0 + u)];
                            xr[u][g] = a.x;
                            xi[u][g] = a.y;
                        }
                        else {
                            xr[u][g] = Ar[g * 16 * s_in + 4 * (t0 + u)];
                            if constexpr (WIDTH == 2) { xi[u][g] = Ai[g * 16 * s_in + 4 * (t0 + u)]; }
                        }
                    }
                }
#pragma unroll
                for (int u = 0; u < U; u++) {
#pragma unroll
                    for (int g = 0; g < G; g++) {
                        accR[g] = mfma_16x16x4(xr[u][g], b[u], accR[g]);
                        if constexpr (WIDTH == 2) { accI[g] = mfma_16x16x4(xi[u][g], b[u], accI[g]); }
                    }
                }
            }
            for (; t0 < nsteps; t0++) {
                const float b = Bp[4 * t0];
#pragma unroll
                for (int g = 0; g < G; g++) {
                    if constexpr (ILV) {
                        const float2 a = A2[g * 16 * s_in + 4 * t0];
                        accR[g] = mfma_16x16x4(a.x, b, accR[g]);
                        accI[g] = mfma_16x16x4(a.y, b, accI[g]);
                    }
                    else {
                        accR[g] = mfma_16x16x4(Ar[g * 16 * s_in + 4 * t0], b, accR[g]);
                        if constexpr (WIDTH == 2) { accI[g] = mfma_16x16x4(Ai[g * 16 * s_in + 4 * t0], b, accI[g]); }
                    }
                }
            }
        }
#ifdef SDRPP_TOEP_PROF
        sched_fence();
        const long long tp1 = TOEP_TICK();
        long long tp2 = tp1, tp3 = tp1, tp4 = tp1;
#endif
        if (it == 0) { TICK_MARK(2); }
        if (piped && it + 1 < job.mt_per_wave && (mt + mts) * omt < job.nout) {
            wave_sync();
            window_store();
#ifdef SDRPP_TOEP_PROF
            sched_fence();
            tp2 = TOEP_TICK();
#endif
            if (it + 2 < job.mt_per_wave && (mt + 2 * mts) * omt < job.nout) { fetch(mt + 2 * mts); }
#ifdef SDRPP_TOEP_PROF
            sched_fence();
            tp3 = TOEP_TICK();
#endif
            discriminate();
            sched_fence();
#ifdef SDRPP_TOEP_PROF
            tp4 = TOEP_TICK();
#endif
        }
#ifdef SDRPP_TOEP_KNOCK
        if ((knock & 1) && accR[0][0] != 123.456f) { continue; }
#endif
        if (obase + omt <= job.nout) {
            if (c < rows) {
                float2* const ob = reinterpret_cast<float2*>(job.out) + obase;
                const int lofs = 4 * kk * rows + c;
#pragma unroll
                for (int g = 0; g < G; g++) {
#pragma unroll
                    for (int r = 0; r < 4; r++) {
                        global_store_f32x2(ob + (g * 16 + r) * rows, lofs, make_float2(accR[g][r], (WIDTH == 2) ? accI[g][r] : accR[g][r]));
                    }
                }
            }
        }
        else if (c < rows) {
#pragma unroll
            for (int g = 0; g < G; g++) {
#pragma unroll
                for (int r = 0; r < 4; r++) {
                    const int o = obase + (g * 16 + 4 * kk + r) * rows + c;
                    if (o < job.nout) {
                        if constexpr (WIDTH == 2) { global_store_f32x2(reinterpret_cast<float2*>(job.out), o, make_float2(accR[g][r], accI[g][r])); }
                        else { global_store_f32x2(reinterpret_cast<float2*>(job.out), o, make_float2(accR[g][r], accR[g][r])); }
                    }
                }
            }
        }
        if (!piped) { wave_sync(); }
#ifdef SDRPP_TOEP_PROF
        sched_fence();
        const long long tp5 = TOEP_TICK();
        tp_acc[0] += tp1 - tp0;
        tp_acc[1] += tp2 - tp1;
        tp_acc[2] += tp3 - tp2;
        tp_acc[3] += tp4 - tp3;
        tp_acc[4] += tp5 - tp4;
        tp_rounds++;
#endif
    }
#ifdef SDRPP_TOEP_PROF
    if (lane == 0) {
        const int kind = QUAD ? 3 : (s_in >= 30 ? 0 : (rows < 15 ? 1 : 2));
        for (int k = 0; k < 5; k++) { atomicAdd(&g_toep_prof[kind][k], (unsigned long long)tp_acc[k]); }
        atomicAdd(&g_toep_prof[kind][5], (unsigned long long)tp_rounds);
        atomicAdd(&g_toep_prof[kind][6], (unsigned long long)(TOEP_TICK() - tp_birth));
        atomicAdd(&g_toep_prof[kind][7], 1ull);
    }
#endif
}
template <int WIDTH, int G, bool QUAD>
__global__ __launch_bounds__(256, 5) void vfo_toep_kernel(const ToepJob* __restrict__ jobs) {
    HIP_DYNAMIC_SHARED(float, smemt)
    vfo_toep_body<WIDTH, G, QUAD>(kidx(blockIdx), kidx(gridDim), smemt, jobs);
}
```

Measured before the change: 23820.

## Emit FM phase from channel FIR and feed phase-difference audio Toeplitz kernel

```diff
diff --git a/sdrplusplus_amd/csrc/gfx950/sdrpp_gfx950.h b/sdrplusplus_amd/csrc/gfx950/sdrpp_gfx950.h
--- a/sdrplusplus_amd/csrc/gfx950/sdrpp_gfx950.h
+++ b/sdrplusplus_amd/csrc/gfx950/sdrpp_gfx950.h
@@ -175,8 +175,7 @@
 
 __device__ __forceinline__ float wave_bcast(float v, int src) { return __int_as_float(__builtin_amdgcn_readlane(__float_as_int(v), src)); }
 __device__ __forceinline__ float wave_shr1(float v, float first) {
-    const float r = __shfl_up(v, 1, 64);
-    return ((threadIdx.x & 63) == 0) ? first : r;
+    return __int_as_float(__builtin_amdgcn_update_dpp(__float_as_int(first), __float_as_int(v), 0x138, 0xf, 0xf, false));
 }
 __device__ __forceinline__ int wave_first(bool pred) {
     const unsigned long long m = __ballot(pred);
diff --git a/sdrplusplus_amd/csrc/host_ctx.h b/sdrplusplus_amd/csrc/host_ctx.h
--- a/sdrplusplus_amd/csrc/host_ctx.h
+++ b/sdrplusplus_amd/csrc/host_ctx.h
@@ -68,6 +68,8 @@
     double theta2 = 0.0, phi2 = 0.0;
     std::vector<Stream> st;
     int i_first = 0, i_poly = -1, i_chan = -1, i_dem = -1, i_out = -1, i_if = 0;
+    int i_phase = -1;
+    int phase_have = 0;
     int lvl_if = 1, lvl_out = 1, lvl_af = 1;
     std::vector<int> tk_if, tk_af;
     ToepTab tp_stage[SDRPP_MAX_DECIM_STAGES], tp_poly, tp_chan, tp_audio;
diff --git a/sdrplusplus_amd/csrc/host_util.h b/sdrplusplus_amd/csrc/host_util.h
--- a/sdrplusplus_amd/csrc/host_util.h
+++ b/sdrplusplus_amd/csrc/host_util.h
@@ -349,6 +349,7 @@
 }
 
 int vfo_reset_state(sdrpp_ctx* c, Vfo& v) {
+    v.phase_have = 0;
     v.phi = 0.0;
     v.phi2 = 0.0;
     v.seen = 0;
@@ -458,6 +459,7 @@
     case TR_TOEP_C: hipLaunchKernelGGL((vfo_toep_kernel<2, 2, false>), grid, b256, r.lds, st, (const ToepJob*)e.jobs); break;
     case TR_TOEP_R: hipLaunchKernelGGL((vfo_toep_kernel<1, 2, false>), grid, b256, r.lds, st, (const ToepJob*)e.jobs); break;
     case TR_TOEP_Q: hipLaunchKernelGGL((vfo_toep_kernel<1, 2, true>), grid, b256, r.lds, st, (const ToepJob*)e.jobs); break;
+    case TR_TOEP_D: hipLaunchKernelGGL((vfo_toep_kernel<1, 2, false, true>), grid, b256, r.lds, st, (const ToepJob*)e.jobs); break;
     case TR_FIRB_C: hipLaunchKernelGGL((vfo_firb_kernel<2, false>), grid, dim3((unsigned)e.aux), r.lds, st, (const FirBJob*)e.jobs); break;
     case TR_FIRB_R: hipLaunchKernelGGL((vfo_firb_kernel<1, false>), grid, dim3((unsigned)e.aux), r.lds, st, (const FirBJob*)e.jobs); break;
     case TR_FIRB_S: hipLaunchKernelGGL((vfo_firb_kernel<1, true>), grid, dim3((unsigned)e.aux), r.lds, st, (const FirBJob*)e.jobs); break;
diff --git a/sdrplusplus_amd/csrc/plan_push.h b/sdrplusplus_amd/csrc/plan_push.h
--- a/sdrplusplus_amd/csrc/plan_push.h
+++ b/sdrplusplus_amd/csrc/plan_push.h
@@ -4,7 +4,7 @@
 
 struct PlanSnapshot {
     struct V { int soff[SDRPP_MAX_DECIM_STAGES]; int pphase, poff; double phi, phi2; long long seen; int i_if, lvl_if, lvl_out, lvl_af; int n[24], cur[24]; size_t nrecs;
-               int af_soff[SDRPP_MAX_DECIM_STAGES], af_pphase, af_poff, af_last, af_state; };
+               int af_soff[SDRPP_MAX_DECIM_STAGES], af_pphase, af_poff, af_last, af_state, phase_have; };
     std::vector<V> v;
     int64_t fft_pos, fft_next;
     int n_lines, iq_cur, wf_cur, wf_lines;
@@ -19,7 +19,7 @@
         for (int k = 0; k < SDRPP_MAX_DECIM_STAGES; k++) { q.soff[k] = v.soff[k]; q.af_soff[k] = v.af.soff[k]; }
         q.pphase = v.pphase; q.poff = v.poff; q.phi = v.phi; q.phi2 = v.phi2; q.seen = v.seen; q.i_if = v.i_if; q.lvl_if = v.lvl_if; q.lvl_out = v.lvl_out; q.lvl_af = v.lvl_af;
         q.nrecs = v.recs.size();
-        q.af_pphase = v.af.pphase; q.af_poff = v.af.poff; q.af_last = v.af.i_last; q.af_state = v.af.state_cur;
+        q.af_pphase = v.af.pphase; q.af_poff = v.af.poff; q.af_last = v.af.i_last; q.af_state = v.af.state_cur; q.phase_have = v.phase_have;
         for (size_t k = 0; k < v.st.size() && k < 24; k++) { q.n[k] = v.st[k].n; q.cur[k] = v.st[k].cur; }
         if (rotate) {
             for (auto& st : v.st) { stream_rotate(st); }
@@ -38,7 +38,7 @@
         const PlanSnapshot::V& q = S.v[i];
         for (int k = 0; k < SDRPP_MAX_DECIM_STAGES; k++) { v.soff[k] = q.soff[k]; v.af.soff[k] = q.af_soff[k]; }
         v.pphase = q.pphase; v.poff = q.poff; v.phi = q.phi; v.phi2 = q.phi2; v.seen = q.seen; v.i_if = q.i_if; v.lvl_if = q.lvl_if; v.lvl_out = q.lvl_out; v.lvl_af = q.lvl_af;
-        v.af.pphase = q.af_pphase; v.af.poff = q.af_poff; v.af.i_last = q.af_last; v.af.state_cur = q.af_state;
+        v.af.pphase = q.af_pphase; v.af.poff = q.af_poff; v.af.i_last = q.af_last; v.af.state_cur = q.af_state; v.phase_have = q.phase_have;
         for (size_t k = 0; k < v.st.size() && k < 24; k++) { v.st[k].n = q.n[k]; v.st[k].cur = q.cur[k]; }
     }
     c->fft_pos = S.fft_pos; c->fft_next = S.fft_next; c->n_lines = S.n_lines; c->iq_cur = S.iq_cur;
diff --git a/sdrplusplus_amd/csrc/plan_vfo.h b/sdrplusplus_amd/csrc/plan_vfo.h
--- a/sdrplusplus_amd/csrc/plan_vfo.h
+++ b/sdrplusplus_amd/csrc/plan_vfo.h
@@ -186,6 +186,7 @@
     Lev<FirBJob> audio;
     Lev<FirBJob> audio_fm;
     Lev<ToepJob> t_dec, t_poly, t_chan, t_audio, t_audio_fm;
+    Lev<ToepJob> t_audio_d;
     std::vector<PipeJob> pipes;
     size_t pipe_lds = 0;
     PipeJob* d_pipes = nullptr;
@@ -217,10 +218,10 @@
     RotJob* d_rot = nullptr;
     const int* d_fb = nullptr;
     struct ToepList { Lev<ToepJob>* L; int npl, width; bool quad; int fam; int role; };
-    static constexpr int kToepLists = 8;
+    static constexpr int kToepLists = 9;
     ToepList tlists[kToepLists] = { { &t_dec, 2, 2, false, F_DECIM, TR_TOEP_C },      { &t_poly, 2, 2, false, F_POLY, TR_TOEP_C },       { &t_chan, 2, 2, false, F_FIR, TR_TOEP_C },
                                     { &t_audio, 1, 1, false, F_FIR, TR_TOEP_R },      { &t_audio_fm, 2, 1, true, F_FIR, TR_TOEP_Q },     { &t_af_dec, 2, 2, false, F_AF, TR_TOEP_C },
-                                    { &t_af_poly, 2, 2, false, F_AF, TR_TOEP_C },     { &t_af_hpf, 2, 2, false, F_AF, TR_TOEP_C } };
+                                    { &t_af_poly, 2, 2, false, F_AF, TR_TOEP_C },     { &t_af_hpf, 2, 2, false, F_AF, TR_TOEP_C },       { &t_audio_d, 1, 1, false, F_FIR, TR_TOEP_D } };
     ToepPlan tplan[kToepLists][kLevels];
 
     explicit BankPlan(sdrpp_ctx* c_) : c(c_), fb(c_->vfo_bounds) {
@@ -244,7 +245,7 @@
         lev_reset(f_dec); lev_reset(poly);
         for (auto& q : polyb) { lev_reset(q); }
         lev_reset(chan); lev_reset(seq); lev_reset(pre); lev_reset(audio); lev_reset(audio_fm);
-        lev_reset(t_dec); lev_reset(t_poly); lev_reset(t_chan); lev_reset(t_audio); lev_reset(t_audio_fm);
+        lev_reset(t_dec); lev_reset(t_poly); lev_reset(t_chan); lev_reset(t_audio); lev_reset(t_audio_fm); lev_reset(t_audio_d);
         lev_reset(t_af_dec); lev_reset(t_af_poly); lev_reset(t_af_hpf); lev_reset(af_dec); lev_reset(af_hpf); lev_reset(af_poly); lev_reset(af_deemp);
         lev_reset(ssbx_l); lev_reset(carry);
         pipe_lds = 0;
@@ -467,11 +468,22 @@
             nxt->wlevel = lvl;
             cur = nxt;
         }
+        Stream* const ph = v.i_phase >= 0 ? &v.st[(size_t)v.i_phase] : nullptr;
+        const bool phase_feed = ticking && ph && (v.d.demod == SDRPP_DEMOD_WFM || v.d.demod == SDRPP_DEMOD_NFM) && v.i_chan >= 0 && v.chan_ntaps > 0 && v.tp_chan.ok &&
+                                v.tp_audio.ok;
+        if (ph) { ph->n = 0; }
         if (v.i_chan >= 0 && v.chan_ntaps > 0) {
             Stream* nxt = &v.st[(size_t)v.i_chan];
             lvl++;
             cur->clevel = lvl;
-            if (piped_be) {
+            if (phase_feed) {
+                ToepJob j = toep_job(v.tp_chan, 0, stream_in(*cur), nxt->data, -(v.chan_ntaps - 1), cur->n, 0.0f);
+                j.phase_out = ph->data;
+                t_chan.add(lvl, j);
+                ph->n = cur->n;
+                ph->wlevel = lvl;
+            }
+            else if (piped_be) {
                 pj.st[2] = toep_job(v.tp_chan, 0, stream_in(*cur), nxt->data, -(v.chan_ntaps - 1), cur->n, 0.0f);
                 pj.keep[2] = 0;
             }
@@ -501,6 +513,10 @@
                 pj.st[3] = toep_job(v.tp_audio, 0, stream_in(*cur), out.data, -(v.audio_ntaps - 1), nif, v.d.inv_deviation);
                 pipes.push_back(pj);
                 pipe_lds = std::max(pipe_lds, pj_lds);
+            }
+            else if (phase_feed && v.phase_have >= ph->hist_len) {
+                ph->clevel = lvl;
+                t_audio_d.add(lvl, toep_job(v.tp_audio, 0, stream_in(*ph), out.data, -(v.audio_ntaps - 1), nif, v.d.inv_deviation));
             }
             else if (v.tp_audio.ok) { t_audio_fm.add(lvl, toep_job(v.tp_audio, 0, stream_in(*cur), out.data, -(v.audio_ntaps - 1), nif, v.d.inv_deviation)); }
             else { audio_fm.add(lvl, FirBJob{ stream_in(*cur), out.data, v.d_audio, v.audio_ntaps, 0, 0, nif, v.audio_kp, v.d.inv_deviation }); }
@@ -614,9 +630,10 @@
             v.phi = p - std::floor(p);
         }
         v.seen += n_in;
+        v.phase_have = phase_feed ? std::min(ph->hist_len, v.phase_have + nif) : 0;
         const Stream* phantom = (v.fused_front && v.d.n_stages >= 2 && !v.nco_exact) ? &v.st[(size_t)v.i_first] : nullptr;
         for (auto& s : v.st) {
-            if (s.hist_len > 0 && s.data && &s != phantom) {
+            if (s.hist_len > 0 && s.data && &s != phantom && !(&s == ph && !phase_feed)) {
                 const int cl = !ticking ? carry_last : (s.clevel > 0 ? s.clevel : (s.wlevel > 0 ? s.wlevel + 1 : lvl + 1));
                 carry.add(cl, CarryJob{ s.data, s.hist[s.cur], s.hist[s.cur ^ 1], s.hist_len, s.n, s.width, s.hist_len });
             }
@@ -1229,6 +1246,7 @@
                 FamilyTimer t(c, F_FIR);
                 emit_toep(3, l);
                 emit_toep(4, l);
+                emit_toep(8, l);
                 if (l < audio.top) {
                     rc = launch_fir(l, F_FIR, audio.at[l], audio.dev[l], 1, true);
                     if (rc) { return rc; }
diff --git a/sdrplusplus_amd/csrc/sdrpp_gpu.hip b/sdrplusplus_amd/csrc/sdrpp_gpu.hip
--- a/sdrplusplus_amd/csrc/sdrpp_gpu.hip
+++ b/sdrplusplus_amd/csrc/sdrpp_gpu.hip
@@ -908,6 +908,10 @@
         }
         v->i_out = add_stream(2, 0, cap);
         if (v->i_out < 0) { return SDRPP_ERR_NOMEM; }
+        if (fm) {
+            v->i_phase = add_stream(1, v->audio_ntaps, cap);
+            if (v->i_phase < 0) { return SDRPP_ERR_NOMEM; }
+        }
     }
     v->d.audio_taps = nullptr;
     rc = dev_alloc(c, &v->d_state, 2 * sizeof(AgcState) + sizeof(float));
@@ -1032,6 +1036,7 @@
     if (it == c->vfos.end()) { return fail(c, SDRPP_ERR_NOT_FOUND, "no VFO %d", id); }
     Vfo& v = *it->second;
     HIPCHK(c, hipStreamSynchronize(c->stream));
+    v.phase_have = 0;
     {
         const int idx = (v.i_poly >= 0) ? v.i_poly : v.i_first + std::max(v.d.n_stages, 1) - 1;
         Stream& fs = v.st[(size_t)idx];
@@ -1939,7 +1944,7 @@
     static const char* const names[] = { "none", "copy", "carry", "rot", "fcm_132_4", "fcm_6", "fcm_10", "fcm_16", "fcm16_132_4", "fcl_0", "fcl_pf", "toep_c", "toep_r", "toep_q",
                                          "firb_c", "firb_r", "firb_s", "firb_q", "pre", "seq", "fft_s10", "fft_s11", "fft_s12", "fft_p1_5", "fft_p1_6", "fft_p1_7", "fft_p1_8", "fft_p1_9",
                                          "fft_p1_10", "fft_p2_7", "fft_p2_8", "fft_p2_9", "fft_p2_10", "fft_p2row", "fft_tr", "zoom_16", "zoom_4", "zoom_1", "polyc", "deemp_p0", "deemp_p1",
-                                         "dc_p0", "dc_p1", "wf_ring", "wf_trace", "pipe", "rotx16", "fird", "ssbx", "s1_1", "s1d_1", "f2_1", "poly" };
+                                         "dc_p0", "dc_p1", "wf_ring", "wf_trace", "pipe", "rotx16", "fird", "ssbx", "s1_1", "s1d_1", "f2_1", "poly", "toep_d" };
     static_assert(sizeof(names) / sizeof(names[0]) == TR_COUNT, "role names out of step with TickRole");
     return (role >= 0 && role < TR_COUNT) ? names[role] : nullptr;
 }
diff --git a/sdrplusplus_amd/csrc/tick_host.h b/sdrplusplus_amd/csrc/tick_host.h
--- a/sdrplusplus_amd/csrc/tick_host.h
+++ b/sdrplusplus_amd/csrc/tick_host.h
@@ -59,7 +59,7 @@
     case TR_POLYC: return 55;
     case TR_DEEMP_P1: case TR_DC_P1: return 52;
     case TR_DEEMP_P0: case TR_DC_P0: return 48;
-    case TR_TOEP_Q: return 65;
+    case TR_TOEP_Q: case TR_TOEP_D: return 65;
     case TR_TOEP_C: case TR_TOEP_R: case TR_FFT_S10: case TR_FFT_S11: case TR_FFT_S12: return 60;
     case TR_FFT_P2_7: case TR_FFT_P2_8: case TR_FFT_P2_9: case TR_FFT_P2_10: case TR_FFT_P2ROW: return 50;
     case TR_FFT_TR: return 25;
diff --git a/sdrplusplus_amd/csrc/tick_kernels.h b/sdrplusplus_amd/csrc/tick_kernels.h
--- a/sdrplusplus_amd/csrc/tick_kernels.h
+++ b/sdrplusplus_amd/csrc/tick_kernels.h
@@ -90,6 +90,7 @@
     TR_S1D_1,
     TR_F2_1,
     TR_POLY,
+    TR_TOEP_D,
     TR_COUNT
 };
 struct TickP1 { IqSrc src; FrameGeom g; const float* window; const float2* tw1; const float2* twn; float2* scratch; int lg2, ntiles; };
@@ -248,6 +249,7 @@
             case TR_TOEP_C: vfo_toep_body<2, 2, false>(bid, gdim, smem, reinterpret_cast<const ToepJob*>(e_jobs)); break;
             case TR_TOEP_R: vfo_toep_body<1, 2, false>(bid, gdim, smem, reinterpret_cast<const ToepJob*>(e_jobs)); break;
             case TR_TOEP_Q: vfo_toep_body<1, 2, true>(bid, gdim, smem, reinterpret_cast<const ToepJob*>(e_jobs)); break;
+            case TR_TOEP_D: vfo_toep_body<1, 2, false, true>(bid, gdim, smem, reinterpret_cast<const ToepJob*>(e_jobs)); break;
             case TR_FIRB_C:
                 vfo_firb_body<2, false>(bid, smem, e_aux, reinterpret_cast<const FirBJob*>(e_jobs));
                 break;
diff --git a/sdrplusplus_amd/csrc/vfo_toep_kernels.h b/sdrplusplus_amd/csrc/vfo_toep_kernels.h
--- a/sdrplusplus_amd/csrc/vfo_toep_kernels.h
+++ b/sdrplusplus_amd/csrc/vfo_toep_kernels.h
@@ -11,6 +11,7 @@
     int nout;
     int mt_per_wave;
     float inv_deviation;
+    float* phase_out;
 };
 
 #ifdef SDRPP_TOEP_KNOCK
@@ -21,8 +22,9 @@
 #define TOEP_TICK() ((long long)__builtin_readcyclecounter())
 #endif
 
-template <int WIDTH, int G, bool QUAD>
+template <int WIDTH, int G, bool QUAD, bool DIFF = false>
 __device__ __forceinline__ void vfo_toep_body(const KIdx bid, const KIdx gdim, float* smemt, const ToepJob* __restrict__ jobs) {
+    static_assert(!DIFF || (WIDTH == 1 && !QUAD), "DIFF reads a real phase stream");
     const ToepJob job = jobs[bid.y];
     const int tid = threadIdx.x, lane = tid & 63, wv = tid >> 6;
 #ifdef SDRPP_TOEP_KNOCK
@@ -62,7 +64,8 @@
     constexpr int PF = 18;
     constexpr int PF4 = 9;
     constexpr bool CPLX_IN = (WIDTH == 2) || QUAD;
-    const int cnt = QUAD ? span + 1 : span;
+    constexpr bool DISC = QUAD || DIFF;
+    const int cnt = DISC ? span + 1 : span;
     const int npair = (cnt + 1) >> 1;
     const bool piped = ILV ? (npair <= PF4 * 64) : (cnt <= PF * 64);
     float2 pf2[(CPLX_IN && !ILV) ? PF : 1];
@@ -72,7 +75,7 @@
 #ifdef SDRPP_TOEP_KNOCK
         if (knock & 2) { return; }
 #endif
-        const int lo = job.base0 + mt * G * 16 * s_in - (QUAD ? 1 : 0);
+        const int lo = job.base0 + mt * G * 16 * s_in - (DISC ? 1 : 0);
         const bool inside = lo >= 0 && lo + cnt <= job.in.n;
         if constexpr (ILV) {
             if (inside) {
@@ -132,6 +135,18 @@
             for (int q = 0; q < PF4; q++) {
                 const int e = q * 64 + lane;
                 if (e < npair) { X4[e] = pf4[q]; }
+            }
+            return;
+        }
+        if constexpr (DIFF) {
+            float last = 0.0f;
+#pragma unroll
+            for (int q = 0; q < PF; q++) {
+                const float prev = wave_shr1(pf1[q], last);
+                last = wave_bcast(pf1[q], 63);
+                const int s = q * 64 + lane;
+                const float d = normalize_phase(pf1[q] - prev) * job.inv_deviation;
+                if (s >= 1 && s < cnt) { XR[s - 1] = d; }
             }
             return;
         }
@@ -170,8 +185,11 @@
         const int obase = mt * omt;
         if (obase >= job.nout) { break; }
         if (!piped) {
-            const int lo = job.base0 + mt * G * 16 * s_in - (QUAD ? 1 : 0);
-            for (int s = lane; s < cnt; s += 64) {
+            const int lo = job.base0 + mt * G * 16 * s_in - (DISC ? 1 : 0);
+            if constexpr (DIFF) {
+                for (int s = lane; s < span; s += 64) { XR[s] = normalize_phase(stream_load1(job.in, lo + s + 1) - stream_load1(job.in, lo + s)) * job.inv_deviation; }
+            }
+            else for (int s = lane; s < cnt; s += 64) {
                 if constexpr (QUAD) {
                     const float2 x = stream_load2(job.in, lo + s);
                     XI[s] = fm_phase(x.y, x.x);
@@ -275,6 +293,16 @@
                         global_store_f32x2(ob + (g * 16 + r) * rows, lofs, make_float2(accR[g][r], (WIDTH == 2) ? accI[g][r] : accR[g][r]));
                     }
                 }
+                if constexpr (WIDTH == 2) {
+                    if (job.phase_out) {
+                        float* const pb = job.phase_out + obase;
+#pragma unroll
+                        for (int g = 0; g < G; g++) {
+#pragma unroll
+                            for (int r = 0; r < 4; r++) { global_store_f32_boff(pb + (g * 16 + r) * rows, (unsigned)lofs * 4u, fm_phase(accI[g][r], accR[g][r])); }
+                        }
+                    }
+                }
             }
         }
         else if (c < rows) {
@@ -284,7 +312,10 @@
                 for (int r = 0; r < 4; r++) {
                     const int o = obase + (g * 16 + 4 * kk + r) * rows + c;
                     if (o < job.nout) {
-                        if constexpr (WIDTH == 2) { global_store_f32x2(reinterpret_cast<float2*>(job.out), o, make_float2(accR[g][r], accI[g][r])); }
+                        if constexpr (WIDTH == 2) {
+                            global_store_f32x2(reinterpret_cast<float2*>(job.out), o, make_float2(accR[g][r], accI[g][r]));
+                            if (job.phase_out) { global_store_f32_boff(job.phase_out, (unsigned)o * 4u, fm_phase(accI[g][r], accR[g][r])); }
+                        }
                         else { global_store_f32x2(reinterpret_cast<float2*>(job.out), o, make_float2(accR[g][r], accR[g][r])); }
                     }
                 }
@@ -304,7 +335,7 @@
     }
 #ifdef SDRPP_TOEP_PROF
     if (lane == 0) {
-        const int kind = QUAD ? 3 : (s_in >= 30 ? 0 : (rows < 15 ? 1 : 2));
+        const int kind = DISC ? 3 : (s_in >= 30 ? 0 : (rows < 15 ? 1 : 2));
         for (int k = 0; k < 5; k++) { atomicAdd(&g_toep_prof[kind][k], (unsigned long long)tp_acc[k]); }
         atomicAdd(&g_toep_prof[kind][5], (unsigned long long)tp_rounds);
         atomicAdd(&g_toep_prof[kind][6], (unsigned long long)(TOEP_TICK() - tp_birth));
@@ -312,8 +343,8 @@
     }
 #endif
 }
-template <int WIDTH, int G, bool QUAD>
+template <int WIDTH, int G, bool QUAD, bool DIFF = false>
 __global__ __launch_bounds__(256, 5) void vfo_toep_kernel(const ToepJob* __restrict__ jobs) {
     HIP_DYNAMIC_SHARED(float, smemt)
-    vfo_toep_body<WIDTH, G, QUAD>(kidx(blockIdx), kidx(gridDim), smemt, jobs);
+    vfo_toep_body<WIDTH, G, QUAD, DIFF>(kidx(blockIdx), kidx(gridDim), smemt, jobs);
 }
```

Measured after the change: 23580, median of 6. -1.0%, worse.
